# George0828Zhang/simulst

Measured on AMD Instinct MI355X. Metric: decoded tgt tokens/sec (Emformer encoder + wait-k=5 greedy decode, MuST-C en-de shape), higher is better.
Workload: dtype bf16; 1 GPU; configs[1]: Emformer enc (12L) + wait-k=5 dec (6L), 80x1000 fbank, batch 64/GPU, 110 forced greedy steps; batch_per_gpu=64, frames=1000, decode_steps=110, streams=3, warmup_steps_executed=164

## Files before the change

include/simulst_hip.h:

```cpp
#ifndef SIMULST_HIP_H
#define SIMULST_HIP_H

#include <stdint.h>

#ifdef __cplusplus
extern "C" {
#endif

typedef struct simulst_handle simulst_handle;

enum { SIMULST_F32 = 0, SIMULST_BF16 = 1 };

enum {
  SIMULST_OK = 0,
  SIMULST_E_NULL = -1,
  SIMULST_E_SHAPE = -2,
  SIMULST_E_DTYPE = -3,
  SIMULST_E_ARG = -4
};

enum {
  SIMULST_EPI_BIAS = 0,
  SIMULST_EPI_BIAS_GELU = 1,
  SIMULST_EPI_BIAS_RES = 2,
  SIMULST_EPI_GLU = 3,
  SIMULST_EPI_EMF_OUT = 4,
  SIMULST_EPI_BIAS_F32OUT = 5,
  SIMULST_EPI_BIAS_RES_GELU = 6
};

enum { SIMULST_ATTN_HARD = 0, SIMULST_ATTN_INFINITE_LOOKBACK = 1, SIMULST_ATTN_WAITK = 2,
       SIMULST_ATTN_CHUNKWISE = 3, SIMULST_ATTN_FULL = 4 };

enum { SIMULST_K_LINEAR = 0, SIMULST_K_LAYERNORM = 1, SIMULST_K_EMF_ATTN = 2, SIMULST_K_CONV_POS = 3,
       SIMULST_K_DEC_SELF_ATTN = 4, SIMULST_K_DEC_CROSS_ATTN = 5, SIMULST_K_SCAN = 6,
       SIMULST_K_ARGMAX = 7, SIMULST_K_MISC = 8, SIMULST_K_LINEAR_SKINNY = 9, SIMULST_K_LINEAR_TILE64 = 10,
       SIMULST_K_DEC_QKV_CHAIN = 11, SIMULST_K_DEC_PROJ_CHAIN = 12, SIMULST_K_DEC_FFN_CHAIN = 13,
       SIMULST_K_DEC_ATTN_CHAIN = 14, SIMULST_K_DEC_VOCAB_CHAIN = 15,
       SIMULST_K_DEC_TALL_GEMM = 16, SIMULST_K_COUNT = 17 };

int simulst_create(simulst_handle** out, void* hip_stream);
int simulst_destroy(simulst_handle* h);
int simulst_set_stream(simulst_handle* h, void* hip_stream);
const char* simulst_last_error(simulst_handle* h);
int simulst_version(void);
int simulst_stream_create(void** out_stream, int32_t priority, const uint32_t* cu_mask, int32_t mask_words);
int simulst_stream_destroy(void* stream);
int simulst_timer_enable(simulst_handle* h, int kernel_class, int on);
int simulst_timer_read(simulst_handle* h, int kernel_class, double* total_ms, int64_t* launches);
int simulst_timer_reset(simulst_handle* h);
int simulst_graph_enable(simulst_handle* h, int on);
enum { SIMULST_OPT_VALU_ATTENTION = 0, SIMULST_OPT_UNFUSED_DECODE = 1, SIMULST_OPT_FFN_WAVES = 2, SIMULST_OPT_DEC_CHAIN = 3,
       SIMULST_OPT_DEC_ATTN_CHAIN_MAX_ROWS = 4, SIMULST_OPT_DEC_ATTN_CHAIN_ROWS = 5, SIMULST_OPT_FUSED_ARGMAX = 6,
       SIMULST_OPT_DEC_VOCAB_CHAIN_SPLIT = 7, SIMULST_OPT_DEC_EMBED_QKV_CHAIN = 8, SIMULST_OPT_PANEL_WIDE = 9,
       SIMULST_OPT_DEC_FUSE_PROJ_CROSS = 10, SIMULST_OPT_WEIGHT_STATIONARY = 11, SIMULST_OPT_CONV_TILE256 = 12, SIMULST_OPT_DEC_FUSE_FFN_QKV = 13, SIMULST_OPT_DEC_CHAIN_ROWS32 = 14,
       SIMULST_OPT_DEC_TALL_FFN = 15 };
int simulst_set_option(simulst_handle* h, int32_t option, int32_t value);
int simulst_get_option(simulst_handle* h, int32_t option, int32_t* value);
int simulst_has_experiments(void);

#ifdef SIMULST_DEBUG_HOOKS
int simulst_debug_ffn_variant(simulst_handle* h, int variant);

int simulst_debug_chain_lds_bytes(simulst_handle* h, int32_t bytes);
int simulst_debug_chain_xmode(simulst_handle* h, int32_t mode);
int simulst_debug_chain_tail(simulst_handle* h, void* dbg);
int64_t simulst_debug_chain_probe_bytes(int32_t B);
int simulst_debug_chain_probe(simulst_handle* h, const void* ctx, void* x, const void* wo_fm, const float* bo,
                              const float* ln_g, const float* ln_b, const void* wq_fm, const float* bq, void* q,
                              int32_t B, int32_t variant, void* dbg);
#endif

typedef struct {
  int32_t M_batches, rows_per_batch, N, K;
  int64_t a_batch_stride, a_row_stride, a_lead;
  int64_t c_batch_stride, c_row_stride;
  int64_t r_batch_stride, r_row_stride;
  int32_t epilogue, dtype;
  float scale;
  int32_t n_main, aux_rows;
  int64_t aux_batch_stride;
  const float* ln_gamma;
  const float* ln_beta;
  int32_t w_fragment_major;
  int32_t c_head_dim;
  int64_t c_head_stride;
  int32_t c_tensor_heads;
  int64_t c_tensor_stride;
} simulst_linear_desc;

int simulst_linear(simulst_handle* h, const simulst_linear_desc* d, const void* A, const void* W,
                   const float* bias, const void* R, void* C, void* aux);
int simulst_dec_tall_gemm(simulst_handle* h, const void* A, const void* W, const float* bias, const void* R, void* C,
                          int32_t B, int32_t N, int32_t K, int32_t dtype);
int simulst_dec_tall_fc1(simulst_handle* h, const void* A, const void* W, const float* bias, const float* ln_g, const float* ln_b,
                         void* C, int32_t B, int32_t N, int32_t K, int32_t dtype);

int simulst_fbank(simulst_handle* h, const float* wave, int64_t wave_stride, const float* window, const float* tw_cos,
                  const float* tw_sin, const int32_t* mel_lo, const float* mel_w, void* out, int32_t B,
                  int32_t n_frames, int32_t n_mel, float preemphasis, int32_t out_dtype);

int simulst_conv_pos(simulst_handle* h, const void* x, const void* hist, const void* W,
                     const float* bias, const int32_t* lengths, void* y,
                     int32_t B, int32_t T, int32_t D, int32_t groups, int32_t k, int32_t dtype);

int simulst_conv_pos_mfma(simulst_handle* h, const void* x, const void* hist, const void* Wp, const float* bias,
                          const int32_t* lengths, void* y, int32_t B, int32_t T, int32_t D, int32_t groups,
                          int32_t k);

int simulst_emformer_pack_rows(simulst_handle* h, const void* x, void* X, int32_t B, int32_t T, int32_t D, int32_t seg_len,
                               int32_t right_context, int32_t n_seg, int32_t dtype);

int simulst_emformer_ffn(simulst_handle* h, const void* x, const float* ln_gamma, const float* ln_beta,
                         const void* w1_packed, const float* b1, const void* w2_packed, const float* b2, void* out,
                         int64_t rows, int32_t D, int32_t F, int32_t dtype);

int simulst_emformer_ffn_prenorm(simulst_handle* h, const void* x, const float* ln_gamma, const float* ln_beta,
                                 const void* w1_packed, const float* b1, const void* w2_packed, const float* b2, void* out,
                                 const float* next_gamma, const float* next_beta, const int32_t* lengths, void* z_next,
                                 int32_t B, int32_t T, int32_t D, int32_t F, int32_t n_mem, int32_t n_rc, int32_t n_sum,
                                 int32_t seg_len, int32_t dtype);

int simulst_emformer_ffn_prenorm_qkv(simulst_handle* h, const void* x, const float* ln_gamma, const float* ln_beta,
                                     const void* w1_packed, const float* b1, const void* w2_packed, const float* b2, void* out,
                                     const float* next_gamma, const float* next_beta, const int32_t* lengths, void* z_next,
                                     const void* wqkv_fm, const float* bqkv, void* qkv_next,
                                     int32_t B, int32_t T, int32_t D, int32_t F, int32_t n_mem, int32_t n_rc, int32_t n_sum,
                                     int32_t seg_len, int32_t dtype);

int simulst_emformer_qkv_mem_sum(simulst_handle* h, const void* z, const void* wqkv_fm, const float* bqkv, void* qkv,
                                 int32_t B, int32_t T, int32_t D, int32_t n_mem, int32_t n_rc, int32_t n_sum, int32_t dtype);

int simulst_emformer_prenorm(simulst_handle* h, const void* X, const float* gamma, const float* beta,
                             const int32_t* lengths, void* Z, int32_t B, int32_t T, int32_t D,
                             int32_t n_mem, int32_t n_rc, int32_t n_sum, int32_t seg_len, int32_t dtype);

int simulst_layernorm(simulst_handle* h, const void* X, const float* gamma, const float* beta, void* Y,
                      int64_t rows, int32_t D, int64_t x_row_stride, int64_t y_row_stride, int32_t dtype);

int simulst_segment_mean(simulst_handle* h, const void* X, const int32_t* lengths, void* out,
                         int32_t B, int32_t T, int32_t D, int64_t x_batch_stride, int64_t out_batch_stride,
                         int32_t seg_len, int32_t n_out, int32_t dtype);

typedef struct {
  int32_t B, T, D, H, S, R, Lc, M;
  int32_t n_mem, n_seg;
  int32_t use_summary;
  int32_t dtype;
} simulst_emf_attn_desc;

int simulst_emformer_attention(simulst_handle* h, const simulst_emf_attn_desc* d, const void* QKV,
                               const int32_t* lengths, const void* lc_k, const void* lc_v,
                               const int32_t* lc_valid, const int32_t* n_mem_valid, void* CTX);

int simulst_waitk_p_choose(simulst_handle* h, float* p, const int32_t* key_len, int32_t BH,
                           int32_t tgt_len, int32_t tgt_offset, int32_t S, int32_t k, int32_t online);

int simulst_mma_step_search(simulst_handle* h, const float* p, int64_t* head_step, uint8_t* head_read,
                            float* alpha, const int32_t* src_len, int32_t BH, int32_t S,
                            int32_t mass_preservation);

int simulst_expected_alignment(simulst_handle* h, const float* p, float* alpha, const int32_t* key_len,
                               int32_t BH, int32_t U, int32_t S, float eps);

int simulst_mass_preservation(simulst_handle* h, float* alpha, const int32_t* key_len,
                              int32_t BH, int32_t U, int32_t S);

int simulst_expected_delays(simulst_handle* h, const float* alpha, float* out, int64_t rows, int32_t S);

enum { SIMULST_LATENCY_AL = 0, SIMULST_LATENCY_AP = 1, SIMULST_LATENCY_DAL = 2 };
int simulst_latency_metric(simulst_handle* h, const float* delays, const float* src_len, const float* tgt_len,
                           const uint8_t* target_padding_mask, float* out, int32_t B, int32_t T, int32_t metric);

int simulst_expected_alignment_backward(simulst_handle* h, const float* p, const float* alpha, const float* grad_alpha,
                                        float* grad_p, const int32_t* key_len, int32_t BH, int32_t U, int32_t S,
                                        float eps);
int simulst_expected_delays_backward(simulst_handle* h, const float* grad_out, float* grad_alpha, int64_t rows, int32_t S);
int simulst_latency_metric_backward(simulst_handle* h, const float* delays, const float* src_len, const float* tgt_len,
                                    const uint8_t* target_padding_mask, const float* grad_out, float* grad_delays,
                                    int32_t B, int32_t T, int32_t metric);

int simulst_expected_soft_attention(simulst_handle* h, const float* alpha, const float* energy,
                                    float* beta, const int32_t* key_len, int32_t BH, int32_t U,
                                    int32_t S, int32_t chunk_size, float eps);

int simulst_step_p_choose(simulst_handle* h, const void* q, const void* Kmono, float energy_bias,
                          const int32_t* key_len, float* p, int32_t B, int32_t S_cap, int32_t H, int32_t d,
                          int32_t ratio, int32_t incremental, int32_t attn_type, int32_t waitk_k,
                          const int32_t* tgt_idx, int32_t online, int32_t dtype);

int simulst_step_p_choose_padded(simulst_handle* h, const void* q, const void* Kmono, float energy_bias,
                                 const int32_t* key_len, float* p, int32_t B, int32_t S_pad, int32_t S_cap, int32_t H,
                                 int32_t d, int32_t ratio, int32_t incremental, int32_t attn_type, float pad_threshold,
                                 int32_t dtype);

int simulst_cif_integrate(simulst_handle* h, const void* x, const float* alpha, const int32_t* src_len,
                          void* out, int32_t* cif_len, float* delays, float* tail_w, float* alpha_sum,
                          int32_t B, int32_t S, int32_t C, int32_t T_cap, float beta, float tail_thres,
                          int32_t dtype);

int simulst_cif_alpha_head(simulst_handle* h, const void* hidden, const float* gamma, const float* beta_ln,
                           const void* w, float bias, float* alpha, int64_t rows, int32_t D, int32_t dtype);

int simulst_embed_tokens(simulst_handle* h, const int64_t* tokens, const void* E, const float* pos_table,
                         const int32_t* pos_row, void* x, int32_t B, int32_t D, float scale, int32_t dtype);

int simulst_decoder_self_attention(simulst_handle* h, const void* qkv, void* k_cache, void* v_cache,
                                   const int32_t* n_prev, void* ctx, int32_t B, int32_t H, int32_t d,
                                   int32_t cap, int32_t dtype);

int simulst_decoder_cross_attention(simulst_handle* h, const void* q, const void* Kc, const void* Vc,
                                    const int64_t* step, const int32_t* key_len, void* ctx, float* beta,
                                    int32_t B, int32_t H, int32_t d, int32_t S_cap, int32_t attn_type,
                                    int32_t mass_preservation, int32_t dtype);

int simulst_greedy_argmax(simulst_handle* h, const float* logits, const float* eos_bias, int64_t* out,
                          int32_t B, int32_t V, int32_t pad_idx, int32_t eos_idx, int32_t mask_eos);

int simulst_pack_fragment_major(simulst_handle* h, const void* W, void* out, int32_t N, int32_t K, int32_t dtype);

int64_t simulst_ctc_best_alignment_scratch_bytes(int32_t N, int32_t S, int32_t max_target_length);
int simulst_ctc_best_alignment(simulst_handle* h, const float* log_probs, int64_t lp_stride_t, int64_t lp_stride_b,
                               int64_t lp_stride_v, const int64_t* targets, int64_t tg_stride_b,
                               const int64_t* input_lengths, const int64_t* target_lengths, int32_t S, int32_t N,
                               int32_t max_target_length, int32_t blank, int32_t as_labels, void* scratch,
                               int64_t* out, float* neg_log_likelihood);

typedef struct {
  const void* wqkv; const float* bqkv;
  const void* wo; const float* bo;
  const float *ln1_g, *ln1_b, *ln2_g, *ln2_b, *ln3_g, *ln3_b;
  const void* c_wq; const float* c_bq;
  const void* c_wq_soft; const float* c_bq_soft;
  const void* c_wo; const float* c_bo;
  const void* fc1; const float* b1; const void* fc2; const float* b2;
  float energy_bias;
  void *k_cache, *v_cache;
  int64_t* head_step;
  uint8_t* head_read;
  const void *Kmono, *Ksoft, *V;
  const float* Kpool;
} simulst_dec_layer;

typedef struct {
  int32_t B, D, H, F, V, n_layers, cap, S_cap, dtype;
  int32_t attn_type, ratio, waitk_k, mass_preservation, online;
  int32_t pad_idx, eos_idx;
  int32_t n_prev_uniform;
  float embed_scale;
  const void* E;
  const void* out_proj;
  const float* pos_table;
  const float *ln_g, *ln_b;
  const int32_t* enc_len;
  int32_t* n_prev;
  void *x, *qkv, *ctx, *q, *q2, *hidden;
  float* logits;
  void* x_mid;
  float* partial_self;
  int32_t weights_fragment_major;
  float* ffn_partial;
  int32_t P_cap;
  int32_t* ffn_sem;
} simulst_decoder_desc;

int simulst_mma_decode(simulst_handle* h, const simulst_decoder_desc* d, const simulst_dec_layer* layers,
                       int64_t* tokens_io, int64_t* out_tokens, int32_t n_steps, int32_t mask_eos);

int simulst_mma_retire_rows(simulst_handle* h, const simulst_decoder_desc* d, const simulst_dec_layer* layers,
                            const int64_t* chunk_tokens, int32_t n_steps, int32_t rows, int32_t B, int32_t* slot_row,
                            int32_t* row_cap, int64_t* last_tokens, int64_t* hyp, int32_t U, int32_t* enc_len_bh,
                            int32_t* result);

int simulst_beam_topk(simulst_handle* h, const float* logits, int32_t R, int32_t V, int32_t beam, int32_t step,
                      const int32_t* max_len, const int32_t* finished, int32_t pad_idx, int32_t eos_idx, float* cand_lp,
                      int32_t* cand_tok);

int simulst_beam_select(simulst_handle* h, const float* cand_lp, const int32_t* cand_tok, int32_t Bs, int32_t beam, int32_t V,
                        int32_t step, const int32_t* max_len, int32_t L, double lenpen, int32_t eos_idx, float* cum,
                        int64_t* next_tok, int32_t* reorder, int32_t* bp_parent, int32_t* bp_token, float* bp_cum,
                        int32_t* fin_step, int32_t* fin_row, float* fin_score, float* fin_raw, int32_t* fin_count,
                        int32_t* finished, int32_t* result);

int simulst_beam_reorder(simulst_handle* h, const simulst_decoder_desc* d, const simulst_dec_layer* src, const simulst_dec_layer* dst,
                         const int32_t* reorder, const int32_t* finished, int32_t beam, int32_t n_prev, int32_t* result);

int simulst_beam_backtrack(simulst_handle* h, int32_t Bs, int32_t beam, int32_t nbest, int32_t L, const int32_t* bp_parent,
                           const int32_t* bp_token, const float* bp_cum, const int32_t* fin_step, const int32_t* fin_row,
                           const float* fin_score, const float* fin_raw, const int32_t* fin_count, int32_t pad_idx,
                           int32_t eos_idx, int64_t* tokens, int32_t* lengths, float* scores, float* pos_scores);

typedef struct {
  uint8_t* active;
  uint8_t* read_flag;
  uint8_t* online;
  uint8_t* done;
  int32_t* delays_ms;
  int64_t* hyp;
  int32_t cap, cur_ms, max_len_now;
  int32_t n_chunks;
  const int32_t* sched_rows;
  const int32_t* sched_ms;
  const int32_t* sched_max_len;
  int32_t* chunk_idx;
  int32_t* enc_len;
  int32_t* tok_chunk;
  const int32_t* row_chunks;
  int32_t ff_waitk, ff_ratio;
  float* p_probe; int64_t* step_probe; const int64_t* step_force; int32_t probe_P;
  int32_t* row_map; int32_t compact_rows;
} simulst_stream_ctl;

int simulst_mma_stream_steps(simulst_handle* h, const simulst_decoder_desc* d, const simulst_dec_layer* layers,
                             int64_t* tokens_io, const simulst_stream_ctl* ctl, int32_t n_iter);


typedef struct {
  const void* wqkv; const float* bqkv;
  const void* wo; const float* bo;
  const float *ln1_g, *ln1_b, *ln2_g, *ln2_b, *ln3_g, *ln3_b;
  const void* c_wq;
  const void* c_wo; const float* c_bo;
  const void* fc1; const float* b1; const void* fc2; const float* b2;
  void *k_cache, *v_cache;
  const void* Kc;
} simulst_cif_dec_layer;

typedef struct {
  int32_t B, D, H, F, V, n_layers, cap, n_cap, dtype;
  int32_t pad_idx, eos_idx;
  int32_t highway;
  int32_t n_prev_uniform;
  float embed_scale, overshoot_weight;
  const void* E; const void* out_proj; const float* pos_table; const float *ln_g, *ln_b;
  const int32_t* cif_len;
  const void* cif;
  int32_t* n_prev;
  void *x, *qkv, *ctx, *q, *hidden;
  float* logits;
  void* kk;
  void* cif_t;
  float* eos_bias;
  void* x_mid; float* ffn_partial;
  int32_t weights_fragment_major;
} simulst_cif_decoder_desc;

int simulst_cif_decode(simulst_handle* h, const simulst_cif_decoder_desc* d, const simulst_cif_dec_layer* layers,
                       int64_t* tokens_io, int64_t* out_tokens, int32_t n_steps, int32_t mask_eos);

typedef struct {
  uint8_t* online;
  uint8_t* done;
  int32_t* delays_ms;
  int64_t* hyp;
  int32_t cap, cur_ms, max_len_now;
  int32_t n_chunks;
  const int32_t* sched_cif_len;
  const int32_t* sched_ms;
  const int32_t* sched_max_len;
  int32_t* chunk_idx;
  int32_t* cif_len;
  int32_t* tok_chunk;
  const int32_t* row_chunks;
} simulst_cif_stream_ctl;

int simulst_cif_stream_steps(simulst_handle* h, const simulst_cif_decoder_desc* d, const simulst_cif_dec_layer* layers,
                             int64_t* tokens_io, const simulst_cif_stream_ctl* ctl, int32_t n_iter);

int simulst_cif_stream_append(simulst_handle* h, const void* out, const int32_t* n, const float* tail_w, void* acc,
                              int32_t* acc_len, void* prev_feat, float* prev_weight, int32_t B, int32_t T_cap, int32_t n_cap,
                              int32_t D, float beta, int32_t finish, int32_t dtype);

int simulst_decoder_proj_chain(simulst_handle* h, const void* ctx, void* x, const void* wo_fm, const float* bo,
                               const float* ln_g, const float* ln_b, const void* wq_fm, const float* bq, void* q,
                               const void* wq2_fm, const float* bq2, void* q2, int32_t B, int32_t D, int32_t dtype);
int simulst_decoder_ffn_chain(simulst_handle* h, const void* ctx, void* x, const void* wco_fm, const float* bco,
                              const float* ln_g, const float* ln_b, const void* w1_fm, const float* b1, const void* w2_fm,
                              const float* b2, float* partial, int32_t* sem, void* x_mid, int32_t B, int32_t D, int32_t F,
                              int32_t dtype);
int simulst_decoder_slab_sum_qkv(simulst_handle* h, const void* x_mid, void* x, const float* partial, const float* b2,
                                 const float* ln_g, const float* ln_b, const void* wqkv_fm, const float* bqkv, void* qkv,
                                 int32_t B, int32_t D, int32_t F, int32_t dtype);

int simulst_decoder_vocab_chain(simulst_handle* h, const void* x_mid, void* x, const float* partial, const float* b2,
                                const float* ln_g, const float* ln_b, const void* wout_fm, float* pairs, int32_t B, int32_t D,
                                int32_t F, int32_t V, int32_t split, int32_t skip_a, int32_t skip_b, const float* row_bias,
                                int32_t row_bias_col, int32_t dtype);

#ifdef SIMULST_EXPERIMENTS
int simulst_decoder_attn_proj_chain(simulst_handle* h, const void* qkv, void* k_cache, void* v_cache, const int32_t* n_prev,
                                    void* x, const void* wo_fm, const float* bo, const float* ln_g, const float* ln_b,
                                    const void* wq_fm, const float* bq, void* q, const void* wq2_fm, const float* bq2, void* q2,
                                    const void* kk_gelu, int32_t B, int32_t H, int32_t d, int32_t cap, int32_t n_prev_uniform,
                                    int32_t rows_per_workgroup, int32_t dtype);
#endif

int simulst_pool_keys(simulst_handle* h, const void* Kmono, float* Kpool, const int32_t* key_len, int32_t B, int32_t H, int32_t d,
                      int32_t S_cap, int32_t P_cap, int32_t ratio, int32_t j_lo, int32_t j_hi, int32_t dtype);

int simulst_policy_cross_attention(simulst_handle* h, const void* qm, const void* qs, const void* Kmono,
                                   const void* Ksoft, const void* Vc, float energy_bias, const int32_t* key_len,
                                   const int32_t* tgt_idx, int64_t* head_step, uint8_t* head_read, void* ctx,
                                   int32_t B, int32_t H, int32_t d, int32_t S_cap, int32_t ratio, int32_t attn_type,
                                   int32_t waitk_k, int32_t online, int32_t mass_preservation, int32_t dtype);

int simulst_decoder_self_attention_causal(simulst_handle* h, const void* qkv, void* ctx, int32_t B, int32_t U, int32_t H,
                                          int32_t d, int32_t dtype);

enum { SIMULST_ENERGY_SOFT = 0, SIMULST_ENERGY_MONOTONIC = 1, SIMULST_ENERGY_WAITK = 2 };
int simulst_mma_energy(simulst_handle* h, const void* q, const void* K, float* out, const int32_t* key_len, float energy_bias,
                       float pad_threshold, int32_t B, int32_t U, int32_t S, int32_t S_cap, int32_t H, int32_t d, int32_t ratio,
                       int32_t mode, int32_t waitk_k, int32_t dtype);

int simulst_mma_softmax(simulst_handle* h, float* energy, const int32_t* key_len, int32_t B, int32_t U, int32_t S, int32_t H);

int simulst_mma_context(simulst_handle* h, const float* beta, const void* V, void* ctx, int32_t B, int32_t U, int32_t S,
                        int32_t S_cap, int32_t H, int32_t d, int32_t dtype);

int simulst_transducer_pool(simulst_handle* h, const void* x, const int32_t* lengths, void* y, int32_t* new_len, int32_t B,
                            int32_t S_in, int32_t D, int64_t x_batch_stride, int32_t T_max, int32_t k, int32_t dtype);

int simulst_joiner_scan(simulst_handle* h, const float* P, const float* g, const void* W_fm, const int32_t* prev_emit,
                        const int32_t* src_len, float* blank_logit, float* best, int32_t* best_idx, int32_t B, int32_t S,
                        int32_t D, int32_t V, int32_t blank, int32_t n_split, int32_t dtype);

int simulst_joiner_emit(simulst_handle* h, const float* P, const float* g, const float* blank_logit, const float* best,
                        const int32_t* best_idx, int32_t* prev_emit, const int32_t* src_len, void* z, int32_t* at_eos, int32_t B,
                        int32_t S, int32_t D, int32_t V, int32_t blank, int32_t n_split, int32_t dtype);

int simulst_joiner_mask_blank(simulst_handle* h, float* logits, const int32_t* at_eos, int32_t B, int32_t V, int32_t blank);

#ifdef __cplusplus
}
#endif
#endif
```

simulst_amd/_lib.py:

```python
import ctypes as C
import os

_HERE = os.path.dirname(os.path.abspath(__file__))
LIB_PATH = os.environ.get("SIMULST_LIB_PATH") or os.path.join(_HERE, "libsimulst_hip.so")

F32, BF16 = 0, 1
EPI_BIAS, EPI_BIAS_GELU, EPI_BIAS_RES, EPI_GLU, EPI_EMF_OUT, EPI_BIAS_F32OUT, EPI_BIAS_RES_GELU = range(7)
ATTN_HARD, ATTN_INFINITE_LOOKBACK, ATTN_WAITK, ATTN_CHUNKWISE, ATTN_FULL = range(5)
(K_LINEAR, K_LAYERNORM, K_EMF_ATTN, K_CONV_POS, K_DEC_SELF_ATTN, K_DEC_CROSS_ATTN, K_SCAN, K_ARGMAX,
 K_MISC, K_LINEAR_SKINNY, K_LINEAR_TILE64, K_DEC_QKV_CHAIN, K_DEC_PROJ_CHAIN, K_DEC_FFN_CHAIN, K_DEC_ATTN_CHAIN,
 K_DEC_VOCAB_CHAIN, K_DEC_TALL_GEMM, K_COUNT) = range(18)
KERNEL_CLASS_NAMES = ["linear", "layernorm", "emformer_attention", "conv_pos", "decoder_self_attention",
                      "decoder_cross_attention", "scan", "argmax", "misc", "linear_skinny", "linear_tile64",
                      "dec_qkv_chain", "dec_proj_chain", "dec_ffn_chain", "dec_attn_proj_chain", "dec_vocab_chain", "dec_tall_gemm"]

ATTN_ENUM = {"hard_aligned": ATTN_HARD, "infinite_lookback": ATTN_INFINITE_LOOKBACK,
             "waitk": ATTN_WAITK, "chunkwise": ATTN_CHUNKWISE, "full": ATTN_FULL}


class LinearDesc(C.Structure):
    _fields_ = [("M_batches", C.c_int32), ("rows_per_batch", C.c_int32), ("N", C.c_int32), ("K", C.c_int32),
                ("a_batch_stride", C.c_int64), ("a_row_stride", C.c_int64), ("a_lead", C.c_int64),
                ("c_batch_stride", C.c_int64), ("c_row_stride", C.c_int64),
                ("r_batch_stride", C.c_int64), ("r_row_stride", C.c_int64),
                ("epilogue", C.c_int32), ("dtype", C.c_int32), ("scale", C.c_float),
                ("n_main", C.c_int32), ("aux_rows", C.c_int32), ("aux_batch_stride", C.c_int64),
                ("ln_gamma", C.c_void_p), ("ln_beta", C.c_void_p), ("w_fragment_major", C.c_int32),
                ("c_head_dim", C.c_int32), ("c_head_stride", C.c_int64),
                ("c_tensor_heads", C.c_int32), ("c_tensor_stride", C.c_int64)]


class EmfAttnDesc(C.Structure):
    _fields_ = [(n, C.c_int32) for n in ("B", "T", "D", "H", "S", "R", "Lc", "M", "n_mem", "n_seg",
                                         "use_summary", "dtype")]


_vp, _i32, _i64, _f32 = C.c_void_p, C.c_int32, C.c_int64, C.c_float


class DecLayer(C.Structure):
    _fields_ = [(n, C.c_void_p) for n in ("wqkv", "bqkv", "wo", "bo", "ln1_g", "ln1_b", "ln2_g", "ln2_b", "ln3_g",
                                          "ln3_b", "c_wq", "c_bq", "c_wq_soft", "c_bq_soft", "c_wo", "c_bo", "fc1",
                                          "b1", "fc2", "b2")] + [("energy_bias", C.c_float)] + \
               [(n, C.c_void_p) for n in ("k_cache", "v_cache", "head_step", "head_read", "Kmono", "Ksoft", "V", "Kpool")]


class DecoderDesc(C.Structure):
    _fields_ = [(n, C.c_int32) for n in ("B", "D", "H", "F", "V", "n_layers", "cap", "S_cap", "dtype", "attn_type",
                                         "ratio", "waitk_k", "mass_preservation", "online", "pad_idx", "eos_idx",
                                         "n_prev_uniform")] + \
               [("embed_scale", C.c_float)] + \
               [(n, C.c_void_p) for n in ("E", "out_proj", "pos_table", "ln_g", "ln_b", "enc_len", "n_prev", "x", "qkv",
                                          "ctx", "q", "q2", "hidden", "logits", "x_mid", "partial_self")] + \
               [("weights_fragment_major", C.c_int32), ("ffn_partial", C.c_void_p), ("P_cap", C.c_int32), ("ffn_sem", C.c_void_p)]

class CifDecLayer(C.Structure):
    _fields_ = [(n, C.c_void_p) for n in ("wqkv", "bqkv", "wo", "bo", "ln1_g", "ln1_b", "ln2_g", "ln2_b", "ln3_g", "ln3_b",
                                          "c_wq", "c_wo", "c_bo", "fc1", "b1", "fc2", "b2", "k_cache", "v_cache", "Kc")]


class CifDecoderDesc(C.Structure):
    _fields_ = [(n, C.c_int32) for n in ("B", "D", "H", "F", "V", "n_layers", "cap", "n_cap", "dtype", "pad_idx", "eos_idx",
                                         "highway", "n_prev_uniform")] + \
               [("embed_scale", C.c_float), ("overshoot_weight", C.c_float)] + \
               [(n, C.c_void_p) for n in ("E", "out_proj", "pos_table", "ln_g", "ln_b", "cif_len", "cif", "n_prev", "x", "qkv",
                                          "ctx", "q", "hidden", "logits", "kk", "cif_t", "eos_bias", "x_mid", "ffn_partial")] + \
               [("weights_fragment_major", C.c_int32)]


class CifStreamCtl(C.Structure):
    _fields_ = [(n, C.c_void_p) for n in ("online", "done", "delays_ms", "hyp")] + \
               [(n, C.c_int32) for n in ("cap", "cur_ms", "max_len_now", "n_chunks")] + \
               [(n, C.c_void_p) for n in ("sched_cif_len", "sched_ms", "sched_max_len", "chunk_idx", "cif_len", "tok_chunk", "row_chunks")]


class StreamCtl(C.Structure):
    _fields_ = [(n, C.c_void_p) for n in ("active", "read_flag", "online", "done", "delays_ms", "hyp")] + \
               [(n, C.c_int32) for n in ("cap", "cur_ms", "max_len_now", "n_chunks")] + \
               [(n, C.c_void_p) for n in ("sched_rows", "sched_ms", "sched_max_len", "chunk_idx", "enc_len", "tok_chunk", "row_chunks")] + \
               [(n, C.c_int32) for n in ("ff_waitk", "ff_ratio")] + \
               [(n, C.c_void_p) for n in ("p_probe", "step_probe", "step_force")] + [("probe_P", C.c_int32)] + \
               [("row_map", C.c_void_p), ("compact_rows", C.c_int32)]


SIGNATURES = {
    "simulst_create": [C.POINTER(_vp), _vp],
    "simulst_destroy": [_vp],
    "simulst_set_stream": [_vp, _vp],
    "simulst_last_error": [_vp],
    "simulst_version": [],
    "simulst_timer_enable": [_vp, C.c_int, C.c_int],
    "simulst_timer_read": [_vp, C.c_int, C.POINTER(C.c_double), C.POINTER(_i64)],
    "simulst_timer_reset": [_vp],
    "simulst_graph_enable": [_vp, C.c_int],
    "simulst_set_option": [_vp, _i32, _i32],
    "simulst_get_option": [_vp, _i32, C.POINTER(_i32)],
    "simulst_stream_create": [C.POINTER(_vp), _i32, _vp, _i32],
    "simulst_stream_destroy": [_vp],
    "simulst_pack_fragment_major": [_vp, _vp, _vp, _i32, _i32, _i32],
    "simulst_linear": [_vp, C.POINTER(LinearDesc), _vp, _vp, _vp, _vp, _vp, _vp],
    "simulst_dec_tall_gemm": [_vp, _vp, _vp, _vp, _vp, _vp, _i32, _i32, _i32, _i32],
    "simulst_dec_tall_fc1": [_vp, _vp, _vp, _vp, _vp, _vp, _vp, _i32, _i32, _i32, _i32],
    "simulst_conv_pos": [_vp, _vp, _vp, _vp, _vp, _vp, _vp, _i32, _i32, _i32, _i32, _i32, _i32],
    "simulst_ctc_best_alignment_scratch_bytes": [_i32, _i32, _i32],
    "simulst_ctc_best_alignment": [_vp, _vp, _i64, _i64, _i64, _vp, _i64, _vp, _vp, _i32, _i32, _i32, _i32, _i32, _vp,
                                   _vp, _vp],
    "simulst_fbank": [_vp, _vp, _i64, _vp, _vp, _vp, _vp, _vp, _vp, _i32, _i32, _i32, C.c_float, _i32],
    "simulst_conv_pos_mfma": [_vp, _vp, _vp, _vp, _vp, _vp, _vp, _i32, _i32, _i32, _i32, _i32],
    "simulst_emformer_pack_rows": [_vp, _vp, _vp, _i32, _i32, _i32, _i32, _i32, _i32, _i32],
    "simulst_emformer_ffn": [_vp, _vp, _vp, _vp, _vp, _vp, _vp, _vp, _vp, _i64, _i32, _i32, _i32],
    "simulst_emformer_ffn_prenorm": [_vp, _vp, _vp, _vp, _vp, _vp, _vp, _vp, _vp, _vp, _vp, _vp, _vp, _i32, _i32, _i32, _i32, _i32, _i32,
                                     _i32, _i32, _i32],
    "simulst_emformer_ffn_prenorm_qkv": [_vp, _vp, _vp, _vp, _vp, _vp, _vp, _vp, _vp, _vp, _vp, _vp, _vp, _vp, _vp, _vp, _i32, _i32, _i32, _i32,
                                         _i32, _i32, _i32, _i32, _i32],
    "simulst_emformer_qkv_mem_sum": [_vp, _vp, _vp, _vp, _vp, _i32, _i32, _i32, _i32, _i32, _i32, _i32],
    "simulst_emformer_prenorm": [_vp, _vp, _vp, _vp, _vp, _vp, _i32, _i32, _i32, _i32, _i32, _i32, _i32, _i32],
    "simulst_layernorm": [_vp, _vp, _vp, _vp, _vp, _i64, _i32, _i64, _i64, _i32],
    "simulst_segment_mean": [_vp, _vp, _vp, _vp, _i32, _i32, _i32, _i64, _i64, _i32, _i32, _i32],
    "simulst_emformer_attention": [_vp, C.POINTER(EmfAttnDesc), _vp, _vp, _vp, _vp, _vp, _vp, _vp],
    "simulst_waitk_p_choose": [_vp, _vp, _vp, _i32, _i32, _i32, _i32, _i32, _i32],
    "simulst_mma_step_search": [_vp, _vp, _vp, _vp, _vp, _vp, _i32, _i32, _i32],
    "simulst_expected_alignment": [_vp, _vp, _vp, _vp, _i32, _i32, _i32, _f32],
    "simulst_mass_preservation": [_vp, _vp, _vp, _i32, _i32, _i32],
    "simulst_expected_delays": [_vp, _vp, _vp, _i64, _i32],
    "simulst_latency_metric": [_vp, _vp, _vp, _vp, _vp, _vp, _i32, _i32, _i32],
    "simulst_expected_alignment_backward": [_vp, _vp, _vp, _vp, _vp, _vp, _i32, _i32, _i32, _f32],
    "simulst_expected_delays_backward": [_vp, _vp, _vp, _i64, _i32],
    "simulst_latency_metric_backward": [_vp, _vp, _vp, _vp, _vp, _vp, _vp, _i32, _i32, _i32],
    "simulst_expected_soft_attention": [_vp, _vp, _vp, _vp, _vp, _i32, _i32, _i32, _i32, _f32],
    "simulst_step_p_choose": [_vp, _vp, _vp, _f32, _vp, _vp, _i32, _i32, _i32, _i32, _i32, _i32, _i32, _i32,
                              _vp, _i32, _i32],
    "simulst_cif_integrate": [_vp, _vp, _vp, _vp, _vp, _vp, _vp, _vp, _vp, _i32, _i32, _i32, _i32, _f32, _f32, _i32],
    "simulst_cif_alpha_head": [_vp, _vp, _vp, _vp, _vp, _f32, _vp, _i64, _i32, _i32],
    "simulst_embed_tokens": [_vp, _vp, _vp, _vp, _vp, _vp, _i32, _i32, _f32, _i32],
    "simulst_decoder_self_attention": [_vp, _vp, _vp, _vp, _vp, _vp, _i32, _i32, _i32, _i32, _i32],
    "simulst_decoder_cross_attention": [_vp, _vp, _vp, _vp, _vp, _vp, _vp, _vp, _i32, _i32, _i32, _i32, _i32,
                                        _i32, _i32],
    "simulst_greedy_argmax": [_vp, _vp, _vp, _vp, _i32, _i32, _i32, _i32, _i32],
    "simulst_mma_decode": [_vp, C.POINTER(DecoderDesc), C.POINTER(DecLayer), _vp, _vp, _i32, _i32],
    "simulst_mma_stream_steps": [_vp, C.POINTER(DecoderDesc), C.POINTER(DecLayer), _vp, C.POINTER(StreamCtl), _i32],
    "simulst_mma_retire_rows": [_vp, C.POINTER(DecoderDesc), C.POINTER(DecLayer), _vp, _i32, _i32, _i32, _vp, _vp, _vp, _vp, _i32,
                                _vp, _vp],
    "simulst_beam_topk": [_vp, _vp, _i32, _i32, _i32, _i32, _vp, _vp, _i32, _i32, _vp, _vp],
    "simulst_beam_select": [_vp, _vp, _vp, _i32, _i32, _i32, _i32, _vp, _i32, C.c_double, _i32] + [_vp] * 13,
    "simulst_beam_reorder": [_vp, C.POINTER(DecoderDesc), C.POINTER(DecLayer), C.POINTER(DecLayer), _vp, _vp, _i32, _i32, _vp],
    "simulst_beam_backtrack": [_vp, _i32, _i32, _i32, _i32] + [_vp] * 8 + [_i32, _i32] + [_vp] * 4,
    "simulst_step_p_choose_padded": [_vp, _vp, _vp, _f32, _vp, _vp] + [_i32] * 8 + [_f32, _i32],
    "simulst_pool_keys": [_vp, _vp, _vp, _vp] + [_i32] * 9,
    "simulst_policy_cross_attention": [_vp, _vp, _vp, _vp, _vp, _vp, _f32, _vp, _vp, _vp, _vp, _vp, _i32, _i32, _i32,
                                       _i32, _i32, _i32, _i32, _i32, _i32, _i32],
    "simulst_cif_decode": [_vp, C.POINTER(CifDecoderDesc), C.POINTER(CifDecLayer), _vp, _vp, _i32, _i32],
    "simulst_cif_stream_steps": [_vp, C.POINTER(CifDecoderDesc), C.POINTER(CifDecLayer), _vp, C.POINTER(CifStreamCtl), _i32],
    "simulst_cif_stream_append": [_vp] * 8 + [_i32, _i32, _i32, _i32, C.c_float, _i32, _i32],
    "simulst_decoder_proj_chain": [_vp] * 13 + [_i32, _i32, _i32],
    "simulst_decoder_ffn_chain": [_vp] * 14 + [_i32, _i32, _i32, _i32],
    "simulst_decoder_slab_sum_qkv": [_vp] * 10 + [_i32, _i32, _i32, _i32],
    "simulst_decoder_vocab_chain": [_vp] * 9 + [_i32] * 7 + [_vp, _i32, _i32],
    "simulst_has_experiments": [],
    "simulst_decoder_self_attention_causal": [_vp, _vp, _vp, _i32, _i32, _i32, _i32, _i32],
    "simulst_mma_energy": [_vp, _vp, _vp, _vp, _vp, _f32, _f32] + [_i32] * 10,
    "simulst_mma_softmax": [_vp, _vp, _vp, _i32, _i32, _i32, _i32],
    "simulst_mma_context": [_vp, _vp, _vp, _vp] + [_i32] * 7,
    "simulst_transducer_pool": [_vp, _vp, _vp, _vp, _vp, _i32, _i32, _i32, _i64, _i32, _i32, _i32],
    "simulst_joiner_scan": [_vp] * 9 + [_i32] * 7,
    "simulst_joiner_emit": [_vp] * 10 + [_i32] * 7,
    "simulst_joiner_mask_blank": [_vp, _vp, _vp, _i32, _i32, _i32],
}
ENERGY_SOFT, ENERGY_MONOTONIC, ENERGY_WAITK = range(3)

EXPERIMENT_SIGNATURES = {
    "simulst_decoder_attn_proj_chain": [_vp] * 17 + [_i32] * 7,
}

DEBUG_SIGNATURES = {
    "simulst_debug_ffn_variant": [_vp, C.c_int],
    "simulst_debug_chain_lds_bytes": [_vp, _i32],
    "simulst_debug_chain_xmode": [_vp, _i32],
    "simulst_debug_chain_tail": [_vp, _vp],
    "simulst_debug_chain_probe_bytes": [_i32],
    "simulst_debug_chain_probe": [_vp] * 10 + [_i32, _i32, _vp],
}
(OPT_VALU_ATTENTION, OPT_UNFUSED_DECODE, OPT_FFN_WAVES, OPT_DEC_CHAIN, OPT_DEC_ATTN_CHAIN_MAX_ROWS, OPT_DEC_ATTN_CHAIN_ROWS,
 OPT_FUSED_ARGMAX, OPT_DEC_VOCAB_CHAIN_SPLIT, OPT_DEC_EMBED_QKV_CHAIN, OPT_PANEL_WIDE, OPT_DEC_FUSE_PROJ_CROSS,
 OPT_WEIGHT_STATIONARY, OPT_CONV_TILE256, OPT_DEC_FUSE_FFN_QKV, OPT_DEC_CHAIN_ROWS32, OPT_DEC_TALL_FFN) = range(16)

_lib = None
ABI_VERSION = 108


def load():
    global _lib
    if _lib is not None:
        return _lib
    if not os.path.exists(LIB_PATH):
        raise RuntimeError(
            f"simulst_amd: {LIB_PATH} is missing -- build it with `python -c 'import __graft_entry__ as g; "
            f"g.build()'` (or `make -C simulst_amd/csrc`). There is no CPU fallback.")
    lib = C.CDLL(LIB_PATH)
    for name, argtypes in SIGNATURES.items():
        fn = getattr(lib, name)
        fn.argtypes = argtypes
        fn.restype = (C.c_char_p if name == "simulst_last_error"
                      else C.c_int64 if name == "simulst_ctc_best_alignment_scratch_bytes"
                      else C.c_int)
    for name, argtypes in EXPERIMENT_SIGNATURES.items():
        fn = getattr(lib, name, None)
        if fn is not None:
            fn.argtypes = argtypes
            fn.restype = C.c_int
    for name, argtypes in DEBUG_SIGNATURES.items():
        fn = getattr(lib, name, None)
        if fn is not None:
            fn.argtypes = argtypes
            fn.restype = C.c_int64 if name == "simulst_debug_chain_probe_bytes" else C.c_int
    if lib.simulst_version() != ABI_VERSION:
        raise RuntimeError(f"simulst_amd: {LIB_PATH} reports ABI version {lib.simulst_version()}, this binding is written for "
                           f"{ABI_VERSION} -- rebuild the library (make -C simulst_amd/csrc)")
    _lib = lib
    return lib


def has_experiments():
    return bool(load().simulst_has_experiments())


def cu_mask_words(cus_per_xcd, n_xcd=8, cus_total_per_xcd=32, take_high=False):
    lo, hi = (cus_total_per_xcd - cus_per_xcd, cus_total_per_xcd) if take_high else (0, cus_per_xcd)
    words = [0] * (n_xcd * cus_total_per_xcd // 32)
    for cu in range(lo, hi):
        for x in range(n_xcd):
            i = cu * n_xcd + x
            words[i >> 5] |= 1 << (i & 31)
    return words


def create_stream(device=None, cu_mask=None, priority=0):
    import torch
    lib = load()
    arr = (C.c_uint32 * len(cu_mask))(*cu_mask) if cu_mask else None
    out = _vp()
    rc = lib.simulst_stream_create(C.byref(out), int(priority), arr, len(cu_mask) if cu_mask else 0)
    if rc != 0:
        raise RuntimeError(f"simulst_stream_create failed (status {rc})")
    return torch.cuda.ExternalStream(out.value, device=device)


def destroy_stream(stream):
    rc = load().simulst_stream_destroy(_vp(stream.cuda_stream))
    if rc != 0:
        raise RuntimeError(f"simulst_stream_destroy failed (status {rc})")


class Handle:

    def __init__(self, stream_ptr=None):
        self.lib = load()
        if stream_ptr is None:
            import torch
            if not torch.cuda.is_available():
                raise RuntimeError("simulst_amd: no HIP device visible; the hot path is GPU only "
                                   "(no CPU fallback)")
            stream_ptr = torch.cuda.current_stream().cuda_stream
        self._h = _vp()
        self.stream_ptr = stream_ptr
        rc = self.lib.simulst_create(C.byref(self._h), _vp(stream_ptr))
        if rc != 0:
            raise RuntimeError(f"simulst_create failed: {rc}")

    @property
    def ptr(self):
        return self._h

    def set_stream(self, stream_ptr):
        self.check(self.lib.simulst_set_stream(self._h, _vp(stream_ptr)), "simulst_set_stream")
        self.stream_ptr = stream_ptr

    def check(self, rc, what):
        if rc != 0:
            msg = self.lib.simulst_last_error(self._h)
            raise RuntimeError(f"{what} failed (status {rc}): {msg.decode() if msg else ''}")

    def set_option(self, option, value):
        self.check(self.lib.simulst_set_option(self._h, int(option), int(value)), "simulst_set_option")

    def get_option(self, option):
        v = _i32(0)
        self.check(self.lib.simulst_get_option(self._h, int(option), C.byref(v)), "simulst_get_option")
        return v.value

    def timer_enable(self, kernel_class=-1, on=True):
        self.check(self.lib.simulst_timer_enable(self._h, kernel_class, int(on)), "simulst_timer_enable")

    def graph_enable(self, on=True):
        self.check(self.lib.simulst_graph_enable(self._h, int(on)), "simulst_graph_enable")

    def timer_reset(self):
        self.check(self.lib.simulst_timer_reset(self._h), "simulst_timer_reset")

    def timer_read(self, kernel_class):
        ms, n = C.c_double(0), _i64(0)
        self.check(self.lib.simulst_timer_read(self._h, kernel_class, C.byref(ms), C.byref(n)), "simulst_timer_read")
        return ms.value, n.value

    def __del__(self):
        try:
            if getattr(self, "_h", None) is not None and self._h.value:
                self.lib.simulst_destroy(self._h)
                self._h = _vp()
        except Exception:
            pass
```

simulst_amd/csrc/common.h:

```cpp
#pragma once
#include <hip/hip_runtime.h>
#include <hip/hip_bf16.h>
#include <stdint.h>
#include <string>
#include <vector>

#include "../../include/simulst_hip.h"

typedef __hip_bfloat16 bf16;
typedef float f32x16 __attribute__((ext_vector_type(16)));
typedef float f32x4 __attribute__((ext_vector_type(4)));
typedef short s16x8 __attribute__((ext_vector_type(8)));
typedef short s16x4 __attribute__((ext_vector_type(4)));

struct simulst_handle {
  hipStream_t stream;
  std::string err;
  bool timer_on[SIMULST_K_COUNT];
  double timer_ms[SIMULST_K_COUNT];
  int64_t timer_n[SIMULST_K_COUNT];
  struct EvPair { hipEvent_t a, b; int cls; };
  std::vector<EvPair> ev_pool;
  int ev_used;
  void* ws;
  size_t ws_bytes;
  bool graph_on;
  bool capturing;
  bool force_valu_attention;
  int panel_split_min_rows;
  int panel_split_blocks;
  int mid_min_blocks;
  int mid_narrow_min_rows;
  int skinny_min_blocks_tall;
  int fuse_q_max_rows;
  bool force_unfused_decode;
  hipGraphExec_t graph_exec;
  uint64_t graph_key;
  bool ffn_lds_attr_set;
  bool ffn_pipe_lds_attr_set;
  bool qkv_rows_lds_attr_set;
  bool ea_general_only;
  int ffn_variant;
  int ffn_waves;
  bool conv_pos_lds_attr_set;
  bool ctc_lds_attr_set;
  bool dec_chain_on;
  int dec_chain_min_rows;
  int dec_chain_max_rows;
  int dec_chain_ffn_max_rows;
  bool dec_tall_ffn;
  int dec_tall_min_rows;
  bool dec_chain_lds_attr_set;
  int dec_chain_lds_bytes;
  bool dec_chain_probe_attr_set;
  void* dec_chain_tail;
  int dec_chain_xmode;
  int dec_attn_chain_max_rows;
  int dec_attn_chain_rows;
  bool dec_embed_qkv_chain;
  bool panel_wide_plain_stores;
  bool dec_chain_rows32;
  int dec_chain_rows32_min;
  bool dec_fuse_ffn_qkv;
  int* chain_sem;
  int chain_sem_splits;
  int tile256;
  bool tile256_lds_attr_set, tile256_ring_attr_set;
  bool wstat;
  bool wstat_lds_attr_set;
  int n_cus;
  bool panel_wide;
  int policy_lds_bytes;
  int dec_vocab_chain_split;
  bool fused_argmax;
  bool dec_fuse_proj_cross;
  int* fuse_flags;
  int fuse_epoch;
};

#define SL_CHECK_NULL(h, p)                                   \
  do {                                                        \
    if ((p) == nullptr) {                                     \
      if (h) (h)->err = std::string("null pointer: ") + #p;   \
      return SIMULST_E_NULL;                                  \
    }                                                         \
  } while (0)

#define SL_REQUIRE(h, cond, code, msg)                        \
  do {                                                        \
    if (!(cond)) {                                            \
      if (h) (h)->err = std::string(msg) + " [" #cond "]";    \
      return (code);                                          \
    }                                                         \
  } while (0)

struct KTimer {
  simulst_handle* h;
  int cls;
  int slot;
  KTimer(simulst_handle* h_, int cls_) : h(h_), cls(cls_), slot(-1) {
    if (!h->timer_on[cls_] || h->capturing) return;
    if (h->ev_used >= (int)h->ev_pool.size()) {
      if (h->ev_pool.size() >= 40000) return;
      simulst_handle::EvPair p;
      if (hipEventCreate(&p.a) != hipSuccess || hipEventCreate(&p.b) != hipSuccess) return;
      p.cls = cls_;
      h->ev_pool.push_back(p);
    }
    slot = h->ev_used++;
    h->ev_pool[slot].cls = cls_;
    if (slot == 0) (void)hipEventRecord(h->ev_pool[0].a, h->stream);
  }
  ~KTimer() {
    if (slot >= 0) (void)hipEventRecord(h->ev_pool[slot].b, h->stream);
  }
};

static inline int sl_launch_status(simulst_handle* h, const char* what) {
  hipError_t e = hipGetLastError();
  if (e != hipSuccess) {
    h->err = std::string(what) + ": " + hipGetErrorString(e);
    return (int)e;
  }
  return SIMULST_OK;
}

__host__ __device__ __forceinline__ int pooled_count(int len, int ratio, bool incremental, bool last) {
  if (last && len < ratio) return incremental ? (len - 1 > 1 ? len - 1 : 1) : len;
  int P = (len + ratio - 1) / ratio;
  if (incremental) { const int fl = len / ratio > 1 ? len / ratio : 1; P = P < fl ? P : fl; }
  return P;
}
__device__ __forceinline__ void pooled_frames(int j, int len, int ratio, bool last, int& f0, int& f1) {
  if (last) {
    f1 = len < ratio ? j + 1 : min((j + 1) * ratio, len);
    f0 = f1 - 1;
  } else {
    f0 = j * ratio;
    f1 = min(f0 + ratio, len);
  }
}

__device__ __forceinline__ float to_f32(float v) { return v; }
__device__ __forceinline__ float to_f32(bf16 v) { return __bfloat162float(v); }
template <typename T> __device__ __forceinline__ T from_f32(float v);
template <> __device__ __forceinline__ float from_f32<float>(float v) { return v; }
template <> __device__ __forceinline__ bf16 from_f32<bf16>(float v) { return __float2bfloat16(v); }

__device__ __forceinline__ float bf16_bits_to_f32(unsigned short b) {
  return __uint_as_float(((unsigned int)b) << 16);
}

__device__ __forceinline__ float wave_sum(float v) {
#pragma unroll
  for (int o = 32; o > 0; o >>= 1) v += __shfl_xor(v, o, 64);
  return v;
}
__device__ __forceinline__ float wave_max(float v) {
#pragma unroll
  for (int o = 32; o > 0; o >>= 1) v = fmaxf(v, __shfl_xor(v, o, 64));
  return v;
}
__device__ __forceinline__ float wave_scan_incl(float v, int lane) {
#pragma unroll
  for (int o = 1; o < 64; o <<= 1) {
    float t = __shfl_up(v, o, 64);
    if (lane >= o) v += t;
  }
  return v;
}

__device__ __forceinline__ float wave_scan_incl_dpp(float v) {
#define SL_DPP_ADD(ctrl, row_mask, bound)                                                                              \
  v += __builtin_bit_cast(float, __builtin_amdgcn_update_dpp(0, __builtin_bit_cast(int, v), ctrl, row_mask, 0xf, bound))
  SL_DPP_ADD(0x111, 0xf, true);
  SL_DPP_ADD(0x112, 0xf, true);
  SL_DPP_ADD(0x114, 0xf, true);
  SL_DPP_ADD(0x118, 0xf, true);
  SL_DPP_ADD(0x142, 0xa, false);
  SL_DPP_ADD(0x143, 0xc, false);
#undef SL_DPP_ADD
  return v;
}
template <int M>
__device__ __forceinline__ float lane_xor_dpp(float v) {
  static_assert(M == 1 || M == 2 || M == 4 || M == 8, "DPP butterfly steps inside a 16-lane row");
  constexpr int ctrl = M == 1 ? 0xB1 : M == 2 ? 0x4E : M == 4 ? 0x141 : 0x128;
  return __builtin_bit_cast(float, __builtin_amdgcn_update_dpp(0, __builtin_bit_cast(int, v), ctrl, 0xf, 0xf, false));
}
template <int O>
__device__ __forceinline__ float lane_xor(float v) {
  if constexpr (O <= 8) return lane_xor_dpp<O>(v);
  else return __shfl_xor(v, O, 64);
}

__device__ __forceinline__ float wave_last(float v) {
  return __builtin_bit_cast(float, __builtin_amdgcn_readlane(__builtin_bit_cast(int, v), 63));
}

__device__ __forceinline__ float gelu_erf(float x) { return 0.5f * x * (1.0f + erff(x * 0.70710678118654752440f)); }
typedef float f32x2 __attribute__((ext_vector_type(2)));
#define SL_GELU_C1 (-2.3020009994506836f)
#define SL_GELU_C2 (-1.838383436203003f)
#define SL_GELU_C3 (-0.4171730577945709f)
#define SL_GELU_C4 (0.11517949402332306f)
#define SL_GELU_C5 (-0.015619269572198391f)
__device__ __forceinline__ f32x2 gelu_fast2(f32x2 x) {
  const f32x2 h = x * 0.5f;
  const f32x2 a = __builtin_elementwise_abs(h);
  f32x2 q = a * SL_GELU_C5 + SL_GELU_C4;
  q = q * a + SL_GELU_C3;
  q = q * a + SL_GELU_C2;
  q = q * a + SL_GELU_C1;
  q = q * a;
  f32x2 e;
  e.x = __builtin_amdgcn_exp2f(q.x);
  e.y = __builtin_amdgcn_exp2f(q.y);
  return (h + a) - a * e;
}
__device__ __forceinline__ float gelu_fast(float x) { return gelu_fast2(f32x2{x, x}).x; }
typedef unsigned int u32x4_t __attribute__((ext_vector_type(4)));
template <typename T>
__device__ __forceinline__ uint4 ld_stream16(const T* p) {
  const u32x4_t v = __builtin_nontemporal_load(reinterpret_cast<const u32x4_t*>(p));
  return make_uint4(v.x, v.y, v.z, v.w);
}
__device__ __forceinline__ void st_stream16(void* p, uint4 v) {
  __builtin_nontemporal_store(u32x4_t{v.x, v.y, v.z, v.w}, reinterpret_cast<u32x4_t*>(p));
}
__device__ __forceinline__ float sigmoidf_(float x) { return 1.0f / (1.0f + __expf(-x)); }

__device__ __forceinline__ void load4(const float* p, float (&o)[4]) {
  float4 v = *reinterpret_cast<const float4*>(p);
  o[0] = v.x; o[1] = v.y; o[2] = v.z; o[3] = v.w;
}
__device__ __forceinline__ void load4(const bf16* p, float (&o)[4]) {
  ushort4 v = *reinterpret_cast<const ushort4*>(p);
  o[0] = bf16_bits_to_f32(v.x); o[1] = bf16_bits_to_f32(v.y);
  o[2] = bf16_bits_to_f32(v.z); o[3] = bf16_bits_to_f32(v.w);
}
__device__ __forceinline__ void store4(float* p, const float (&o)[4]) {
  *reinterpret_cast<float4*>(p) = make_float4(o[0], o[1], o[2], o[3]);
}
__device__ __forceinline__ void store4(bf16* p, const float (&o)[4]) {
  bf16 t[4] = {__float2bfloat16(o[0]), __float2bfloat16(o[1]), __float2bfloat16(o[2]), __float2bfloat16(o[3])};
  *reinterpret_cast<uint2*>(p) = *reinterpret_cast<uint2*>(t);
}

int sl_self_attention(simulst_handle* h, const void* qkv, void* k_cache, void* v_cache, const int32_t* n_prev,
                      int np_uniform, void* ctx, int32_t B, int32_t H, int32_t d, int32_t cap, int32_t dtype,
                      const int32_t* row_map = nullptr);

static inline bool sl_self_attention_fused_ok(int H, int d, int cap) {
  return (d == 32 || d == 64) && H * d <= 1024 && cap <= 256;
}
bool sl_dec_chain_ok(const simulst_handle* h, int dtype, int B, int D, int F, bool packed);
int sl_dec_proj_chain(simulst_handle* h, const void* ctx, void* x, const void* Wo, const float* bo, const float* ln_g,
                      const float* ln_b, const void* Wq, const float* bq, void* q, const void* Wq2, const float* bq2,
                      void* q2, int B, const void* kk_gelu = nullptr);
bool sl_dec_attn_chain_ok(const simulst_handle* h, int dtype, int B, int H, int d, int cap);
int sl_dec_vocab_chain_split(const simulst_handle* h, int dtype, int B, int V, int D, bool packed, bool has_ln);
int sl_dec_embed_qkv_chain(simulst_handle* h, const float2* pairs, int n_pairs, int64_t* tokens, int64_t* out_row, int32_t* n_prev,
                           int np, const void* E, const float* pos, float scale, int pad_idx, void* x, const float* ln_g,
                           const float* ln_b, const void* Wqkv, const float* bqkv, void* qkv, int B);
int sl_dec_vocab_chain(simulst_handle* h, const void* x_mid, void* x, const float* partial, const float* b2, const float* ln_g,
                       const float* ln_b, const void* Wout, float2* pairs, int B, int F, int V, int n_cb, int skip_a, int skip_b,
                       const float* row_bias = nullptr, int row_bias_col = -1);
int sl_dec_attn_proj_chain(simulst_handle* h, const void* qkv, void* k_cache, void* v_cache, const int32_t* n_prev, int np_uniform,
                           int cap, void* x, const void* Wo, const float* bo, const float* ln_g, const float* ln_b, const void* Wq,
                           const float* bq, void* q, const void* Wq2, const float* bq2, void* q2, int B, const void* kk_gelu = nullptr);
bool sl_dec_proj_cross_fused_ok(const simulst_handle* h, int dtype, int B, int H, int d, int S_cap, int attn_type, bool lockstep_offline,
                                bool separate_soft);
int sl_dec_proj_cross_fused(simulst_handle* h, const void* ctx_in, void* x, const void* Wo, const float* bo, const float* ln_g,
                            const float* ln_b, const void* Wq, const float* bq, void* q, const void* Ks, const void* Vc,
                            const int32_t* key_len, const int32_t* tgt_idx, int64_t* head_step, uint8_t* head_read, void* ctx_out, int B,
                            int H, int S_cap, int ratio, int waitk_k, int online, int mass_pres, int n_hint);
int sl_dec_ffn_chain(simulst_handle* h, const void* ctx, void* x, const void* Wco, const float* bco, const float* ln_g,
                     const float* ln_b, const void* W1, const float* b1, const void* W2, const float* b2, float* partial,
                     int32_t* sem, void* x_mid, int B, int F);
bool sl_dec_ffn_qkv_chain_ok(const simulst_handle* h, int B, int F);
int sl_dec_ffn_qkv_chain(simulst_handle* h, const void* ctx, void* x, const void* Wco, const float* bco, const float* ln_g,
                         const float* ln_b, const void* W1, const float* b1, const void* W2, const float* b2, float* partial, int B,
                         int F, const float* nln_g, const float* nln_b, const void* nWqkv, const float* nbqkv, void* qkv);
int sl_dec_qkv_chain(simulst_handle* h, const void* x_mid, void* x, const float* partial, const float* b2, const float* ln_g,
                     const float* ln_b, const void* Wqkv, const float* bqkv, void* qkv, int B, int F);
int sl_self_attention_fused(simulst_handle* h, const void* x, const float* ln_g, const float* ln_b, const void* Wqkv,
                            const float* bqkv, const void* Wo, void* k_cache, void* v_cache, const int32_t* n_prev,
                            int np_uniform, float* partial, int32_t B, int32_t H, int32_t d, int32_t cap,
                            int32_t dtype);

int sl_emformer_attention_mfma(simulst_handle* h, const simulst_emf_attn_desc* d, const void* QKV,
                               const int32_t* lengths, const void* lc_k, const void* lc_v, const int32_t* lc_valid,
                               const int32_t* n_mem_valid, void* CTX);
```

simulst_amd/csrc/dec_gemm_tall.hip:

```cpp
#include "decode_plan.h"
#include "gemm_plan.h"

namespace {

constexpr int DT_CH = 8;
constexpr int DT_STAGE = 4 * DT_CH * 64;

__global__ __launch_bounds__(256) void dec_tall_fc2_kernel(const bf16* __restrict__ A, const bf16* __restrict__ W,
                                                           const float* __restrict__ bias, const bf16* R, bf16* C, int M, int N, int K) {
  constexpr int KS = 32, G = 8;
  __shared__ __attribute__((aligned(16))) unsigned char smem[2 * DT_STAGE * 16];
  uint4* wl = reinterpret_cast<uint4*>(smem);
  float (*tile)[65] = reinterpret_cast<float (*)[65]>(smem);
  float* lbias = reinterpret_cast<float*>(smem + 64 * 65 * sizeof(float));
  const int tid = threadIdx.x, lane = tid & 63, wave = tid >> 6;
  const int lr = lane & 15, lg = lane >> 4;
  int bx, by;
  {
    const int id = (int)blockIdx.x + (int)gridDim.x * (int)blockIdx.y, total = (int)(gridDim.x * gridDim.y);
    const int full = total & ~7;
    const int bid = id < full ? (id & 7) * (full >> 3) + (id >> 3) : id;
    bx = bid % (int)gridDim.x;
    by = bid / (int)gridDim.x;
  }
  const int n0 = bx * 64, m0 = by * 64;
  const int nks = K / KS, nch = (nks + DT_CH - 1) / DT_CH, ntile = N >> 4;
  const int er = tid >> 2, ec = (tid & 3) * 16;
  const bool eok = m0 + er < M && n0 + ec < N;
  const long eoff = eok ? (long)(m0 + er) * N + n0 + ec : 0;
  const uint4 rpre0 = ld16(R + eoff), rpre1 = ld16(R + eoff + 8);
  const float bpre = (tid < 64 && bias && n0 + tid < N) ? bias[n0 + tid] : 0.f;
  const bf16* arow = A + (long)min(m0 + wave * 16 + lr, M - 1) * K + lg * G;
  const bf16* wlane = W + lane * G;
  uint4 faN[DT_CH], wv[DT_CH];
  auto load_chunk = [&](int c) {
#pragma unroll
    for (int u = 0; u < DT_CH; ++u) {
      const int s = c * DT_CH + u;
      faN[u] = ld16(arow + (s < nks ? s : 0) * KS);
    }
#pragma unroll
    for (int q = 0; q < DT_CH; ++q) {
      const int s = c * DT_CH + (q & 1) * 4 + wave, tj = (n0 >> 4) + (q >> 1);
      const bool ok = s < nks && tj < ntile;
      wv[q] = ld16(wlane + ((long)(ok ? tj : 0) * nks + (ok ? s : 0)) * (64 * G));
    }
  };
  auto store_chunk = [&](int c, uint4* dst) {
#pragma unroll
    for (int q = 0; q < DT_CH; ++q) {
      const int s = c * DT_CH + (q & 1) * 4 + wave, tj = (n0 >> 4) + (q >> 1);
      const bool ok = s < nks && tj < ntile;
      dst[q * 256 + tid] = make_uint4(ok ? wv[q].x : 0u, ok ? wv[q].y : 0u, ok ? wv[q].z : 0u, ok ? wv[q].w : 0u);
    }
  };
  f32x4 acc[4][4];
#pragma unroll
  for (int t = 0; t < 4; ++t)
#pragma unroll
    for (int j = 0; j < 4; ++j) acc[t][j] = f32x4{0.f, 0.f, 0.f, 0.f};
  load_chunk(0);
  store_chunk(0, wl);
  for (int c = 0; c < nch; ++c) {
    uint4 fa[DT_CH];
#pragma unroll
    for (int u = 0; u < DT_CH; ++u) fa[u] = faN[u];
    if ((c + 1) * DT_CH > nks) {
#pragma unroll
      for (int u = 0; u < DT_CH; ++u)
        if (c * DT_CH + u >= nks) fa[u] = make_uint4(0u, 0u, 0u, 0u);
    }
    const bool more = c + 1 < nch;
    if (more) load_chunk(c + 1);
    __syncthreads();
    const uint4* wb = wl + (c & 1) * DT_STAGE;
    uint4 wf[2][4];
#pragma unroll
    for (int j = 0; j < 4; ++j) wf[0][j] = wb[(j * DT_CH) * 64 + lane];
#pragma unroll
    for (int u = 0; u < DT_CH; ++u) {
      if (u + 1 < DT_CH) {
#pragma unroll
        for (int j = 0; j < 4; ++j) wf[(u + 1) & 1][j] = wb[(j * DT_CH + u + 1) * 64 + lane];
      }
      __builtin_amdgcn_sched_barrier(0);
      const bf16x8_t af = *reinterpret_cast<const bf16x8_t*>(&fa[u]);
#pragma unroll
      for (int j = 0; j < 4; ++j)
        acc[u & 3][j] = __builtin_amdgcn_mfma_f32_16x16x32_bf16(af, *reinterpret_cast<const bf16x8_t*>(&wf[u & 1][j]), acc[u & 3][j], 0, 0, 0);
      __builtin_amdgcn_sched_barrier(0);
    }
    if (more) store_chunk(c + 1, wl + ((c + 1) & 1) * DT_STAGE);
  }
  __syncthreads();
#pragma unroll
  for (int j = 0; j < 4; ++j)
#pragma unroll
    for (int e = 0; e < 4; ++e)
      tile[wave * 16 + lg * 4 + e][j * 16 + lr] = ((acc[0][j][e] + acc[1][j][e]) + acc[2][j][e]) + acc[3][j][e];
  if (tid < 64) lbias[tid] = bpre;
  __syncthreads();
  if (!eok) return;
  float y[16];
#pragma unroll
  for (int e = 0; e < 16; ++e) {
    const unsigned int w = reinterpret_cast<const unsigned int*>(e < 8 ? &rpre0 : &rpre1)[(e & 7) >> 1];
    float v = tile[er][ec + e] + lbias[ec + e];
    v += __uint_as_float((e & 1) ? (w & 0xffff0000u) : (w << 16));
    y[e] = v;
  }
  bf16* cp = C + eoff;
#pragma unroll
  for (int e = 0; e < 16; e += 4) store4(cp + e, reinterpret_cast<const float(&)[4]>(y[e]));
}

constexpr int DT_F1_STEPS = 2;
constexpr int DT_F1_PF = 3;

__global__ __launch_bounds__(256, 2) void dec_tall_fc1_kernel(const bf16* __restrict__ A, const bf16* __restrict__ Wp,
                                                              const float* __restrict__ bias, const float* __restrict__ ln_g,
                                                              const float* __restrict__ ln_b, bf16* __restrict__ C, int M, int N, int K) {
  __shared__ __attribute__((aligned(16))) uint4 wl[2][4 * 8 * 64];
  float* lng = reinterpret_cast<float*>(wl[1]);
  float* lnb = lng + 256;
  const int tid = threadIdx.x, lane = tid & 63, wave = tid >> 6;
  const int lr = lane & 15, lg = lane >> 4;
  const int m0 = blockIdx.x * 128;
  const int nks = K / 32;
  uint4 fa[2][8];
#pragma unroll
  for (int m = 0; m < 2; ++m) {
    const int ar = m0 + wave * 32 + m * 16 + lr;
    const bool aok = ar < M;
    const bf16* arow = A + (long)(aok ? ar : 0) * K;
#pragma unroll
    for (int s = 0; s < 8; ++s) {
      const bool ok = aok && s < nks;
      const uint4 v = ld16(arow + (ok ? s * 32 + lg * 8 : 0));
      fa[m][s] = make_uint4(ok ? v.x : 0u, ok ? v.y : 0u, ok ? v.z : 0u, ok ? v.w : 0u);
    }
  }
  const int n_all = (N + 63) / 64;
  const int step0 = blockIdx.y * DT_F1_STEPS, n_steps = min(n_all, step0 + DT_F1_STEPS);
  uint4 wv[8];
  auto wload = [&](int step) {
#pragma unroll
    for (int q = 0; q < 8; ++q) {
      const int slot = q * 256 + tid;
      const int ln = slot & 63, s = (slot >> 6) & 7, j = slot >> 9;
      const int ntile = step * 4 + j;
      const bool ok = s < nks && ntile * 16 < N;
      const uint4 v = ld16(Wp + (((long)(ok ? ntile : 0) * nks + (ok ? s : 0)) * 64 + ln) * 8);
      wv[q] = make_uint4(ok ? v.x : 0u, ok ? v.y : 0u, ok ? v.z : 0u, ok ? v.w : 0u);
    }
  };
  float4 bnext[4];
  auto bload = [&](int step) {
#pragma unroll
    for (int j = 0; j < 4; ++j) {
      const int c = step * 64 + j * 16 + 4 * lg;
      bnext[j] = (bias && c < N) ? *reinterpret_cast<const float4*>(bias + c) : float4{0.f, 0.f, 0.f, 0.f};
    }
  };
  wload(step0);
  bload(step0);
  for (int k = tid; k < K; k += 256) { lng[k] = ln_g[k]; lnb[k] = ln_b[k]; }
  __syncthreads();
#pragma unroll
  for (int m = 0; m < 2; ++m) {
    float s1 = 0.f, s2 = 0.f;
#pragma unroll
    for (int s = 0; s < 8; ++s) moments_mid(fa[m][s], s1, s2, bf16());
    s1 += __shfl_xor(s1, 16, 64); s2 += __shfl_xor(s2, 16, 64);
    s1 += __shfl_xor(s1, 32, 64); s2 += __shfl_xor(s2, 32, 64);
    const float mean = s1 / (float)K;
    const float rstd = 1.0f / sqrtf(fmaxf(s2 / (float)K - mean * mean, 0.f) + 1e-5f);
#pragma unroll
    for (int s = 0; s < 8; ++s)
      if (s < nks) fa[m][s] = ln_frag_mid(fa[m][s], mean, rstd, lng, lnb, s * 32 + lg * 8, bf16());
  }
#pragma unroll
  for (int q = 0; q < 8; ++q) wl[0][q * 256 + tid] = wv[q];
  for (int step = step0; step < n_steps; ++step) {
    const int cur = (step - step0) & 1;
    float4 bcur[4];
#pragma unroll
    for (int j = 0; j < 4; ++j) bcur[j] = bnext[j];
    const bool more = step + 1 < n_steps;
    if (more) { wload(step + 1); bload(step + 1); }
    __syncthreads();
    f32x4 acc[2][4];
#pragma unroll
    for (int m = 0; m < 2; ++m)
#pragma unroll
      for (int j = 0; j < 4; ++j) acc[m][j] = f32x4{0.f, 0.f, 0.f, 0.f};
    const uint4* wb = wl[cur];
    u32x4_t wfr[DT_F1_PF];
#pragma unroll
    for (int f = 0; f < DT_F1_PF - 1; ++f) wfr[f] = *reinterpret_cast<const u32x4_t*>(&wb[((f & 3) * 8 + (f >> 2)) * 64 + lane]);
#pragma unroll
    for (int f = 0; f < 32; ++f) {
      const int s = f >> 2, j = f & 3;
      if (f + DT_F1_PF - 1 < 32) {
        const int g2 = f + DT_F1_PF - 1;
        wfr[g2 % DT_F1_PF] = *reinterpret_cast<const u32x4_t*>(&wb[((g2 & 3) * 8 + (g2 >> 2)) * 64 + lane]);
      }
#pragma unroll
      for (int m = 0; m < 2; ++m)
        acc[m][j] = __builtin_amdgcn_mfma_f32_16x16x32_bf16(__builtin_bit_cast(bf16x8_t, wfr[f % DT_F1_PF]),
                                                           *reinterpret_cast<const bf16x8_t*>(&fa[m][s]), acc[m][j], 0, 0, 0);
      asm volatile("" :: "v"(wfr[f % DT_F1_PF]), "v"(acc[0][j]), "v"(acc[1][j]));
    }
    if (more) {
#pragma unroll
      for (int q = 0; q < 8; ++q) wl[cur ^ 1][q * 256 + tid] = wv[q];
    }
#pragma unroll
    for (int m = 0; m < 2; ++m) {
      const int r = m0 + wave * 32 + m * 16 + lr;
#pragma unroll
      for (int j = 0; j < 4; ++j) {
        const int c = step * 64 + j * 16 + 4 * lg;
        const float4 bv = bcur[j];
        f32x2 v0 = f32x2{acc[m][j][0] + bv.x, acc[m][j][1] + bv.y};
        f32x2 v1 = f32x2{acc[m][j][2] + bv.z, acc[m][j][3] + bv.w};
        v0 = gelu_fast2(v0);
        v1 = gelu_fast2(v1);
        const bf16 o0 = __float2bfloat16(v0.x), o1 = __float2bfloat16(v0.y), o2 = __float2bfloat16(v1.x), o3 = __float2bfloat16(v1.y);
        const unsigned int lo = (unsigned int)(*reinterpret_cast<const unsigned short*>(&o0)) |
                                ((unsigned int)(*reinterpret_cast<const unsigned short*>(&o1)) << 16);
        const unsigned int hi = (unsigned int)(*reinterpret_cast<const unsigned short*>(&o2)) |
                                ((unsigned int)(*reinterpret_cast<const unsigned short*>(&o3)) << 16);
        if (r < M && c < N) *reinterpret_cast<uint2*>(C + (long)r * N + c) = make_uint2(lo, hi);
      }
    }
  }
}

}

int sl_dec_tall_fc2(simulst_handle* h, const void* A, const void* W, const float* bias, const void* R, void* C, int B, int N, int K) {
  KTimer t(h, SIMULST_K_DEC_TALL_GEMM);
  hipLaunchKernelGGL(dec_tall_fc2_kernel, dim3((N + 63) / 64, (B + 63) / 64), dim3(256), 0, h->stream, (const bf16*)A, (const bf16*)W,
                     bias, (const bf16*)R, (bf16*)C, B, N, K);
  return sl_launch_status(h, "decode step: tall fc2 tile");
}

int sl_dec_tall_fc1(simulst_handle* h, const void* A, const void* W, const float* bias, const float* ln_g, const float* ln_b, void* C,
                    int B, int N, int K) {
  KTimer t(h, SIMULST_K_DEC_TALL_GEMM);
  const int n_all = (N + 63) / 64;
  hipLaunchKernelGGL(dec_tall_fc1_kernel, dim3((B + 127) / 128, (n_all + DT_F1_STEPS - 1) / DT_F1_STEPS), dim3(256), 0, h->stream,
                     (const bf16*)A, (const bf16*)W, bias, ln_g, ln_b, (bf16*)C, B, N, K);
  return sl_launch_status(h, "decode step: tall fc1 panel");
}

extern "C" int simulst_dec_tall_fc1(simulst_handle* h, const void* A, const void* W, const float* bias, const float* ln_g,
                                    const float* ln_b, void* C, int32_t B, int32_t N, int32_t K, int32_t dtype) {
  if (!h) return SIMULST_E_NULL;
  SL_CHECK_NULL(h, A);
  SL_CHECK_NULL(h, W);
  SL_CHECK_NULL(h, ln_g);
  SL_CHECK_NULL(h, ln_b);
  SL_CHECK_NULL(h, C);
  SL_REQUIRE(h, B > 0 && N > 0 && K > 0, SIMULST_E_SHAPE, "simulst_dec_tall_fc1: non-positive shape");
  SL_REQUIRE(h, sl_dec_tall_fc1_shape_ok(h, dtype, B, N, K, true), SIMULST_E_SHAPE,
             "simulst_dec_tall_fc1: bf16 rows whose simulst_linear launch is the split row panel");
  SL_REQUIRE(h, sl_dec_tall_operands_ok(A, W, C, bias), SIMULST_E_ARG, "simulst_dec_tall_fc1: operands must be 16-byte aligned");
  return sl_dec_tall_fc1(h, A, W, bias, ln_g, ln_b, C, B, N, K);
}

extern "C" int simulst_dec_tall_gemm(simulst_handle* h, const void* A, const void* W, const float* bias, const void* R, void* C,
                                     int32_t B, int32_t N, int32_t K, int32_t dtype) {
  if (!h) return SIMULST_E_NULL;
  SL_CHECK_NULL(h, A);
  SL_CHECK_NULL(h, W);
  SL_CHECK_NULL(h, R);
  SL_CHECK_NULL(h, C);
  SL_REQUIRE(h, B > 0 && N > 0 && K > 0, SIMULST_E_SHAPE, "simulst_dec_tall_gemm: non-positive shape");
  SL_REQUIRE(h, sl_dec_tall_fc2_shape_ok(h, dtype, B, N, K, true), SIMULST_E_SHAPE,
             "simulst_dec_tall_gemm: bf16 rows whose simulst_linear launch is the k-interleaved 16 MT x 16 NT tile without split-K");
  SL_REQUIRE(h, sl_dec_tall_operands_ok(A, W, R, C), SIMULST_E_ARG, "simulst_dec_tall_gemm: operands must be 16-byte aligned");
  return sl_dec_tall_fc2(h, A, W, bias, R, C, B, N, K);
}
```

simulst_amd/csrc/decode_driver.hip:

```cpp
#include "attn_core.h"
#include "policy_core.h"
#include "gemv_mfma.h"
#include "decode_plan.h"
#include "gemm_plan.h"

namespace {

using attn::VL;

struct StreamCtl {
  unsigned char* active;
  unsigned char* read_flag;
  unsigned char* online;
  unsigned char* done;
  int* delays;
  long* hyp;
  int cap, cur_ms, max_len_now;
  int layer;
  const int* sched_rows; const int* sched_ms; const int* sched_max_len;
  const int* row_chunks;
  int* chunk_idx; int* enc_len; int* tok_chunk;
  int n_chunks;
  int ff_waitk, ff_ratio;
  float* p_probe;
  long* step_probe;
  const long* step_force;
  int probe_P;
  const int* row_map;
  int compact_rows;
};

__device__ __forceinline__ bool row_skipped(const StreamCtl ctl, int b) {
  if (!ctl.active) return false;
  const unsigned char rf = ctl.read_flag[b];
  if (!ctl.active[b] || (rf && rf != ctl.layer)) return true;
  return false;
}

struct HeadSplit {
  const float* po;
  const float* bo;
  void* x_mid;
  int w_packed;
};

#ifndef SL_POLICY_WGS
#define SL_POLICY_WGS 4
#endif
template <typename T, int NP, bool FQ>
__global__ __launch_bounds__(256, NP >= 16 ? 2 : (FQ ? 3 : SL_POLICY_WGS)) void policy_cross_attn_kernel(
    const T* __restrict__ qm, const T* __restrict__ qs, const T* __restrict__ Km, const T* __restrict__ Ks,
    const T* __restrict__ Vc, float energy_bias, const int* __restrict__ key_len, const int* __restrict__ tgt_idx,
    long* __restrict__ head_step, unsigned char* __restrict__ head_read, T* __restrict__ ctx, int H, int d,
    int S_cap, int ratio, int attn_type, int waitk_k, int online, int mass_pres, int n_hint,
    const T* __restrict__ xres, const float* __restrict__ ln_g, const float* __restrict__ ln_b,
    const T* __restrict__ Wqm, const float* __restrict__ bqm, const T* __restrict__ Wqs,
    const float* __restrict__ bqs, StreamCtl ctl,
    const float* __restrict__ po, const float* __restrict__ bo, T* __restrict__ x_mid, int w_packed,
    const float* __restrict__ Kpool, int P_cap) {
  constexpr int W = VL<T>::W;
  const int slot = blockIdx.y;
  int brow = slot;
  if (ctl.row_map) { brow = ctl.row_map[slot]; if (brow < 0) return; }
  if (row_skipped(ctl, brow)) return;
  if (ctl.online) online = ctl.online[brow];
  extern __shared__ float sm[];
  float* q_s = sm;
  float* red = sm + 64;
  float* sc = red + attn::RED_FLOATS;
  float* pl = sc + (S_cap > 256 ? S_cap : 256);
  float* pp = pl + S_cap + 1;
  float* xn = pp + S_cap;
  float* qsoft_s = xn + H * d;
  __shared__ int s_found;
  __shared__ __attribute__((aligned(16))) T xn_t[1024];
  const int h = blockIdx.x, b = brow, tid = threadIdx.x, lane = tid & 63;
  const int D = H * d;
  const int len = key_len ? key_len[b] : S_cap;
  const int r = b * H + h;
  const bool pool_last = ratio < 0;
  ratio = ratio < 0 ? -ratio : ratio;
  const int P = pooled_count(len, ratio, true, pool_last);
  const long hb = ((long)b * H + h) * S_cap * d;
  const T* Vh = Vc + hb;
  const T* Kh = Ks ? Ks + hb : nullptr;
  const bool soft = attn_type != SIMULST_ATTN_HARD;
  const bool fast = NP > 0 && soft && S_cap <= 256;
  attn::Regs2<T, NP> rg2;
  const bool full = attn_type == SIMULST_ATTN_FULL;
  const int tg = tgt_idx ? tgt_idx[b] : 0;
  const long hs = full ? 0 : head_step[r];
  if (n_hint < 0) n_hint = attn_type == SIMULST_ATTN_WAITK ? (tg + waitk_k) * ratio : S_cap;
  if (full) n_hint = len;
#ifdef SL_ABLATE_CROSS
  n_hint = 8;
#endif
  const bool fusedq = FQ && xres != nullptr;
  const int n_pref = min(S_cap, n_hint);
  if constexpr (NP > 0) {
    if (fast) attn::prefetch2<T, NP>(rg2, fusedq ? nullptr : qs + (long)slot * D + h * d, Kh, d, Vh, d, n_pref, -1, nullptr, nullptr);
  }
  if constexpr (FQ) if (fusedq) {
    float ps = 0.f;
    for (int k = tid; k < D; k += 256) {
      float v = to_f32(xres[(long)b * D + k]);
      if (po) {
        float a = 0.f;
        for (int hh = 0; hh < H; ++hh) a += po[((long)b * H + hh) * D + k];
        const T r = from_f32<T>(a + (bo ? bo[k] : 0.f) + v);
        if (h == 0) x_mid[(long)b * D + k] = r;
        v = to_f32(r);
      }
      xn[k] = v;
      ps += v;
    }
    const float mean = attn::blk_sum(ps, red + 1024) / (float)D;
    float pq = 0.f;
    for (int k = tid; k < D; k += 256) { const float dd = xn[k] - mean; pq += dd * dd; }
    const float rstd = 1.0f / sqrtf(attn::blk_sum(pq, red + 1024) / (float)D + 1e-5f);
    const float scl = rsqrtf((float)d);
    if (w_packed) {
      constexpr int KS = gemv::MF<T>::KS;
      const int nks = D / KS, wave = tid >> 6, tpp = d >> 4;
      const int tile = (h * d >> 4) + min(wave, tpp - 1);
      gemv::Frag<T, 8> fm;
      gemv::load<T, 8>(fm, Wqm, tile, nks, 0, min(nks, 8));
      for (int k = tid; k < D; k += 256) xn_t[k] = from_f32<T>((xn[k] - mean) * rstd * ln_g[k] + ln_b[k]);
      __syncthreads();
      for (int pass = 0; pass < 2; ++pass) {
        const T* Wp = pass == 0 ? Wqm : Wqs;
        const float* bp = pass == 0 ? bqm : bqs;
        if (!Wp) continue;
        f32x4 acc = {0.f, 0.f, 0.f, 0.f};
        if (pass == 1) gemv::load<T, 8>(fm, Wqs, tile, nks, 0, min(nks, 8));
        gemv::mac<T, 8>(acc, fm, xn_t, min(nks, 8));
        for (int s0 = 8; s0 < nks; s0 += 8) {
          gemv::Frag<T, 8> f;
          gemv::load<T, 8>(f, Wp, tile, nks, s0, min(nks - s0, 8));
          gemv::mac<T, 8>(acc, f, xn_t + s0 * KS, min(nks - s0, 8));
        }
        if (wave < tpp && lane < 16) {
          const int o = wave * 16 + lane;
          const float qv = to_f32(from_f32<T>(acc[0] + (bp ? bp[h * d + o] : 0.f))) * scl;
          if (pass == 0) q_s[o] = qv; else qsoft_s[o] = qv;
        }
      }
    } else {
    for (int k = tid; k < D; k += 256)
      xn[k] = to_f32(from_f32<T>((xn[k] - mean) * rstd * ln_g[k] + ln_b[k]));
    __syncthreads();
    const int o = tid >> 2, part = tid & 3, kq = D >> 2;
    for (int pass = 0; pass < 2; ++pass) {
      const T* Wp = pass == 0 ? Wqm : Wqs;
      const float* bp = pass == 0 ? bqm : bqs;
      if (!Wp) continue;
      float acc = 0.f;
      if (o < d) {
        const T* wr = Wp + (long)(h * d + o) * D + part * kq;
        for (int k = 0; k < kq; k += W) {
          float wv[W];
          VL<T>::cvt(*reinterpret_cast<const uint4*>(wr + k), wv);
#pragma unroll
          for (int i = 0; i < W; ++i) acc = fmaf(wv[i], xn[part * kq + k + i], acc);
        }
      }
      acc += __shfl_xor(acc, 1, 64);
      acc += __shfl_xor(acc, 2, 64);
      if (o < d && part == 0) {
        const float qv = to_f32(from_f32<T>(acc + (bp ? bp[h * d + o] : 0.f))) * scl;
        if (pass == 0) q_s[o] = qv; else qsoft_s[o] = qv;
      }
    }
    }
    __syncthreads();
  }
  long st;
  if (full) {
    st = len - 1;
  } else if (attn_type == SIMULST_ATTN_WAITK) {
    const policy::Step w = policy::waitk_step(tg, waitk_k, online, P, ratio, len, mass_pres, hs);
    st = w.found;
    if (tid == 0) {
      head_step[r] = w.found;
      head_read[r] = w.read ? 1 : 0;
      if (ctl.read_flag && w.read && online) ctl.read_flag[b] = (unsigned char)ctl.layer;
    }
  } else {
  {
    if (!fusedq) {
      if (tid < d) q_s[tid] = to_f32(qm[(long)slot * D + h * d + tid]) * rsqrtf((float)d);
      __syncthreads();
    }
    for (int j = tid; j < P; j += 256) {
      int f0, f1;
      pooled_frames(j, len, ratio, pool_last, f0, f1);
      float en = 0.f;
      if (Kpool && !pool_last && f1 - f0 == ratio && j < P_cap) {
        const float* kp = Kpool + ((long)r * P_cap + j) * d;
        for (int c = 0; c < d; c += 4) {
          const float4 v = *reinterpret_cast<const float4*>(kp + c);
          en = fmaf(v.x, q_s[c], en); en = fmaf(v.y, q_s[c + 1], en); en = fmaf(v.z, q_s[c + 2], en); en = fmaf(v.w, q_s[c + 3], en);
        }
      } else
      for (int c = 0; c < d; c += W) {
        float accv[W];
#pragma unroll
        for (int i = 0; i < W; ++i) accv[i] = 0.f;
        for (int f = f0; f < f1; ++f) {
          float kv[W];
          VL<T>::cvt(*reinterpret_cast<const uint4*>(Km + hb + (long)f * d + c), kv);
#pragma unroll
          for (int i = 0; i < W; ++i) accv[i] += kv[i];
        }
#pragma unroll
        for (int i = 0; i < W; ++i) en = fmaf(accv[i] / (float)(f1 - f0), q_s[c + i], en);
      }
      pp[j] = 1.0f / (1.0f + expf(-(en + energy_bias)));
      if (ctl.p_probe && j < ctl.probe_P) ctl.p_probe[((long)(ctl.layer - 1) * gridDim.y * H + r) * ctl.probe_P + j] = pp[j];
    }
  }
  __syncthreads();
  for (int s = tid; s < S_cap; s += 256) {
    const int j = policy::pooled_index_at(s, len, ratio, P);
    pl[s] = j >= 0 ? pp[j] : 0.f;
  }
  __syncthreads();
  if (tid < 64) {
    int found = policy::first_step(pl, S_cap, len, mass_pres, hs, lane);
    if (ctl.step_probe && lane == 0) ctl.step_probe[(long)(ctl.layer - 1) * gridDim.y * H + r] = found;
    if (ctl.step_force) { const long f = ctl.step_force[(long)(ctl.layer - 1) * gridDim.y * H + r]; if (f >= 0) found = (int)f; }
    if (lane == 0) {
      const bool hr = policy::head_read_of(found, len, mass_pres, policy::p_at_clamp(pl, found, len));
      head_step[r] = found;
      head_read[r] = hr ? 1 : 0;
      if (ctl.read_flag && hr && online) ctl.read_flag[b] = (unsigned char)ctl.layer;
      s_found = found;
    }
  }
  __syncthreads();
    st = s_found;
  }
  float o = 0.f;
  if (!soft) {
    const long row = policy::hard_row(st, len, mass_pres);
    if (row >= 0 && tid < d) o = to_f32(Vh[row * d + tid]);
  } else {
    const int n = policy::attended_keys(st, len, full);
    if (n > 0) {
      const float* qfused = fusedq ? (Wqs ? qsoft_s : q_s) : nullptr;
      if (fast) {
        if constexpr (NP > 0) o = attn::finish3<T, NP>(rg2, n, n_pref, rsqrtf((float)d), red, nullptr, qfused);
      } else {
        __syncthreads();
        if (!fusedq) {
          if (tid < d) q_s[tid] = to_f32(qs[(long)slot * D + h * d + tid]) * rsqrtf((float)d);
          __syncthreads();
        }
        o = attn::looped<T>(fusedq ? qfused : q_s, Kh, d, Vh, d, n, d, -1, nullptr, nullptr, sc, red, nullptr);
      }
    }
  }
  if (tid < d) ctx[(long)slot * D + h * d + tid] = from_f32<T>(o);
}

constexpr int KB_KEYS = SL_CROSS_KEY_BLOCK;
template <typename T, int NP>
__global__ __launch_bounds__(256, NP >= 16 ? 2 : 4) void waitk_cross_attn_block_kernel(
    const T* __restrict__ qs, const T* __restrict__ Ks, const T* __restrict__ Vc, const int* __restrict__ key_len,
    const int* __restrict__ tgt_idx, long* __restrict__ head_step, unsigned char* __restrict__ head_read,
    float* __restrict__ part, int H, int d, int S_cap, int ratio, int waitk_k, int online, int mass_pres, int n_hint,
    StreamCtl ctl, int full) {
  if (row_skipped(ctl, blockIdx.y)) return;
  if (ctl.online) online = ctl.online[blockIdx.y];
  __shared__ float red[attn::RED_FLOATS];
  const int h = blockIdx.x, b = blockIdx.y, kb = blockIdx.z, nblk = gridDim.z, tid = threadIdx.x;
  const int D = H * d;
  const int len = key_len ? key_len[b] : S_cap;
  const int r = b * H + h;
  const bool pool_last = ratio < 0;
  ratio = ratio < 0 ? -ratio : ratio;
  const int P = pooled_count(len, ratio, true, pool_last);
  const long hb = ((long)b * H + h) * S_cap * d;
  const int tg = full ? 0 : tgt_idx[b];
  const long hs = full ? 0 : head_step[r];
  if (n_hint < 0) n_hint = (tg + waitk_k) * ratio;
  if (full) n_hint = len;
  const int j0 = kb * KB_KEYS;
  const int n_pref = max(0, min(min(S_cap, n_hint) - j0, KB_KEYS));
  attn::Regs2<T, NP> rg2;
  if (n_pref > 0)
    attn::prefetch2<T, NP>(rg2, qs + (long)b * D + h * d, Ks + hb + (long)j0 * d, d, Vc + hb + (long)j0 * d, d, n_pref, -1, nullptr, nullptr);
  long st = len - 1;
  if (!full) {
    const policy::Step w = policy::waitk_step(tg, waitk_k, online, P, ratio, len, mass_pres, hs);
    if (kb == 0 && tid == 0) {
      head_step[r] = w.found;
      head_read[r] = w.read ? 1 : 0;
      if (ctl.read_flag && w.read && online) ctl.read_flag[b] = (unsigned char)ctl.layer;
    }
    st = w.found;
  }
  const int n = policy::attended_keys(st, len, full != 0);
  const int nb = n > 0 ? max(0, min(n - j0, KB_KEYS)) : 0;
  float* pw = part + ((long)r * nblk + kb) * (d + 2);
  if (nb <= 0 || n_pref <= 0) {
    if (tid == 0) { pw[0] = -INFINITY; pw[1] = 0.f; }
    return;
  }
  float ml[2];
  const float o = attn::finish3<T, NP>(rg2, nb, n_pref, rsqrtf((float)d), red, nullptr, nullptr, ml);
  if (tid == 0) { pw[0] = ml[0]; pw[1] = ml[1]; }
  if (tid < d) pw[2 + tid] = o;
}

template <typename T>
__global__ __launch_bounds__(64) void cross_attn_merge_kernel(const float* __restrict__ part, T* __restrict__ ctx, int H, int d,
                                                              int nblk, StreamCtl ctl) {
  const int r = blockIdx.x, b = r / H, h = r - b * H, tid = threadIdx.x;
  if (row_skipped(ctl, b)) return;
  const float* p = part + (long)r * nblk * (d + 2);
  float m = -INFINITY;
  for (int k = 0; k < nblk; ++k) m = fmaxf(m, p[k * (d + 2)]);
  float l = 0.f, o = 0.f;
  if (m != -INFINITY)
    for (int k = 0; k < nblk; ++k) {
      const float mk = p[k * (d + 2)];
      if (mk == -INFINITY) continue;
      const float w = expf(mk - m);
      l += p[k * (d + 2) + 1] * w;
      if (tid < d) o += p[k * (d + 2) + 2 + tid] * w;
    }
  if (tid < d) ctx[(long)b * H * d + h * d + tid] = from_f32<T>(l > 0.f ? o / l : 0.f);
}

template <typename T>
__global__ __launch_bounds__(256) void argmax_embed_kernel(const float* __restrict__ logits, long* __restrict__ tokens,
                                                           long* __restrict__ out_tokens, int* __restrict__ n_prev,
                                                           const T* __restrict__ E, const float* __restrict__ pos,
                                                           T* __restrict__ x, int V, int D, int pad_idx, int eos_idx,
                                                           int mask_eos, float scale, int B_, int np_base,
                                                           StreamCtl ctl, const float2* __restrict__ partial, int n_tiles) {
  __shared__ float sv[4];
  __shared__ int si[4];
  __shared__ int s_tok;
  const int slot = blockIdx.x, tid = threadIdx.x;
  int b = slot;
  if (ctl.row_map) { b = ctl.row_map[slot]; if (b < 0) return; }
  const float* row = logits + (long)slot * V;
  const int np = n_prev[b];
  const bool streaming = ctl.active != nullptr;
  const bool no_eos = !streaming && (mask_eos || np == 0);
  float best = -INFINITY;
  int bi = 0x7fffffff;
  if (partial) {
    for (int t = tid; t < n_tiles; t += 256) {
      const float2 pr = partial[(long)slot * n_tiles + t];
      const int c = __float_as_int(pr.y);
      if (pr.x > best || (pr.x == best && c < bi)) { best = pr.x; bi = c; }
    }
  } else
  if ((V & 3) == 0) {
    for (int c4 = tid; c4 < (V >> 2); c4 += 256) {
      const float4 q = *reinterpret_cast<const float4*>(row + 4 * c4);
      const float vv[4] = {q.x, q.y, q.z, q.w};
#pragma unroll
      for (int e = 0; e < 4; ++e) {
        const int c = 4 * c4 + e;
        float v = vv[e];
        if ((!streaming && c == pad_idx) || (no_eos && c == eos_idx)) v = -INFINITY;
        if (v > best || (v == best && c < bi)) { best = v; bi = c; }
      }
    }
  } else
  for (int c = tid; c < V; c += 256) {
    float v = row[c];
    if ((!streaming && c == pad_idx) || (no_eos && c == eos_idx)) v = -INFINITY;
    if (v > best || (v == best && c < bi)) { best = v; bi = c; }
  }
#pragma unroll
  for (int o = 32; o > 0; o >>= 1) {
    float ov = __shfl_xor(best, o, 64);
    int oi = __shfl_xor(bi, o, 64);
    if (ov > best || (ov == best && oi < bi)) { best = ov; bi = oi; }
  }
  if ((tid & 63) == 0) { sv[tid >> 6] = best; si[tid >> 6] = bi; }
  __syncthreads();
  if (tid == 0) {
    for (int w = 1; w < 4; ++w)
      if (sv[w] > best || (sv[w] == best && si[w] < bi)) { best = sv[w]; bi = si[w]; }
    if (bi == 0x7fffffff) bi = 0;
    if (streaming) {
      const bool act = ctl.active[b] != 0, rd = ctl.read_flag[b] != 0;
      int tok_next = (int)tokens[b], np_next = np;
      const int ci = ctl.sched_rows ? ctl.chunk_idx[b] : 0;
      const long sb = (long)b * ctl.n_chunks;
      const int nc = ctl.row_chunks ? ctl.row_chunks[b] : ctl.n_chunks;
      const int cur_ms = ctl.sched_rows ? ctl.sched_ms[sb + ci] : ctl.cur_ms;
      const int max_len_now = ctl.sched_rows ? ctl.sched_max_len[sb + ci] : ctl.max_len_now;
      int c_now = ci;
      bool live = act;
      if (act && !rd) {
        if (np < ctl.cap) {
          ctl.hyp[(long)b * ctl.cap + np] = bi;
          if (ctl.delays) ctl.delays[(long)b * ctl.cap + np] = cur_ms;
          if (ctl.tok_chunk) ctl.tok_chunk[(long)b * ctl.cap + np] = ci;
        }
        tok_next = bi; np_next = np + 1;
        tokens[b] = bi;
        n_prev[b] = np_next;
        if (bi == eos_idx || np_next > max_len_now) { ctl.done[b] = 1; ctl.active[b] = 0; live = false; }
      } else if (act && rd) {
        if (ctl.sched_rows && ci + 1 < nc) {
          c_now = ci + 1;
        } else {
          ctl.active[b] = 0;
          live = false;
        }
      }
      if (ctl.sched_rows && live) {
        if (ctl.ff_waitk > 0) {
          const int ra = ctl.ff_ratio < 0 ? -ctl.ff_ratio : ctl.ff_ratio;
          while (c_now + 1 < nc &&
                 np_next + ctl.ff_waitk - 1 >= pooled_count(ctl.sched_rows[sb + c_now], ra, true, ctl.ff_ratio < 0)) ++c_now;
        }
        if (c_now != ci) {
          ctl.chunk_idx[b] = c_now;
          ctl.enc_len[b] = ctl.sched_rows[sb + c_now];
          ctl.online[b] = c_now + 1 < nc;
        }
      }
      ctl.read_flag[b] = 0;
      s_tok = tok_next;
      sv[0] = __int_as_float(np_next);
    } else {
    tokens[b] = bi;
    if (np_base >= 0) out_tokens[(long)(np - np_base) * B_ + b] = bi; else out_tokens[b] = bi;
    n_prev[b] = np + 1;
    s_tok = bi;
    sv[0] = __int_as_float(np + 1);
    }
  }
  if (ctl.row_map) return;
  __syncthreads();
  const long tok = s_tok;
  const long pr = pad_idx + 1 + __float_as_int(sv[0]);
  for (int c = tid; c < D; c += 256)
    x[(long)b * D + c] = from_f32<T>(scale * to_f32(E[tok * D + c]) + pos[pr * D + c]);
}

__global__ __launch_bounds__(1024) void stream_compact_kernel(const unsigned char* __restrict__ active, int B, int* __restrict__ row_map,
                                                              int cap_rows) {
  __shared__ int wsum[16];
  __shared__ int base;
  const int tid = threadIdx.x, lane = tid & 63, wave = tid >> 6;
  if (tid == 0) base = 0;
  __syncthreads();
  for (int b0 = 0; b0 < B; b0 += 1024) {
    const int b = b0 + tid;
    const bool a = b < B && active[b] != 0;
    const unsigned long long m = __ballot(a);
    const int in_wave = __popcll(m & ((1ull << lane) - 1ull));
    if (lane == 0) wsum[wave] = __popcll(m);
    __syncthreads();
    int off = base;
    for (int w = 0; w < wave; ++w) off += wsum[w];
    if (a && off + in_wave < cap_rows) row_map[off + in_wave] = b;
    __syncthreads();
    if (tid == 0) { int t = 0; for (int w = 0; w < 16; ++w) t += wsum[w]; base += t; }
    __syncthreads();
  }
  for (int i = base + tid; i < cap_rows; i += 1024) row_map[i] = -1;
}

template <typename T>
__global__ void embed_first_kernel(const long* __restrict__ tokens, const T* __restrict__ E,
                                   const float* __restrict__ pos, const int* __restrict__ n_prev, T* __restrict__ x,
                                   int D, int pad_idx, float scale, const int* __restrict__ row_map = nullptr) {
  const int slot = blockIdx.x;
  int b = slot;
  if (row_map) {
    b = row_map[slot];
    if (b < 0) {
      for (int c = threadIdx.x; c < D; c += blockDim.x) x[(long)slot * D + c] = from_f32<T>(0.f);
      return;
    }
  }
  const long tok = tokens[b];
  const long pr = pad_idx + 1 + n_prev[b];
  for (int c = threadIdx.x; c < D; c += blockDim.x)
    x[(long)slot * D + c] = from_f32<T>(scale * to_f32(E[tok * D + c]) + pos[pr * D + c]);
}

template <typename T>
int launch_policy_cross(simulst_handle* h, const void* qm, const void* qs, const void* Km, const void* Ks,
                        const void* Vc, float energy_bias, const int32_t* key_len, const int32_t* tgt_idx,
                        int64_t* head_step, uint8_t* head_read, void* ctx, int B, int H, int d, int S_cap, int ratio,
                        int attn_type, int waitk_k, int online, int mass_pres, int n_hint, const void* xres,
                        const float* ln_g, const float* ln_b, const void* Wqm, const float* bqm, const void* Wqs,
                        const float* bqs, const StreamCtl& ctl, const HeadSplit& hs, const float* kpool, int P_cap) {
  size_t lds = (size_t)(64 + attn::RED_FLOATS + (S_cap > 256 ? S_cap : 256) + 2 * S_cap + 1 + H * d + 64) * sizeof(float);
  if ((size_t)h->policy_lds_bytes > lds && B >= h->dec_chain_min_rows) lds = (size_t)h->policy_lds_bytes;
  KTimer t(h, SIMULST_K_DEC_CROSS_ATTN);
  const int np = attn::lanes_per_row<T>(d);
  if ((attn_type == SIMULST_ATTN_WAITK || attn_type == SIMULST_ATTN_FULL) && S_cap > KB_KEYS && !xres && qs && Ks && np > 0 &&
      !h->force_unfused_decode) {
    const int nblk = (S_cap + KB_KEYS - 1) / KB_KEYS;
    const size_t need = (size_t)B * H * nblk * (d + 2) * sizeof(float);
    if (h->ws_bytes < need) {
      if (h->capturing) { h->err = "simulst_policy_cross_attention: scratch too small while capturing a graph"; return SIMULST_E_ARG; }
      if (h->ws) (void)hipFree(h->ws);
      h->ws = nullptr; h->ws_bytes = 0;
      const size_t want = need < ((size_t)4 << 20) ? ((size_t)4 << 20) : need;
      hipError_t e = hipMalloc(&h->ws, want);
      if (e != hipSuccess) { h->err = "simulst_policy_cross_attention: scratch allocation failed"; return (int)e; }
      h->ws_bytes = want;
    }
    float* part = (float*)h->ws;
#define KB_LAUNCH(NP)                                                                                                  \
    hipLaunchKernelGGL((waitk_cross_attn_block_kernel<T, NP>), dim3(H, B, nblk), dim3(256), 0, h->stream, (const T*)qs,     \
                       (const T*)Ks, (const T*)Vc, key_len, tgt_idx, (long*)head_step, head_read, part, H, d, S_cap, ratio,  \
                       waitk_k, online, mass_pres, n_hint, ctl, attn_type == SIMULST_ATTN_FULL ? 1 : 0)
    switch (np) { case 2: KB_LAUNCH(2); break; case 4: KB_LAUNCH(4); break; case 8: KB_LAUNCH(8); break; default: KB_LAUNCH(16); break; }
#undef KB_LAUNCH
    int rc = sl_launch_status(h, "simulst_policy_cross_attention(blocks)");
    if (rc) return rc;
    hipLaunchKernelGGL(cross_attn_merge_kernel<T>, dim3(B * H), dim3(64), 0, h->stream, (const float*)part, (T*)ctx, H, d, nblk, ctl);
    return sl_launch_status(h, "simulst_policy_cross_attention(merge)");
  }
#define PC_LAUNCH_Q(NP, FQ)                                                                                            \
  hipLaunchKernelGGL((policy_cross_attn_kernel<T, NP, FQ>), dim3(H, B), dim3(256), lds, h->stream, (const T*)qm,       \
                     (const T*)qs, (const T*)Km, (const T*)Ks, (const T*)Vc, energy_bias, key_len, tgt_idx,            \
                     (long*)head_step, head_read, (T*)ctx, H, d, S_cap, ratio, attn_type, waitk_k, online, mass_pres,   \
                     n_hint, (const T*)xres, ln_g, ln_b, (const T*)Wqm, bqm, (const T*)Wqs, bqs, ctl, hs.po, hs.bo,     \
                     (T*)hs.x_mid, hs.w_packed, kpool, P_cap)
#define PC_LAUNCH(NP) do { if (xres) PC_LAUNCH_Q(NP, true); else PC_LAUNCH_Q(NP, false); } while (0)
  SL_DISPATCH_NP(attn::lanes_per_row<T>(d), PC_LAUNCH)
#undef PC_LAUNCH
#undef PC_LAUNCH_Q
  return sl_launch_status(h, "simulst_policy_cross_attention");
}

}

static int policy_cross(simulst_handle* h, const void* qm, const void* qs, const void* Kmono, const void* Ksoft,
                        const void* Vc, float energy_bias, const int32_t* key_len, const int32_t* tgt_idx,
                        int64_t* head_step, uint8_t* head_read, void* ctx, int32_t B, int32_t H, int32_t d,
                        int32_t S_cap, int32_t ratio, int32_t attn_type, int32_t waitk_k, int32_t online,
                        int32_t mass_preservation, int32_t dtype, int32_t n_hint, const void* xres = nullptr,
                        const float* ln_g = nullptr, const float* ln_b = nullptr, const void* Wqm = nullptr,
                        const float* bqm = nullptr, const void* Wqs = nullptr, const float* bqs = nullptr,
                        const StreamCtl* ctl = nullptr, const HeadSplit* hs = nullptr, const float* kpool = nullptr,
                        int P_cap = 0);

extern "C" int simulst_policy_cross_attention(simulst_handle* h, const void* qm, const void* qs, const void* Kmono,
                                              const void* Ksoft, const void* Vc, float energy_bias,
                                              const int32_t* key_len, const int32_t* tgt_idx, int64_t* head_step,
                                              uint8_t* head_read, void* ctx, int32_t B, int32_t H, int32_t d,
                                              int32_t S_cap, int32_t ratio, int32_t attn_type, int32_t waitk_k,
                                              int32_t online, int32_t mass_preservation, int32_t dtype) {
  return policy_cross(h, qm, qs, Kmono, Ksoft, Vc, energy_bias, key_len, tgt_idx, head_step, head_read, ctx, B, H, d,
                      S_cap, ratio, attn_type, waitk_k, online, mass_preservation, dtype, S_cap);
}

static int policy_cross(simulst_handle* h, const void* qm, const void* qs, const void* Kmono, const void* Ksoft,
                        const void* Vc, float energy_bias, const int32_t* key_len, const int32_t* tgt_idx,
                        int64_t* head_step, uint8_t* head_read, void* ctx, int32_t B, int32_t H, int32_t d,
                        int32_t S_cap, int32_t ratio, int32_t attn_type, int32_t waitk_k, int32_t online,
                        int32_t mass_preservation, int32_t dtype, int32_t n_hint, const void* xres,
                        const float* ln_g, const float* ln_b, const void* Wqm, const float* bqm, const void* Wqs,
                        const float* bqs, const StreamCtl* ctlp, const HeadSplit* hsp, const float* kpool, int P_cap) {
  if (!h) return SIMULST_E_NULL;
  StreamCtl ctl = {};
  if (ctlp) ctl = *ctlp;
  HeadSplit hs = {};
  if (hsp) {
    hs = *hsp;
    SL_REQUIRE(h, (xres || (!hs.po && !hs.w_packed)) && (!hs.po || hs.x_mid) && (!hs.w_packed || d % 16 == 0), SIMULST_E_ARG,
               "simulst_policy_cross_attention: head-split projections need the fused query path");
  }
  SL_CHECK_NULL(h, Vc); SL_CHECK_NULL(h, ctx);
  SL_REQUIRE(h, dtype == SIMULST_F32 || dtype == SIMULST_BF16, SIMULST_E_DTYPE, "simulst_policy_cross_attention: dtype");
  SL_REQUIRE(h, attn_type >= SIMULST_ATTN_HARD && attn_type <= SIMULST_ATTN_FULL, SIMULST_E_ARG,
             "simulst_policy_cross_attention: attn_type");
  if (attn_type != SIMULST_ATTN_FULL) { SL_CHECK_NULL(h, head_step); SL_CHECK_NULL(h, head_read); }
  if (attn_type == SIMULST_ATTN_WAITK) { SL_CHECK_NULL(h, tgt_idx); SL_REQUIRE(h, waitk_k > 0, SIMULST_E_ARG, "simulst_policy_cross_attention: lagging"); }
  else if (attn_type != SIMULST_ATTN_FULL) { if (!xres) SL_CHECK_NULL(h, qm); SL_CHECK_NULL(h, Kmono); }
  if (attn_type != SIMULST_ATTN_HARD) { if (!xres) SL_CHECK_NULL(h, qs); SL_CHECK_NULL(h, Ksoft); }
  if (xres) { SL_CHECK_NULL(h, ln_g); SL_CHECK_NULL(h, ln_b); SL_CHECK_NULL(h, Wqm);
              SL_REQUIRE(h, (H * d) % 32 == 0, SIMULST_E_SHAPE, "simulst_policy_cross_attention: D % 32 for the fused projection"); }
  SL_REQUIRE(h, H > 0 && d >= 8 && d <= 64 && d % 8 == 0 && S_cap > 0 && ratio != 0, SIMULST_E_SHAPE,
             "simulst_policy_cross_attention: head_dim must be a multiple of 8, <= 64");
  SL_REQUIRE(h, (size_t)(64 + attn::RED_FLOATS + (S_cap > 256 ? S_cap : 256) + 2 * S_cap + 1 + H * d + 64) * sizeof(float) <= 64 * 1024, SIMULST_E_SHAPE,
             "simulst_policy_cross_attention: source too long for the LDS rows");
  if (B <= 0) return SIMULST_OK;
  if (dtype == SIMULST_F32)
    return launch_policy_cross<float>(h, qm, qs, Kmono, Ksoft, Vc, energy_bias, key_len, tgt_idx, head_step, head_read,
                                      ctx, B, H, d, S_cap, ratio, attn_type, waitk_k, online, mass_preservation, n_hint,
                                      xres, ln_g, ln_b, Wqm, bqm, Wqs, bqs, ctl, hs, kpool, P_cap);
  return launch_policy_cross<bf16>(h, qm, qs, Kmono, Ksoft, Vc, energy_bias, key_len, tgt_idx, head_step, head_read,
                                   ctx, B, H, d, S_cap, ratio, attn_type, waitk_k, online, mass_preservation, n_hint,
                                   xres, ln_g, ln_b, Wqm, bqm, Wqs, bqs, ctl, hs, kpool, P_cap);
}


template <typename T>
__global__ void pool_keys_kernel(const T* __restrict__ Km, float* __restrict__ Kpool, const int* __restrict__ key_len, int H, int d,
                                 int S_cap, int P_cap, int ratio, int j_lo) {
  const int j = j_lo + blockIdx.x, r = blockIdx.y, b = r / H, c = threadIdx.x;
  const int len = key_len ? key_len[b] : S_cap;
  if (c >= d || j >= P_cap || (j + 1) * ratio > len) return;
  const T* k = Km + ((long)r * S_cap + (long)j * ratio) * d + c;
  float acc = 0.f;
  for (int f = 0; f < ratio; ++f) acc += to_f32(k[(long)f * d]);
  Kpool[((long)r * P_cap + j) * d + c] = acc / (float)ratio;
}

extern "C" int simulst_pool_keys(simulst_handle* h, const void* Kmono, float* Kpool, const int32_t* key_len, int32_t B, int32_t H,
                                 int32_t d, int32_t S_cap, int32_t P_cap, int32_t ratio, int32_t j_lo, int32_t j_hi, int32_t dtype) {
  if (!h) return SIMULST_E_NULL;
  SL_CHECK_NULL(h, Kmono); SL_CHECK_NULL(h, Kpool);
  SL_REQUIRE(h, dtype == SIMULST_F32 || dtype == SIMULST_BF16, SIMULST_E_DTYPE, "simulst_pool_keys: dtype");
  SL_REQUIRE(h, B >= 0 && H > 0 && d > 0 && d <= 256 && S_cap > 0 && P_cap > 0 && ratio > 0 && j_lo >= 0, SIMULST_E_SHAPE,
             "simulst_pool_keys: shape (average pooling only: ratio > 0)");
  if (j_hi > P_cap) j_hi = P_cap;
  if (B == 0 || j_hi <= j_lo) return SIMULST_OK;
  KTimer t(h, SIMULST_K_MISC);
  const dim3 grid(j_hi - j_lo, B * H), block(d <= 64 ? 64 : 256);
  if (dtype == SIMULST_F32)
    hipLaunchKernelGGL(pool_keys_kernel<float>, grid, block, 0, h->stream, (const float*)Kmono, Kpool, key_len, H, d, S_cap, P_cap, ratio, j_lo);
  else
    hipLaunchKernelGGL(pool_keys_kernel<bf16>, grid, block, 0, h->stream, (const bf16*)Kmono, Kpool, key_len, H, d, S_cap, P_cap, ratio, j_lo);
  return sl_launch_status(h, "simulst_pool_keys");
}

static int run_decode(simulst_handle* h, const simulst_decoder_desc* dd, const simulst_dec_layer* layers,
                      int64_t* tokens_io, int64_t* out_tokens, int32_t n_steps, int32_t mask_eos, bool do_embed,
                      bool device_indexed, const StreamCtl* ctlp = nullptr);

static uint64_t fnv(uint64_t hsh, const void* p, size_t n) {
  const unsigned char* c = (const unsigned char*)p;
  for (size_t i = 0; i < n; ++i) { hsh ^= c[i]; hsh *= 1099511628211ull; }
  return hsh;
}

extern "C" int simulst_mma_decode(simulst_handle* h, const simulst_decoder_desc* dd, const simulst_dec_layer* layers,
                                  int64_t* tokens_io, int64_t* out_tokens, int32_t n_steps, int32_t mask_eos) {
  if (!h) return SIMULST_E_NULL;
  SL_CHECK_NULL(h, dd); SL_CHECK_NULL(h, layers);
  bool timers = false;
  for (int i = 0; i < SIMULST_K_COUNT; ++i) timers |= h->timer_on[i];
  if (!h->graph_on || timers || h->stream == nullptr || n_steps <= 0 || dd->n_prev_uniform < 0)
    return run_decode(h, dd, layers, tokens_io, out_tokens, n_steps, mask_eos, true, false);
  uint64_t key = 1469598103934665603ull;
  key = fnv(key, dd, sizeof(*dd));
  key = fnv(key, layers, sizeof(simulst_dec_layer) * dd->n_layers);
  key = fnv(key, &tokens_io, sizeof(tokens_io));
  key = fnv(key, &out_tokens, sizeof(out_tokens));
  key = fnv(key, &mask_eos, sizeof(mask_eos));
  int rc0 = run_decode(h, dd, layers, tokens_io, out_tokens, 0, mask_eos, true, true);
  if (rc0 != SIMULST_OK) return rc0;
  if (!h->graph_exec || h->graph_key != key) {
    if (h->graph_exec) { (void)hipGraphExecDestroy(h->graph_exec); h->graph_exec = nullptr; }
    hipError_t e = hipStreamBeginCapture(h->stream, hipStreamCaptureModeThreadLocal);
    if (e != hipSuccess) { h->err = std::string("simulst_mma_decode: begin capture: ") + hipGetErrorString(e); return (int)e; }
    h->capturing = true;
    int rc = run_decode(h, dd, layers, tokens_io, out_tokens, 1, mask_eos, false, true);
    h->capturing = false;
    hipGraph_t g = nullptr;
    e = hipStreamEndCapture(h->stream, &g);
    if (rc != SIMULST_OK) { if (g) (void)hipGraphDestroy(g); return rc; }
    if (e != hipSuccess) { h->err = std::string("simulst_mma_decode: end capture: ") + hipGetErrorString(e); return (int)e; }
    e = hipGraphInstantiate(&h->graph_exec, g, nullptr, nullptr, 0);
    (void)hipGraphDestroy(g);
    if (e != hipSuccess) { h->graph_exec = nullptr; h->err = std::string("simulst_mma_decode: instantiate: ") + hipGetErrorString(e); return (int)e; }
    h->graph_key = key;
  }
  for (int s = 0; s < n_steps; ++s) {
    hipError_t e = hipGraphLaunch(h->graph_exec, h->stream);
    if (e != hipSuccess) { h->err = std::string("simulst_mma_decode: graph launch: ") + hipGetErrorString(e); return (int)e; }
  }
  return SIMULST_OK;
}

struct DecodeCall {
  simulst_handle* h;
  const simulst_decoder_desc* dd;
  const simulst_dec_layer* layers;
  int64_t* tokens_io;
  int64_t* out_tokens;
  sl_decode_call in;
  sl_decode_plan plan;
  sl_step_bufs bufs;
  StreamCtl ctl;
  int np_base, mask_eos;
};

static int launch_embed(const DecodeCall& c, const int* row_map) {
  const simulst_decoder_desc* dd = c.dd;
  if (dd->dtype == SIMULST_F32)
    hipLaunchKernelGGL(embed_first_kernel<float>, dim3(c.in.B), dim3(256), 0, c.h->stream, (const long*)c.tokens_io, (const float*)dd->E,
                       dd->pos_table, dd->n_prev, (float*)dd->x, dd->D, dd->pad_idx, dd->embed_scale, row_map);
  else
    hipLaunchKernelGGL(embed_first_kernel<bf16>, dim3(c.in.B), dim3(256), 0, c.h->stream, (const long*)c.tokens_io, (const bf16*)dd->E,
                       dd->pos_table, dd->n_prev, (bf16*)dd->x, dd->D, dd->pad_idx, dd->embed_scale, row_map);
  return sl_launch_status(c.h, row_map ? "simulst_mma_stream_steps(compaction + embedding)" : "simulst_mma_decode(embed)");
}

static int self_attention_block(const DecodeCall& c, int s, int l, HeadSplit& hs, const void*& xin) {
  simulst_handle* h = c.h;
  const simulst_decoder_desc* dd = c.dd;
  const simulst_dec_layer& L = c.layers[l];
  const int B = c.in.B, D = dd->D, H = dd->H, d = D / H, dt = dd->dtype, np = c.in.np_uniform < 0 ? -1 : c.in.np_uniform + s;
  int rc;
  if (c.plan.split) {
    rc = sl_self_attention_fused(h, dd->x, L.ln1_g, L.ln1_b, L.wqkv, L.bqkv, L.wo, L.k_cache, L.v_cache, dd->n_prev, np,
                                 dd->partial_self, B, H, d, dd->cap, dt);
    hs.po = dd->partial_self; hs.bo = L.bo; hs.x_mid = dd->x_mid;
    xin = dd->x_mid;
    return rc;
  }
  if (l == 0 && s > 0 && c.plan.fuse_commit)
    rc = sl_dec_embed_qkv_chain(h, (const float2*)dd->logits, c.plan.n_pairs, c.tokens_io, c.out_tokens + (long)(s - 1) * B, dd->n_prev,
                                c.in.np_uniform + s - 1, dd->E, dd->pos_table, dd->embed_scale, dd->pad_idx, dd->x, L.ln1_g, L.ln1_b,
                                L.wqkv, L.bqkv, dd->qkv, B);
  else
    rc = sl_step_qkv(h, c.plan, c.bufs, l, l > 0 ? c.layers[l - 1].b2 : nullptr, sl_qkv_of(L));
  if (rc) return rc;
  if (!c.plan.attn_chain)
    if ((rc = sl_self_attention(h, dd->qkv, L.k_cache, L.v_cache, dd->n_prev, np, dd->ctx, B, H, d, dd->cap, dt,
                                c.in.compact ? c.ctl.row_map : nullptr))) return rc;
  if (!c.plan.chain)
    return sl_lin(h, dt, B, D, D, dd->ctx, L.wo, L.bo, dd->x, dd->x, SIMULST_EPI_BIAS_RES, nullptr, nullptr, c.bufs.packed);
  return SIMULST_OK;
}

static int cross_attention_block(DecodeCall& c, int s, int l, const HeadSplit& hs) {
  simulst_handle* h = c.h;
  const simulst_decoder_desc* dd = c.dd;
  const simulst_dec_layer& L = c.layers[l];
  const int B = c.in.B, D = dd->D, H = dd->H, d = D / H, dt = dd->dtype, pk = c.bufs.packed;
  const int n_hint = c.in.mode != SL_CALL_OFFLINE ? -1
                     : (dd->attn_type == SIMULST_ATTN_WAITK && c.in.np_uniform >= 0)
                           ? (c.in.np_uniform + s + dd->waitk_k) * (dd->ratio < 0 ? -dd->ratio : dd->ratio) : dd->S_cap;
  const StreamCtl* ctlp = c.in.mode == SL_CALL_STREAM ? &c.ctl : nullptr;
  const void* Ks = L.Ksoft ? L.Ksoft : L.Kmono;
  int rc;
  c.ctl.layer = l + 1;
  if (c.plan.fuse_q)
    return policy_cross(h, nullptr, nullptr, L.Kmono, Ks, L.V, L.energy_bias, dd->enc_len, dd->n_prev, L.head_step, L.head_read, dd->ctx,
                        B, H, d, dd->S_cap, dd->ratio, dd->attn_type, dd->waitk_k, dd->online, dd->mass_preservation, dt, n_hint, dd->x,
                        L.ln2_g, L.ln2_b, L.c_wq, L.c_bq, L.c_wq_soft, L.c_bq_soft, ctlp, &hs, L.Kpool, dd->P_cap);
  if (c.plan.attn_chain) {
    rc = sl_dec_attn_proj_chain(h, dd->qkv, L.k_cache, L.v_cache, dd->n_prev, c.in.np_uniform < 0 ? -1 : c.in.np_uniform + s, dd->cap, dd->x,
                                L.wo, L.bo, L.ln2_g, L.ln2_b, L.c_wq, L.c_bq, dd->q, L.c_wq_soft, L.c_bq_soft, dd->q2, B);
  } else if (c.plan.proj_cross && !L.c_wq_soft) {
    return sl_dec_proj_cross_fused(h, dd->ctx, dd->x, L.wo, L.bo, L.ln2_g, L.ln2_b, L.c_wq, L.c_bq, dd->q, Ks, L.V, dd->enc_len,
                                   dd->n_prev, L.head_step, L.head_read, dd->ctx, B, H, dd->S_cap, dd->ratio, dd->waitk_k, dd->online,
                                   dd->mass_preservation, n_hint);
  } else if (c.plan.chain) {
    rc = sl_dec_proj_chain(h, dd->ctx, dd->x, L.wo, L.bo, L.ln2_g, L.ln2_b, L.c_wq, L.c_bq, dd->q, L.c_wq_soft, L.c_bq_soft, dd->q2, B);
  } else {
    rc = sl_lin(h, dt, B, D, D, dd->x, L.c_wq, L.c_bq, nullptr, dd->q, SIMULST_EPI_BIAS, L.ln2_g, L.ln2_b, pk);
    if (!rc && L.c_wq_soft)
      rc = sl_lin(h, dt, B, D, D, dd->x, L.c_wq_soft, L.c_bq_soft, nullptr, dd->q2, SIMULST_EPI_BIAS, L.ln2_g, L.ln2_b, pk);
  }
  if (rc) return rc;
  return policy_cross(h, dd->q, L.c_wq_soft ? dd->q2 : dd->q, L.Kmono, Ks, L.V, L.energy_bias, dd->enc_len, dd->n_prev, L.head_step,
                      L.head_read, dd->ctx, B, H, d, dd->S_cap, dd->ratio, dd->attn_type, dd->waitk_k, dd->online, dd->mass_preservation,
                      dt, n_hint, nullptr, nullptr, nullptr, nullptr, nullptr, nullptr, nullptr, ctlp, nullptr, L.Kpool, dd->P_cap);
}

static int close_step(const DecodeCall& c, int s, int n_steps) {
  simulst_handle* h = c.h;
  const simulst_decoder_desc* dd = c.dd;
  const int B = c.in.B, D = dd->D, V = dd->V, dt = dd->dtype;
  const float* last_b2 = c.layers[dd->n_layers - 1].b2;
  const bool stream = c.in.mode == SL_CALL_STREAM;
  const int skip_pad = stream ? -1 : dd->pad_idx;
  const bool no_eos = !stream && (c.mask_eos || (c.in.np_uniform >= 0 && c.in.np_uniform + s == 0));
  int rc;
  if ((rc = sl_step_last_slabs(h, c.plan, c.bufs, last_b2))) return rc;
  if (c.plan.vsplit)
    rc = sl_dec_vocab_chain(h, dd->x_mid, dd->x, dd->ffn_partial, last_b2, dd->ln_g, dd->ln_b, dd->out_proj, (float2*)dd->logits, B,
                            dd->F, V, c.plan.vsplit, skip_pad, no_eos ? dd->eos_idx : -1);
  else if (c.plan.tile_argmax)
    rc = sl_launch_vocab_argmax(h, dd->x, dd->out_proj, dd->ln_g, dd->ln_b, (float2*)dd->logits, B, V, D, skip_pad,
                                no_eos ? dd->eos_idx : -1);
  else
    rc = sl_lin(h, dt, B, V, D, dd->x, dd->out_proj, nullptr, nullptr, dd->logits, SIMULST_EPI_BIAS_F32OUT, dd->ln_g, dd->ln_b,
                c.bufs.packed);
  if (rc) return rc;
  if (c.plan.fuse_commit && s + 1 < n_steps) return SIMULST_OK;
  const float2* part = c.plan.n_pairs ? (const float2*)dd->logits : nullptr;
  const int n_part = c.plan.vsplit ? c.plan.vsplit : V / 64;
  long* out_row = (long*)c.out_tokens + (c.in.mode != SL_CALL_OFFLINE ? 0 : (long)s * B);
  KTimer t(h, SIMULST_K_ARGMAX);
  if (dt == SIMULST_F32)
    hipLaunchKernelGGL(argmax_embed_kernel<float>, dim3(B), dim3(256), 0, h->stream, dd->logits, (long*)c.tokens_io, out_row, dd->n_prev,
                       (const float*)dd->E, dd->pos_table, (float*)dd->x, V, D, dd->pad_idx, dd->eos_idx, c.mask_eos, dd->embed_scale, B,
                       c.np_base, c.ctl, part, n_part);
  else
    hipLaunchKernelGGL(argmax_embed_kernel<bf16>, dim3(B), dim3(256), 0, h->stream, dd->logits, (long*)c.tokens_io, out_row, dd->n_prev,
                       (const bf16*)dd->E, dd->pos_table, (bf16*)dd->x, V, D, dd->pad_idx, dd->eos_idx, c.mask_eos, dd->embed_scale, B,
                       c.np_base, c.ctl, part, n_part);
  return sl_launch_status(h, "simulst_mma_decode(argmax)");
}

static int run_decode(simulst_handle* h, const simulst_decoder_desc* dd, const simulst_dec_layer* layers,
                      int64_t* tokens_io, int64_t* out_tokens, int32_t n_steps, int32_t mask_eos, bool do_embed,
                      bool device_indexed, const StreamCtl* ctlp) {
  StreamCtl ctl = {};
  if (ctlp) ctl = *ctlp;
  const int np_uniform = (dd && !device_indexed) ? dd->n_prev_uniform : -1;
  const int np_base = device_indexed ? dd->n_prev_uniform : -1;
  if (!h) return SIMULST_E_NULL;
  SL_CHECK_NULL(h, dd); SL_CHECK_NULL(h, layers); SL_CHECK_NULL(h, tokens_io);
  if (!ctlp) SL_CHECK_NULL(h, out_tokens);
  SL_CHECK_NULL(h, dd->E); SL_CHECK_NULL(h, dd->out_proj); SL_CHECK_NULL(h, dd->pos_table);
  SL_CHECK_NULL(h, dd->n_prev); SL_CHECK_NULL(h, dd->enc_len);
  SL_CHECK_NULL(h, dd->x); SL_CHECK_NULL(h, dd->qkv); SL_CHECK_NULL(h, dd->ctx); SL_CHECK_NULL(h, dd->q);
  SL_CHECK_NULL(h, dd->q2); SL_CHECK_NULL(h, dd->hidden); SL_CHECK_NULL(h, dd->logits);
  SL_REQUIRE(h, dd->dtype == SIMULST_F32 || dd->dtype == SIMULST_BF16, SIMULST_E_DTYPE, "simulst_mma_decode: dtype");
  SL_REQUIRE(h, dd->B > 0 && dd->D > 0 && dd->H > 0 && dd->D % dd->H == 0 && dd->n_layers > 0 && n_steps >= 0,
             SIMULST_E_SHAPE, "simulst_mma_decode: shape");
  const bool compact = ctlp && ctl.row_map != nullptr;
  const int B_streams = dd->B;
  const int B = compact ? ctl.compact_rows : dd->B, D = dd->D, H = dd->H, F = dd->F, V = dd->V, d = D / H, dt = dd->dtype;
  int rc;
  if (compact) {
    SL_REQUIRE(h, ctl.compact_rows > h->fuse_q_max_rows && ctl.compact_rows <= B_streams, SIMULST_E_ARG,
               "simulst_mma_stream_steps: compact_rows must exceed the fused-query row limit (128) and not the number of streams");
    SL_REQUIRE(h, !(dd->attn_type == SIMULST_ATTN_WAITK && dd->S_cap > KB_KEYS), SIMULST_E_ARG,
               "simulst_mma_stream_steps: active-row compaction covers sources of up to 256 encoder rows");
    SL_REQUIRE(h, !ctl.p_probe && !ctl.step_probe && !ctl.step_force, SIMULST_E_ARG, "simulst_mma_stream_steps: the audit hooks index by stream");
    do_embed = false;
  }
  const int pk = dd->weights_fragment_major;
  SL_REQUIRE(h, !pk || (D % 64 == 0 && F % 64 == 0 && V % 16 == 0 && d % 16 == 0), SIMULST_E_SHAPE,
             "simulst_mma_decode: fragment-major weights need D, F multiples of 64, V and head_dim of 16");
  sl_decode_call call = {};
  call.dtype = dt; call.B = B; call.D = D; call.H = H; call.F = F; call.V = V; call.cap = dd->cap; call.S_cap = dd->S_cap;
  call.attn_type = dd->attn_type; call.packed = pk != 0;
  call.x_mid = dd->x_mid != nullptr; call.partial_self = dd->partial_self != nullptr; call.ffn_partial = dd->ffn_partial != nullptr;
  call.final_ln = dd->ln_g != nullptr && dd->ln_b != nullptr;
  call.mode = ctlp ? SL_CALL_STREAM : device_indexed ? SL_CALL_GRAPH_STEP : SL_CALL_OFFLINE;
  call.np_uniform = np_uniform; call.compact = compact; call.mask_eos = mask_eos != 0; call.force_unfused = h->force_unfused_decode;
  DecodeCall c = {h, dd, layers, tokens_io, out_tokens, call, sl_plan_decode(h, call),
                  {dt, B, D, F, pk, dd->x, dd->x_mid, dd->qkv, dd->hidden, dd->ffn_partial, dd->ffn_sem}, ctl, np_base, mask_eos};
  if (do_embed) {
    KTimer t(h, SIMULST_K_MISC);
    if ((rc = launch_embed(c, nullptr))) return rc;
  }
  for (int s = 0; s < n_steps; ++s) {
    if (compact) {
      KTimer t(h, SIMULST_K_MISC);
      hipLaunchKernelGGL(stream_compact_kernel, dim3(1), dim3(1024), 0, h->stream, ctl.active, B_streams, (int*)ctl.row_map, B);
      if ((rc = launch_embed(c, ctl.row_map))) return rc;
    }
    for (int l = 0; l < dd->n_layers; ++l) {
      const void* xin = dd->x;
      HeadSplit hs = {nullptr, nullptr, nullptr, pk};
      if ((rc = self_attention_block(c, s, l, hs, xin))) return rc;
      if ((rc = cross_attention_block(c, s, l, hs))) return rc;
      if ((rc = sl_step_ffn(h, c.plan, c.bufs, dd->ctx, xin, sl_ffn_of(layers[l]),
                            l + 1 < dd->n_layers ? sl_qkv_of(layers[l + 1]) : sl_qkv_weights{}))) return rc;
    }
    if ((rc = close_step(c, s, n_steps))) return rc;
  }
  return SIMULST_OK;
}

extern "C" int simulst_mma_stream_steps(simulst_handle* h, const simulst_decoder_desc* dd, const simulst_dec_layer* layers,
                                        int64_t* tokens_io, const simulst_stream_ctl* c, int32_t n_iter) {
  if (!h) return SIMULST_E_NULL;
  SL_REQUIRE(h, !dd || dd->attn_type != SIMULST_ATTN_FULL, SIMULST_E_ARG,
             "simulst_mma_stream_steps: full attention is not a simultaneous policy (offline decoding only)");
  SL_CHECK_NULL(h, c); SL_CHECK_NULL(h, c->active); SL_CHECK_NULL(h, c->read_flag); SL_CHECK_NULL(h, c->online);
  SL_CHECK_NULL(h, c->done); SL_CHECK_NULL(h, c->hyp);
  SL_REQUIRE(h, c->cap > 0 && n_iter >= 0, SIMULST_E_SHAPE, "simulst_mma_stream_steps: cap / n_iter");
  StreamCtl ctl;
  ctl.active = c->active; ctl.read_flag = c->read_flag; ctl.online = c->online; ctl.done = c->done;
  ctl.delays = c->delays_ms; ctl.hyp = (long*)c->hyp; ctl.cap = c->cap; ctl.cur_ms = c->cur_ms;
  ctl.max_len_now = c->max_len_now;
  ctl.sched_rows = c->sched_rows; ctl.sched_ms = c->sched_ms; ctl.sched_max_len = c->sched_max_len;
  ctl.chunk_idx = c->chunk_idx; ctl.enc_len = c->enc_len; ctl.tok_chunk = c->tok_chunk; ctl.n_chunks = c->n_chunks;
  ctl.row_chunks = c->row_chunks;
  ctl.ff_waitk = c->sched_rows ? c->ff_waitk : 0; ctl.ff_ratio = c->ff_ratio;
  ctl.p_probe = c->p_probe; ctl.step_probe = (long*)c->step_probe; ctl.step_force = (const long*)c->step_force; ctl.probe_P = c->probe_P;
  ctl.row_map = c->compact_rows > 0 ? c->row_map : nullptr; ctl.compact_rows = c->compact_rows;
  SL_REQUIRE(h, c->compact_rows <= 0 || c->row_map, SIMULST_E_NULL, "simulst_mma_stream_steps: compact_rows needs the row_map scratch");
  SL_REQUIRE(h, !c->p_probe || c->probe_P > 0, SIMULST_E_SHAPE, "simulst_mma_stream_steps: p_probe needs probe_P");
  if (c->sched_rows) {
    SL_REQUIRE(h, c->ff_waitk == 0 || (dd && dd->attn_type == SIMULST_ATTN_WAITK && c->ff_waitk == dd->waitk_k && c->ff_ratio == dd->ratio),
               SIMULST_E_ARG, "simulst_mma_stream_steps: ff_waitk / ff_ratio must be the descriptor's wait-k lagging and ratio");
    SL_CHECK_NULL(h, c->sched_ms); SL_CHECK_NULL(h, c->sched_max_len); SL_CHECK_NULL(h, c->chunk_idx); SL_CHECK_NULL(h, c->enc_len);
    SL_REQUIRE(h, c->n_chunks > 0, SIMULST_E_SHAPE, "simulst_mma_stream_steps: n_chunks");
    SL_REQUIRE(h, dd && c->enc_len == dd->enc_len, SIMULST_E_SHAPE, "simulst_mma_stream_steps: ctl.enc_len must be the descriptor's enc_len");
  }
  return run_decode(h, dd, layers, tokens_io, nullptr, n_iter, 0, true, true, &ctl);
}
```

simulst_amd/csrc/decode_plan.cpp:

```cpp
#include "decode_plan.h"
#include "gemm_plan.h"

#ifdef SL_EXPERIMENTS
static constexpr bool HEAD_SPLIT_BUILT = true;
#else
static constexpr bool HEAD_SPLIT_BUILT = false;
#endif

static bool rows_fuse_q(const simulst_handle* h, int B) { return B <= h->fuse_q_max_rows; }
static bool rows_chain_ffn(const simulst_handle* h, int B) { return B <= h->dec_chain_ffn_max_rows; }

bool sl_dec_tall_fc2_shape_ok(const simulst_handle* h, int dtype, int B, int N, int K, bool packed) {
  if (dtype != SIMULST_BF16 || !packed || B <= 0 || N <= 0 || K <= 0) return false;
  LinArgs p = {};
  p.M = B; p.rpb = B; p.N = N; p.K = K;
  p.a_rs = K; p.c_rs = N; p.r_rs = N;
  p.scale = 1.f; p.w_packed = 1; p.amax_skip_a = p.amax_skip_b = -1;
  const sl_linear_ops o = {};
  const sl_linear_plan pl = sl_plan_linear(h, dtype, SIMULST_EPI_BIAS_RES, p, o);
  return pl.family == SL_LIN_SKINNY && pl.splits == 1;
}
bool sl_dec_tall_fc1_shape_ok(const simulst_handle* h, int dtype, int B, int N, int K, bool packed) {
  if (dtype != SIMULST_BF16 || !packed || B <= 0 || N <= 0 || K <= 0 || K > 256) return false;
  LinArgs p = {};
  p.M = B; p.rpb = B; p.N = N; p.K = K;
  p.a_rs = K; p.c_rs = N; p.r_rs = N;
  p.scale = 1.f; p.w_packed = 1; p.amax_skip_a = p.amax_skip_b = -1;
  p.ln_g = p.ln_b = (const float*)h;
  const sl_linear_ops o = {};
  const sl_linear_plan pl = sl_plan_linear(h, dtype, SIMULST_EPI_BIAS_GELU, p, o);
  return pl.family == SL_LIN_PANEL_SPLIT;
}
bool sl_dec_tall_fc1_ok(const simulst_handle* h, int dtype, int B, int D, int F, bool packed) {
  return h->dec_tall_ffn && B >= h->dec_tall_min_rows && sl_dec_tall_fc1_shape_ok(h, dtype, B, F, D, packed);
}
bool sl_dec_tall_fc2_ok(const simulst_handle* h, int dtype, int B, int D, int F, bool packed) {
  return h->dec_tall_ffn && B >= h->dec_tall_min_rows && sl_dec_tall_fc2_shape_ok(h, dtype, B, D, F, packed);
}

sl_decode_plan sl_plan_decode(const simulst_handle* h, const sl_decode_call& c) {
  sl_decode_plan p = {};
  const int d = c.D / c.H;
  const bool lockstep = c.mode == SL_CALL_OFFLINE && c.np_uniform >= 0;
  const bool own_rows = !c.compact;
  p.full_blocked = c.attn_type == SIMULST_ATTN_FULL && c.S_cap > SL_CROSS_KEY_BLOCK && !c.force_unfused;
  p.split = HEAD_SPLIT_BUILT && own_rows && !c.cif && !p.full_blocked && c.packed && c.x_mid && c.partial_self && !c.force_unfused &&
            sl_self_attention_fused_ok(c.H, d, c.cap) && c.B <= 128 && (c.dtype == SIMULST_BF16 ? c.D <= 512 : c.D <= 256);
  p.fuse_q = !c.cif && (p.split || rows_fuse_q(h, c.B)) && !p.full_blocked;
  p.chain = !p.split && !p.fuse_q && !c.force_unfused && c.ffn_partial && !(c.cif && !c.x_mid) &&
            sl_dec_chain_ok(h, c.dtype, c.B, c.D, c.F, c.packed);
  p.chain_ffn = p.chain && rows_chain_ffn(h, c.B) && c.x_mid;
  p.attn_chain = own_rows && p.chain && sl_dec_attn_chain_ok(h, c.dtype, c.B, c.H, d, c.cap);
  p.proj_cross = own_rows && !c.cif && p.chain && !p.attn_chain &&
                 sl_dec_proj_cross_fused_ok(h, c.dtype, c.B, c.H, d, c.S_cap, c.attn_type, lockstep, false);
  p.fuse_ffn_qkv = p.chain_ffn && !p.attn_chain && sl_dec_ffn_qkv_chain_ok(h, c.B, c.F);
  p.tall_ffn = !p.chain_ffn && !c.force_unfused && sl_dec_tall_fc2_ok(h, c.dtype, c.B, c.D, c.F, c.packed);
  p.tall_fc1 = !p.chain_ffn && !c.force_unfused && sl_dec_tall_fc1_ok(h, c.dtype, c.B, c.D, c.F, c.packed);
  const bool masks_known = c.mode == SL_CALL_STREAM || c.mask_eos || lockstep;
  p.vsplit = (p.chain_ffn && masks_known && h->fused_argmax && !c.highway)
                 ? sl_dec_vocab_chain_split(h, c.dtype, c.B, c.V, c.D, c.packed, c.final_ln) : 0;
  p.tile_argmax = !p.vsplit && !c.cif && masks_known && sl_vocab_argmax_ok(h, c.dtype, c.B, c.V, c.D, c.packed);
  p.n_pairs = p.vsplit ? p.vsplit : p.tile_argmax ? c.V / 64 : 0;
  p.fuse_commit = !c.cif && p.chain_ffn && lockstep && h->dec_embed_qkv_chain && p.n_pairs > 0 && p.n_pairs <= 64;
  return p;
}

int sl_retire_floor_rows(const simulst_handle* h, int B) {
  int f = 1;
  if (!rows_chain_ffn(h, B)) f = h->dec_chain_ffn_max_rows + 1;
  else if (B >= h->dec_chain_min_rows) f = h->dec_chain_min_rows;
  else if (!rows_fuse_q(h, B)) f = h->fuse_q_max_rows + 1;
  for (int t : {TILE_MIN_ROWS, h->mid_narrow_min_rows, h->panel_split_min_rows})
    if (B >= t && f < t) f = t;
  if (B > SKINNY_MAX_ROWS_PACKED) f = B;
  return min((f + 15) / 16 * 16, B);
}

int sl_lin(simulst_handle* h, int dtype, int B, int N, int K, const void* A, const void* W, const float* bias, const void* R,
           void* C, int epi, const float* ln_g, const float* ln_b, int w_packed) {
  simulst_linear_desc d;
  d.M_batches = 1; d.rows_per_batch = B; d.N = N; d.K = K;
  d.a_batch_stride = 0; d.a_row_stride = K; d.a_lead = 0;
  d.c_batch_stride = 0; d.c_row_stride = N;
  d.r_batch_stride = 0; d.r_row_stride = N;
  d.epilogue = epi; d.dtype = dtype; d.scale = 1.f; d.n_main = 0; d.aux_rows = 0; d.aux_batch_stride = 0;
  d.ln_gamma = ln_g; d.ln_beta = ln_b; d.w_fragment_major = w_packed; d.c_head_dim = 0; d.c_head_stride = 0; d.c_tensor_heads = 0; d.c_tensor_stride = 0;
  return simulst_linear(h, &d, A, W, bias, R, C, nullptr);
}

int sl_step_qkv(simulst_handle* h, const sl_decode_plan& p, const sl_step_bufs& w, int l, const float* prev_b2, const sl_qkv_weights& q) {
  if (l > 0 && p.fuse_ffn_qkv) return SIMULST_OK;
  if (l > 0 && p.chain_ffn)
    return sl_dec_qkv_chain(h, w.x_mid, w.x, w.ffn_partial, prev_b2, q.ln_g, q.ln_b, q.w, q.b, w.qkv, w.B, w.F);
  return sl_lin(h, w.dtype, w.B, 3 * w.D, w.D, w.x, q.w, q.b, nullptr, w.qkv, SIMULST_EPI_BIAS, q.ln_g, q.ln_b, w.packed);
}

int sl_step_ffn(simulst_handle* h, const sl_decode_plan& p, const sl_step_bufs& w, const void* ctx, const void* res,
                const sl_ffn_weights& f, const sl_qkv_weights& next) {
  if (p.chain_ffn && p.fuse_ffn_qkv && next.w)
    return sl_dec_ffn_qkv_chain(h, ctx, w.x, f.c_wo, f.c_bo, f.ln_g, f.ln_b, f.fc1, f.b1, f.fc2, f.b2, w.ffn_partial, w.B, w.F,
                                next.ln_g, next.ln_b, next.w, next.b, w.qkv);
  if (p.chain_ffn)
    return sl_dec_ffn_chain(h, ctx, w.x, f.c_wo, f.c_bo, f.ln_g, f.ln_b, f.fc1, f.b1, f.fc2, f.b2, w.ffn_partial, w.ffn_sem, w.x_mid,
                            w.B, w.F);
  int rc;
  if ((rc = sl_lin(h, w.dtype, w.B, w.D, w.D, ctx, f.c_wo, f.c_bo, res, w.x, SIMULST_EPI_BIAS_RES, nullptr, nullptr, w.packed))) return rc;
  if (p.tall_fc1 && f.ln_g && f.ln_b && sl_dec_tall_operands_ok(w.x, f.fc1, w.hidden, f.b1))
    rc = sl_dec_tall_fc1(h, w.x, f.fc1, f.b1, f.ln_g, f.ln_b, w.hidden, w.B, w.F, w.D);
  else
    rc = sl_lin(h, w.dtype, w.B, w.F, w.D, w.x, f.fc1, f.b1, nullptr, w.hidden, SIMULST_EPI_BIAS_GELU, f.ln_g, f.ln_b, w.packed);
  if (rc) return rc;
  if (p.tall_ffn && sl_dec_tall_operands_ok(w.hidden, f.fc2, w.x, w.x))
    return sl_dec_tall_fc2(h, w.hidden, f.fc2, f.b2, w.x, w.x, w.B, w.D, w.F);
  return sl_lin(h, w.dtype, w.B, w.D, w.F, w.hidden, f.fc2, f.b2, w.x, w.x, SIMULST_EPI_BIAS_RES, nullptr, nullptr, w.packed);
}

int sl_step_last_slabs(simulst_handle* h, const sl_decode_plan& p, const sl_step_bufs& w, const float* last_b2) {
  if (!p.chain_ffn || p.vsplit) return SIMULST_OK;
  return sl_dec_qkv_chain(h, w.x_mid, w.x, w.ffn_partial, last_b2, nullptr, nullptr, nullptr, nullptr, nullptr, w.B, w.F);
}
```

simulst_amd/csrc/decode_plan.h:

```cpp
#pragma once
#include "common.h"

constexpr int SL_CROSS_KEY_BLOCK = 256;

enum { SL_CALL_OFFLINE = 0,
       SL_CALL_GRAPH_STEP = 1,
       SL_CALL_STREAM = 2 };

struct sl_decode_call {
  int dtype, B, D, H, F, V, cap, S_cap, attn_type;
  bool packed;
  bool x_mid, partial_self, ffn_partial, final_ln;
  int mode;
  int np_uniform;
  bool compact, mask_eos;
  bool force_unfused;
  bool cif;
  bool highway;
};

struct sl_decode_plan {
  bool full_blocked;
  bool split;
  bool fuse_q;
  bool chain;
  bool chain_ffn;
  bool attn_chain;
  bool proj_cross;
  bool fuse_commit;
  bool fuse_ffn_qkv;
  bool tall_ffn;
  bool tall_fc1;
  int vsplit;
  bool tile_argmax;
  int n_pairs;
};

sl_decode_plan sl_plan_decode(const simulst_handle* h, const sl_decode_call& c);

int sl_retire_floor_rows(const simulst_handle* h, int B);

struct sl_step_bufs {
  int dtype, B, D, F, packed;
  void *x, *x_mid, *qkv, *hidden;
  float* ffn_partial;
  int32_t* ffn_sem;
};
struct sl_qkv_weights { const float *ln_g, *ln_b; const void* w; const float* b; };
struct sl_ffn_weights { const void* c_wo; const float* c_bo; const float *ln_g, *ln_b; const void* fc1; const float* b1; const void* fc2; const float* b2; };
template <typename Layer> sl_qkv_weights sl_qkv_of(const Layer& L) { return {L.ln1_g, L.ln1_b, L.wqkv, L.bqkv}; }
template <typename Layer> sl_ffn_weights sl_ffn_of(const Layer& L) { return {L.c_wo, L.c_bo, L.ln3_g, L.ln3_b, L.fc1, L.b1, L.fc2, L.b2}; }

int sl_lin(simulst_handle* h, int dtype, int B, int N, int K, const void* A, const void* W, const float* bias, const void* R,
           void* C, int epi, const float* ln_g, const float* ln_b, int w_packed);
bool sl_dec_tall_fc2_shape_ok(const simulst_handle* h, int dtype, int B, int N, int K, bool packed);
bool sl_dec_tall_fc2_ok(const simulst_handle* h, int dtype, int B, int D, int F, bool packed);
static inline bool sl_dec_tall_operands_ok(const void* A, const void* W, const void* R, const void* C) {
  return (((uintptr_t)A | (uintptr_t)W | (uintptr_t)R | (uintptr_t)C) & 15) == 0;
}
int sl_dec_tall_fc2(simulst_handle* h, const void* A, const void* W, const float* bias, const void* R, void* C, int B, int N, int K);
bool sl_dec_tall_fc1_shape_ok(const simulst_handle* h, int dtype, int B, int N, int K, bool packed);
bool sl_dec_tall_fc1_ok(const simulst_handle* h, int dtype, int B, int D, int F, bool packed);
int sl_dec_tall_fc1(simulst_handle* h, const void* A, const void* W, const float* bias, const float* ln_g, const float* ln_b, void* C,
                    int B, int N, int K);
int sl_step_qkv(simulst_handle* h, const sl_decode_plan& p, const sl_step_bufs& w, int l, const float* prev_b2, const sl_qkv_weights& q);
int sl_step_ffn(simulst_handle* h, const sl_decode_plan& p, const sl_step_bufs& w, const void* ctx, const void* res,
                const sl_ffn_weights& f, const sl_qkv_weights& next);
int sl_step_last_slabs(simulst_handle* h, const sl_decode_plan& p, const sl_step_bufs& w, const float* last_b2);
```

simulst_amd/csrc/handle.cpp:

```cpp
#include "common.h"
#include <cstdlib>

extern "C" int simulst_version(void) { return 108; }

extern "C" int simulst_create(simulst_handle** out, void* hip_stream) {
  if (!out) return SIMULST_E_NULL;
  simulst_handle* h = new (std::nothrow) simulst_handle();
  if (!h) return SIMULST_E_ARG;
  h->stream = (hipStream_t)hip_stream;
  h->ev_used = 0;
  h->ws = nullptr;
  h->ws_bytes = 0;
  h->graph_on = false;
  h->capturing = false;
  h->force_valu_attention = false;
  h->force_unfused_decode = false;
  h->panel_split_min_rows = 2560;
  if (const char* e = getenv("SIMULST_PANEL_SPLIT_MIN_ROWS")) h->panel_split_min_rows = atoi(e);
  h->panel_split_blocks = 256;
  if (const char* e = getenv("SIMULST_PANEL_SPLIT_BLOCKS")) h->panel_split_blocks = atoi(e);
  h->mid_min_blocks = 48;
  if (const char* e = getenv("SIMULST_MID_MIN_BLOCKS")) h->mid_min_blocks = atoi(e);
  h->mid_narrow_min_rows = 3072;
  if (const char* e = getenv("SIMULST_MID_NARROW_MIN_ROWS")) h->mid_narrow_min_rows = atoi(e);
  h->skinny_min_blocks_tall = 192;
  if (const char* e = getenv("SIMULST_SKINNY_MIN_BLOCKS_TALL")) h->skinny_min_blocks_tall = atoi(e);
  h->fuse_q_max_rows = 128;
  if (const char* e = getenv("SIMULST_FUSE_Q_MAX_ROWS")) h->fuse_q_max_rows = atoi(e);
  h->dec_chain_on = true;
  if (const char* e = getenv("SIMULST_DEC_CHAIN")) h->dec_chain_on = atoi(e) != 0;
  h->dec_chain_min_rows = 129;
  if (const char* e = getenv("SIMULST_DEC_CHAIN_MIN_ROWS")) h->dec_chain_min_rows = atoi(e);
  h->dec_chain_max_rows = 1 << 30;
  if (const char* e = getenv("SIMULST_DEC_CHAIN_MAX_ROWS")) h->dec_chain_max_rows = atoi(e);
  h->dec_chain_ffn_max_rows = 1024;
  if (const char* e = getenv("SIMULST_DEC_CHAIN_FFN_MAX_ROWS")) h->dec_chain_ffn_max_rows = atoi(e);
  h->dec_tall_ffn = true;
  if (const char* e = getenv("SIMULST_DEC_TALL_FFN")) h->dec_tall_ffn = atoi(e) != 0;
  h->dec_tall_min_rows = h->dec_chain_ffn_max_rows + 1;
  if (const char* e = getenv("SIMULST_DEC_TALL_MIN_ROWS")) h->dec_tall_min_rows = atoi(e);
  h->dec_chain_lds_attr_set = false;
  h->dec_chain_probe_attr_set = false;
  h->dec_chain_lds_bytes = 0;
  h->dec_chain_xmode = 3;
  h->dec_chain_tail = nullptr;
#ifdef SL_DEBUG_HOOKS
  if (const char* e = getenv("SIMULST_DEC_CHAIN_XMODE")) { const int v = atoi(e); if (v >= 0 && v <= 3) h->dec_chain_xmode = v; }
  if (const char* e = getenv("SIMULST_DEC_CHAIN_LDS_BYTES")) { const int v = atoi(e); if (v >= 0 && v <= 160 * 1024) h->dec_chain_lds_bytes = v; }
#endif
  h->dec_attn_chain_max_rows = 0;
#ifdef SL_EXPERIMENTS
  if (const char* e = getenv("SIMULST_DEC_ATTN_CHAIN_MAX_ROWS")) h->dec_attn_chain_max_rows = atoi(e);
#endif
  h->dec_attn_chain_rows = 0;
  h->dec_vocab_chain_split = 4;
  if (const char* e = getenv("SIMULST_DEC_VOCAB_CHAIN_SPLIT")) { const int v = atoi(e); if (v == 0 || v == 1 || v == 2 || v == 4 || v == 8 || v == 16) h->dec_vocab_chain_split = v; }
  h->dec_embed_qkv_chain = true;
  if (const char* e = getenv("SIMULST_DEC_EMBED_QKV_CHAIN")) h->dec_embed_qkv_chain = atoi(e) != 0;
  h->dec_chain_rows32 = false;
  h->dec_chain_rows32_min = 256;
#ifdef SL_EXPERIMENTS
  if (const char* e = getenv("SIMULST_DEC_CHAIN_ROWS32")) h->dec_chain_rows32 = atoi(e) != 0;
  if (const char* e = getenv("SIMULST_DEC_CHAIN_ROWS32_MIN")) h->dec_chain_rows32_min = atoi(e);
#endif
  h->dec_fuse_ffn_qkv = false;
#ifdef SL_EXPERIMENTS
  if (const char* e = getenv("SIMULST_DEC_FUSE_FFN_QKV")) h->dec_fuse_ffn_qkv = atoi(e) != 0;
#endif
  h->chain_sem = nullptr;
  h->chain_sem_splits = 0;
  h->tile256 = 2;
  if (const char* e = getenv("SIMULST_CONV_TILE256")) { const int v = atoi(e); if (v >= 0 && v <= 2) h->tile256 = v; }
  h->tile256_lds_attr_set = false;
  h->tile256_ring_attr_set = false;
  h->wstat = true;
  if (const char* e = getenv("SIMULST_WEIGHT_STATIONARY")) h->wstat = atoi(e) != 0;
  h->wstat_lds_attr_set = false;
  {
    int dev = 0, n = 0;
    if (hipGetDevice(&dev) != hipSuccess || hipDeviceGetAttribute(&n, hipDeviceAttributeMultiprocessorCount, dev) != hipSuccess || n < 8) n = 0;
    h->n_cus = n;
  }
  h->panel_wide = true;
  h->panel_wide_plain_stores = false;
  if (const char* e = getenv("SIMULST_PANEL_WIDE")) {
    h->panel_wide = atoi(e) != 0;
#ifdef SL_EXPERIMENTS
    h->panel_wide_plain_stores = atoi(e) == 2;
#endif
  }
  h->policy_lds_bytes = 0;
  if (const char* e = getenv("SIMULST_POLICY_LDS_BYTES")) { const int v = atoi(e); if (v >= 0 && v <= 64 * 1024) h->policy_lds_bytes = v; }
  h->fused_argmax = true;
  if (const char* e = getenv("SIMULST_FUSED_ARGMAX")) h->fused_argmax = atoi(e) != 0;
#ifdef SL_EXPERIMENTS
  if (const char* e = getenv("SIMULST_DEC_ATTN_CHAIN_ROWS")) { const int v = atoi(e); if (v == 4 || v == 8 || v == 16) h->dec_attn_chain_rows = v; }
#endif
  h->dec_fuse_proj_cross = false;
#ifdef SL_EXPERIMENTS
  if (const char* e = getenv("SIMULST_DEC_FUSE_PROJ_CROSS")) h->dec_fuse_proj_cross = atoi(e) != 0;
#endif
  h->fuse_flags = nullptr;
  h->fuse_epoch = 0;
  h->graph_exec = nullptr;
  h->ctc_lds_attr_set = false;
  h->conv_pos_lds_attr_set = false;
  h->ffn_lds_attr_set = false;
  h->ffn_pipe_lds_attr_set = false;
  h->qkv_rows_lds_attr_set = false;
  h->ffn_variant = 0;
  h->ffn_waves = 0;
  h->ea_general_only = false;
  if (const char* e = getenv("SIMULST_EA_GENERAL")) h->ea_general_only = atoi(e) != 0;
  h->graph_key = 0;
  for (int i = 0; i < SIMULST_K_COUNT; ++i) { h->timer_on[i] = false; h->timer_ms[i] = 0.0; h->timer_n[i] = 0; }
  *out = h;
  return SIMULST_OK;
}

extern "C" int simulst_destroy(simulst_handle* h) {
  if (!h) return SIMULST_E_NULL;
  for (auto& p : h->ev_pool) { (void)hipEventDestroy(p.a); (void)hipEventDestroy(p.b); }
  if (h->ws) (void)hipFree(h->ws);
  if (h->fuse_flags) (void)hipFree(h->fuse_flags);
  if (h->chain_sem) (void)hipFree(h->chain_sem);
  if (h->graph_exec) (void)hipGraphExecDestroy(h->graph_exec);
  delete h;
  return SIMULST_OK;
}

extern "C" int simulst_set_stream(simulst_handle* h, void* hip_stream) {
  if (!h) return SIMULST_E_NULL;
  h->stream = (hipStream_t)hip_stream;
  return SIMULST_OK;
}

extern "C" const char* simulst_last_error(simulst_handle* h) { return h ? h->err.c_str() : "null handle"; }

extern "C" int simulst_timer_enable(simulst_handle* h, int cls, int on) {
  if (!h) return SIMULST_E_NULL;
  if (cls < 0) { for (int i = 0; i < SIMULST_K_COUNT; ++i) h->timer_on[i] = on != 0; return SIMULST_OK; }
  SL_REQUIRE(h, cls < SIMULST_K_COUNT, SIMULST_E_ARG, "simulst_timer_enable: kernel class");
  h->timer_on[cls] = on != 0;
  return SIMULST_OK;
}

#include <algorithm>
static void resolve_events(simulst_handle* h) {
  if (h->ev_used == 0) return;
  (void)hipStreamSynchronize(h->stream);
  for (int i = 0; i < h->ev_used; ++i) {
    float ms = 0.f;
    hipEvent_t from = i == 0 ? h->ev_pool[0].a : h->ev_pool[i - 1].b;
    if (hipEventElapsedTime(&ms, from, h->ev_pool[i].b) == hipSuccess) {
      h->timer_ms[h->ev_pool[i].cls] += ms;
      h->timer_n[h->ev_pool[i].cls] += 1;
    }
  }
  h->ev_used = 0;
}

extern "C" int simulst_timer_read(simulst_handle* h, int cls, double* total_ms, int64_t* launches) {
  if (!h) return SIMULST_E_NULL;
  SL_REQUIRE(h, cls >= 0 && cls < SIMULST_K_COUNT, SIMULST_E_ARG, "simulst_timer_read: kernel class");
  resolve_events(h);
  if (total_ms) *total_ms = h->timer_ms[cls];
  if (launches) *launches = h->timer_n[cls];
  return SIMULST_OK;
}

extern "C" int simulst_timer_reset(simulst_handle* h) {
  if (!h) return SIMULST_E_NULL;
  resolve_events(h);
  for (int i = 0; i < SIMULST_K_COUNT; ++i) { h->timer_ms[i] = 0.0; h->timer_n[i] = 0; }
  return SIMULST_OK;
}

extern "C" int simulst_graph_enable(simulst_handle* h, int on) {
  if (!h) return SIMULST_E_NULL;
  h->graph_on = on != 0;
  if (!h->graph_on && h->graph_exec) { (void)hipGraphExecDestroy(h->graph_exec); h->graph_exec = nullptr; h->graph_key = 0; }
  if (h->graph_on && h->ws_bytes < (size_t)(16u << 20)) {
    if (h->ws) (void)hipFree(h->ws);
    h->ws = nullptr; h->ws_bytes = 0;
    hipError_t e = hipMalloc(&h->ws, (size_t)(16u << 20));
    if (e != hipSuccess) { h->err = "simulst_graph_enable: scratch allocation failed"; return (int)e; }
    h->ws_bytes = (size_t)(16u << 20);
  }
  return SIMULST_OK;
}

extern "C" int simulst_set_option(simulst_handle* h, int32_t option, int32_t value) {
  if (!h) return SIMULST_E_NULL;
  switch (option) {
    case SIMULST_OPT_VALU_ATTENTION: h->force_valu_attention = value != 0; return SIMULST_OK;
    case SIMULST_OPT_UNFUSED_DECODE: h->force_unfused_decode = value != 0; return SIMULST_OK;
    case SIMULST_OPT_FFN_WAVES:
#ifdef SL_EXPERIMENTS
      SL_REQUIRE(h, value == 0 || value == 4 || value == 8 || value == 41 || value == 43 || value == 45 || value == 47 || value == 81 || value == 83 || value == 87
#ifdef SL_DEBUG_HOOKS
                        || value == 42 || value == 82
#endif
                 , SIMULST_E_ARG,
                 "simulst_set_option(FFN_WAVES): 0 (the library's choice), 4 / 8 (GELU as a block between the products), 41 / 81 (GELU inside the "
                 "MFMA stream, 4 / 8 waves; 42 / 82: packed GELU, DEBUG_HOOKS builds only), 43 / 83 (GELU spread over all 32 MFMAs), 45 (64 rows per wave)");
#else
      SL_REQUIRE(h, value == 0 || value == 4 || value == 8 || value == 43, SIMULST_E_ARG,
                 "simulst_set_option(FFN_WAVES): 0 (the library's choice: 43 while F <= 2048), 43 (GELU inside the MFMA stream), 4 / 8 (the block form "
                 "with that many waves: GELU between the two products); the measured-slower forms exist in EXPERIMENTS builds");
#endif
      h->ffn_waves = value; return SIMULST_OK;
    case SIMULST_OPT_DEC_CHAIN: h->dec_chain_on = value != 0; return SIMULST_OK;
#ifdef SL_EXPERIMENTS
    case SIMULST_OPT_DEC_ATTN_CHAIN_MAX_ROWS:
      SL_REQUIRE(h, value >= 0, SIMULST_E_ARG, "simulst_set_option(DEC_ATTN_CHAIN_MAX_ROWS): >= 0");
      h->dec_attn_chain_max_rows = value; return SIMULST_OK;
    case SIMULST_OPT_DEC_ATTN_CHAIN_ROWS:
      SL_REQUIRE(h, value == 0 || value == 4 || value == 8 || value == 16, SIMULST_E_ARG, "simulst_set_option(DEC_ATTN_CHAIN_ROWS): 0, 4, 8 or 16");
      h->dec_attn_chain_rows = value; return SIMULST_OK;
#else
    case SIMULST_OPT_DEC_ATTN_CHAIN_MAX_ROWS:
    case SIMULST_OPT_DEC_ATTN_CHAIN_ROWS:
      h->err = "simulst_set_option: self-attention inside the projection chain exists in EXPERIMENTS builds only (measured slower)";
      return SIMULST_E_ARG;
#endif
    case SIMULST_OPT_FUSED_ARGMAX: h->fused_argmax = value != 0; return SIMULST_OK;
    case SIMULST_OPT_DEC_EMBED_QKV_CHAIN: h->dec_embed_qkv_chain = value != 0; return SIMULST_OK;
    case SIMULST_OPT_WEIGHT_STATIONARY: h->wstat = value != 0; return SIMULST_OK;
    case SIMULST_OPT_DEC_TALL_FFN: h->dec_tall_ffn = value != 0; return SIMULST_OK;
    case SIMULST_OPT_CONV_TILE256:
      SL_REQUIRE(h, value >= 0 && value <= 2, SIMULST_E_ARG, "simulst_set_option(CONV_TILE256): 0 (128 x 128 tiles), 1 (256 x 256, register stage), 2 (256 x 256, LDS-DMA ring)");
      h->tile256 = value; return SIMULST_OK;
    case SIMULST_OPT_DEC_CHAIN_ROWS32:
#ifdef SL_EXPERIMENTS
      h->dec_chain_rows32 = value != 0; return SIMULST_OK;
#else
      h->err = "simulst_set_option: the layer chains on 32-row tiles exist in EXPERIMENTS builds only (measured slower)";
      return SIMULST_E_ARG;
#endif
    case SIMULST_OPT_DEC_FUSE_FFN_QKV:
#ifdef SL_EXPERIMENTS
      h->dec_fuse_ffn_qkv = value != 0; return SIMULST_OK;
#else
      h->err = "simulst_set_option: the feed-forward chain + next layer's QKV in one launch exists in EXPERIMENTS builds only (measured slower)";
      return SIMULST_E_ARG;
#endif
    case SIMULST_OPT_PANEL_WIDE:
#ifdef SL_EXPERIMENTS
      SL_REQUIRE(h, value >= 0 && value <= 2, SIMULST_E_ARG, "simulst_set_option(PANEL_WIDE): 0, 1, 2 (plain stores)");
#else
      SL_REQUIRE(h, value == 0 || value == 1, SIMULST_E_ARG, "simulst_set_option(PANEL_WIDE): 0 or 1 (2, plain stores: EXPERIMENTS builds)");
#endif
      h->panel_wide = value != 0; h->panel_wide_plain_stores = value == 2; return SIMULST_OK;
    case SIMULST_OPT_DEC_FUSE_PROJ_CROSS:
#ifdef SL_EXPERIMENTS
      h->dec_fuse_proj_cross = value != 0; return SIMULST_OK;
#else
      h->err = "simulst_set_option: the one-launch projection chain + cross-attention exists in EXPERIMENTS builds only (measured slower)";
      return SIMULST_E_ARG;
#endif
    case SIMULST_OPT_DEC_VOCAB_CHAIN_SPLIT:
      SL_REQUIRE(h, value == 0 || value == 1 || value == 2 || value == 4 || value == 8 || value == 16, SIMULST_E_ARG,
                 "simulst_set_option(DEC_VOCAB_CHAIN_SPLIT): 0 (off), 1, 2, 4, 8 or 16");
      h->dec_vocab_chain_split = value; return SIMULST_OK;
    default: break;
  }
  h->err = "simulst_set_option: unknown option";
  return SIMULST_E_ARG;
}

extern "C" int simulst_get_option(simulst_handle* h, int32_t option, int32_t* value) {
  if (!h) return SIMULST_E_NULL;
  SL_CHECK_NULL(h, value);
  switch (option) {
    case SIMULST_OPT_VALU_ATTENTION: *value = h->force_valu_attention; return SIMULST_OK;
    case SIMULST_OPT_UNFUSED_DECODE: *value = h->force_unfused_decode; return SIMULST_OK;
    case SIMULST_OPT_FFN_WAVES: *value = h->ffn_waves; return SIMULST_OK;
    case SIMULST_OPT_DEC_CHAIN: *value = h->dec_chain_on; return SIMULST_OK;
    case SIMULST_OPT_DEC_ATTN_CHAIN_MAX_ROWS: *value = h->dec_attn_chain_max_rows; return SIMULST_OK;
    case SIMULST_OPT_DEC_ATTN_CHAIN_ROWS: *value = h->dec_attn_chain_rows; return SIMULST_OK;
    case SIMULST_OPT_FUSED_ARGMAX: *value = h->fused_argmax; return SIMULST_OK;
    case SIMULST_OPT_DEC_EMBED_QKV_CHAIN: *value = h->dec_embed_qkv_chain; return SIMULST_OK;
    case SIMULST_OPT_PANEL_WIDE: *value = h->panel_wide ? (h->panel_wide_plain_stores ? 2 : 1) : 0; return SIMULST_OK;
    case SIMULST_OPT_DEC_VOCAB_CHAIN_SPLIT: *value = h->dec_vocab_chain_split; return SIMULST_OK;
    case SIMULST_OPT_WEIGHT_STATIONARY: *value = h->wstat; return SIMULST_OK;
    case SIMULST_OPT_DEC_TALL_FFN: *value = h->dec_tall_ffn; return SIMULST_OK;
    case SIMULST_OPT_CONV_TILE256: *value = h->tile256; return SIMULST_OK;
    case SIMULST_OPT_DEC_FUSE_FFN_QKV: *value = h->dec_fuse_ffn_qkv; return SIMULST_OK;
    case SIMULST_OPT_DEC_CHAIN_ROWS32: *value = h->dec_chain_rows32; return SIMULST_OK;
    case SIMULST_OPT_DEC_FUSE_PROJ_CROSS: {
      int err = 0;
      if (h->fuse_flags) {
        (void)hipStreamSynchronize(h->stream);
        (void)hipMemcpy(&err, h->fuse_flags + 1023, sizeof(int), hipMemcpyDeviceToHost);
      }
      *value = (h->dec_fuse_proj_cross ? 1 : 0) | (err ? 2 : 0);
      return SIMULST_OK;
    }
    default: break;
  }
  h->err = "simulst_get_option: unknown option";
  return SIMULST_E_ARG;
}

extern "C" int simulst_stream_create(void** out_stream, int32_t priority, const uint32_t* cu_mask, int32_t mask_words) {
  if (!out_stream) return SIMULST_E_NULL;
  hipStream_t s = nullptr;
  hipError_t e;
  if (cu_mask && mask_words > 0) {
    e = hipExtStreamCreateWithCUMask(&s, (uint32_t)mask_words, cu_mask);
  } else if (priority != 0) {
    int least = 0, greatest = 0;
    e = hipDeviceGetStreamPriorityRange(&least, &greatest);
    if (e == hipSuccess) e = hipStreamCreateWithPriority(&s, hipStreamNonBlocking, priority > 0 ? greatest : least);
  } else {
    e = hipStreamCreateWithFlags(&s, hipStreamNonBlocking);
  }
  if (e != hipSuccess) return (int)e;
  *out_stream = (void*)s;
  return SIMULST_OK;
}

extern "C" int simulst_stream_destroy(void* stream) {
  if (!stream) return SIMULST_E_NULL;
  hipError_t e = hipStreamDestroy((hipStream_t)stream);
  return e == hipSuccess ? SIMULST_OK : (int)e;
}

extern "C" int simulst_has_experiments(void) {
#ifdef SL_EXPERIMENTS
  return 1;
#else
  return 0;
#endif
}
```

Measured before the change: 1.900 million tokens/s.

## Generalize tall LN-fused K256 panel kernel to QKV and vocab argmax in decode

Turns the tall fc1 panel kernel into a template with three epilogues: bias+GELU, plain bias for the LayerNorm+QKV projection, and per-tile max/argmax pairs for the vocabulary projection with greedy pick. The number of column steps per workgroup becomes tunable and defaults to 4 for fc1 (previously 2), with bias staged in shared memory. The weight load/store pattern is reorganised per wave, and the last step is peeled so it skips the prefetch. The decode plan routes QKV and vocab through the new kernel when the row count is large enough, replacing the generic linear path. The aim is to cut launch and tile overhead on these skinny-K decode GEMMs, at the cost of extra code paths and some risk in the argmax tie handling.

```diff
diff --git a/include/simulst_hip.h b/include/simulst_hip.h
--- a/include/simulst_hip.h
+++ b/include/simulst_hip.h
@@ -54,7 +54,7 @@
        SIMULST_OPT_DEC_ATTN_CHAIN_MAX_ROWS = 4, SIMULST_OPT_DEC_ATTN_CHAIN_ROWS = 5, SIMULST_OPT_FUSED_ARGMAX = 6,
        SIMULST_OPT_DEC_VOCAB_CHAIN_SPLIT = 7, SIMULST_OPT_DEC_EMBED_QKV_CHAIN = 8, SIMULST_OPT_PANEL_WIDE = 9,
        SIMULST_OPT_DEC_FUSE_PROJ_CROSS = 10, SIMULST_OPT_WEIGHT_STATIONARY = 11, SIMULST_OPT_CONV_TILE256 = 12, SIMULST_OPT_DEC_FUSE_FFN_QKV = 13, SIMULST_OPT_DEC_CHAIN_ROWS32 = 14,
-       SIMULST_OPT_DEC_TALL_FFN = 15 };
+       SIMULST_OPT_DEC_TALL_FFN = 15, SIMULST_OPT_DEC_TALL_K256 = 16 };
 int simulst_set_option(simulst_handle* h, int32_t option, int32_t value);
 int simulst_get_option(simulst_handle* h, int32_t option, int32_t* value);
 int simulst_has_experiments(void);
@@ -95,6 +95,10 @@
                           int32_t B, int32_t N, int32_t K, int32_t dtype);
 int simulst_dec_tall_fc1(simulst_handle* h, const void* A, const void* W, const float* bias, const float* ln_g, const float* ln_b,
                          void* C, int32_t B, int32_t N, int32_t K, int32_t dtype);
+int simulst_dec_tall_qkv(simulst_handle* h, const void* A, const void* W, const float* bias, const float* ln_g, const float* ln_b,
+                         void* C, int32_t B, int32_t N, int32_t K, int32_t dtype, int32_t steps);
+int simulst_dec_tall_vocab(simulst_handle* h, const void* x, const void* W, const float* ln_g, const float* ln_b, void* pairs,
+                           int32_t B, int32_t V, int32_t D, int32_t skip_a, int32_t skip_b, int32_t steps);
 
 int simulst_fbank(simulst_handle* h, const float* wave, int64_t wave_stride, const float* window, const float* tw_cos,
                   const float* tw_sin, const int32_t* mel_lo, const float* mel_w, void* out, int32_t B,
diff --git a/simulst_amd/_lib.py b/simulst_amd/_lib.py
--- a/simulst_amd/_lib.py
+++ b/simulst_amd/_lib.py
@@ -101,6 +101,8 @@
     "simulst_linear": [_vp, C.POINTER(LinearDesc), _vp, _vp, _vp, _vp, _vp, _vp],
     "simulst_dec_tall_gemm": [_vp, _vp, _vp, _vp, _vp, _vp, _i32, _i32, _i32, _i32],
     "simulst_dec_tall_fc1": [_vp, _vp, _vp, _vp, _vp, _vp, _vp, _i32, _i32, _i32, _i32],
+    "simulst_dec_tall_qkv": [_vp, _vp, _vp, _vp, _vp, _vp, _vp, _i32, _i32, _i32, _i32, _i32],
+    "simulst_dec_tall_vocab": [_vp, _vp, _vp, _vp, _vp, _vp, _i32, _i32, _i32, _i32, _i32, _i32],
     "simulst_conv_pos": [_vp, _vp, _vp, _vp, _vp, _vp, _vp, _i32, _i32, _i32, _i32, _i32, _i32],
     "simulst_ctc_best_alignment_scratch_bytes": [_i32, _i32, _i32],
     "simulst_ctc_best_alignment": [_vp, _vp, _i64, _i64, _i64, _vp, _i64, _vp, _vp, _i32, _i32, _i32, _i32, _i32, _vp,
@@ -182,7 +184,8 @@
 }
 (OPT_VALU_ATTENTION, OPT_UNFUSED_DECODE, OPT_FFN_WAVES, OPT_DEC_CHAIN, OPT_DEC_ATTN_CHAIN_MAX_ROWS, OPT_DEC_ATTN_CHAIN_ROWS,
  OPT_FUSED_ARGMAX, OPT_DEC_VOCAB_CHAIN_SPLIT, OPT_DEC_EMBED_QKV_CHAIN, OPT_PANEL_WIDE, OPT_DEC_FUSE_PROJ_CROSS,
- OPT_WEIGHT_STATIONARY, OPT_CONV_TILE256, OPT_DEC_FUSE_FFN_QKV, OPT_DEC_CHAIN_ROWS32, OPT_DEC_TALL_FFN) = range(16)
+ OPT_WEIGHT_STATIONARY, OPT_CONV_TILE256, OPT_DEC_FUSE_FFN_QKV, OPT_DEC_CHAIN_ROWS32, OPT_DEC_TALL_FFN,
+ OPT_DEC_TALL_K256) = range(17)
 
 _lib = None
 ABI_VERSION = 108
diff --git a/simulst_amd/csrc/common.h b/simulst_amd/csrc/common.h
--- a/simulst_amd/csrc/common.h
+++ b/simulst_amd/csrc/common.h
@@ -50,6 +50,10 @@
   int dec_chain_ffn_max_rows;
   bool dec_tall_ffn;
   int dec_tall_min_rows;
+  bool dec_tall_k256;
+  int dec_tall_fc1_steps;
+  int dec_tall_qkv_steps;
+  int dec_tall_vocab_steps;
   bool dec_chain_lds_attr_set;
   int dec_chain_lds_bytes;
   bool dec_chain_probe_attr_set;
diff --git a/simulst_amd/csrc/dec_gemm_tall.hip b/simulst_amd/csrc/dec_gemm_tall.hip
--- a/simulst_amd/csrc/dec_gemm_tall.hip
+++ b/simulst_amd/csrc/dec_gemm_tall.hip
@@ -114,13 +114,18 @@
   for (int e = 0; e < 16; e += 4) store4(cp + e, reinterpret_cast<const float(&)[4]>(y[e]));
 }
 
-constexpr int DT_F1_STEPS = 2;
+enum { DT_BIAS_GELU = 0, DT_BIAS = 1, DT_PAIRS = 2 };
+constexpr int DT_MAX_SPW = 8;
 constexpr int DT_F1_PF = 3;
 
-__global__ __launch_bounds__(256, 2) void dec_tall_fc1_kernel(const bf16* __restrict__ A, const bf16* __restrict__ Wp,
-                                                              const float* __restrict__ bias, const float* __restrict__ ln_g,
-                                                              const float* __restrict__ ln_b, bf16* __restrict__ C, int M, int N, int K) {
+template <int EPI>
+__global__ __launch_bounds__(256, 2) void dec_tall_k256_kernel(const bf16* __restrict__ A, const bf16* __restrict__ Wp,
+                                                               const float* __restrict__ bias, const float* __restrict__ ln_g,
+                                                               const float* __restrict__ ln_b, bf16* __restrict__ C,
+                                                               float2* __restrict__ amax, int M, int N, int K, int spw, int amax_tiles,
+                                                               int skip_a, int skip_b) {
   __shared__ __attribute__((aligned(16))) uint4 wl[2][4 * 8 * 64];
+  __shared__ __attribute__((aligned(16))) float lbias[DT_MAX_SPW * 64];
   float* lng = reinterpret_cast<float*>(wl[1]);
   float* lnb = lng + 256;
   const int tid = threadIdx.x, lane = tid & 63, wave = tid >> 6;
@@ -140,31 +145,28 @@
       fa[m][s] = make_uint4(ok ? v.x : 0u, ok ? v.y : 0u, ok ? v.z : 0u, ok ? v.w : 0u);
     }
   }
-  const int n_all = (N + 63) / 64;
-  const int step0 = blockIdx.y * DT_F1_STEPS, n_steps = min(n_all, step0 + DT_F1_STEPS);
+  const int n_all = (N + 63) / 64, ntiles = N >> 4;
+  const int step0 = blockIdx.y * spw, n_steps = min(n_all, step0 + spw);
   uint4 wv[8];
   auto wload = [&](int step) {
 #pragma unroll
     for (int q = 0; q < 8; ++q) {
-      const int slot = q * 256 + tid;
-      const int ln = slot & 63, s = (slot >> 6) & 7, j = slot >> 9;
-      const int ntile = step * 4 + j;
-      const bool ok = s < nks && ntile * 16 < N;
-      const uint4 v = ld16(Wp + (((long)(ok ? ntile : 0) * nks + (ok ? s : 0)) * 64 + ln) * 8);
-      wv[q] = make_uint4(ok ? v.x : 0u, ok ? v.y : 0u, ok ? v.z : 0u, ok ? v.w : 0u);
-    }
-  };
-  float4 bnext[4];
-  auto bload = [&](int step) {
-#pragma unroll
-    for (int j = 0; j < 4; ++j) {
-      const int c = step * 64 + j * 16 + 4 * lg;
-      bnext[j] = (bias && c < N) ? *reinterpret_cast<const float4*>(bias + c) : float4{0.f, 0.f, 0.f, 0.f};
+      const int s = (q * 4 + wave) & 7, ntile = step * 4 + (q >> 1);
+      const bool ok = s < nks && ntile < ntiles;
+      wv[q] = ld16(Wp + (((long)(ok ? ntile : 0) * nks + (ok ? s : 0)) * 64 + lane) * 8);
+    }
+  };
+  auto wstore = [&](int step, uint4* dst) {
+#pragma unroll
+    for (int q = 0; q < 8; ++q) {
+      const int s = (q * 4 + wave) & 7, ntile = step * 4 + (q >> 1);
+      const bool ok = s < nks && ntile < ntiles;
+      dst[q * 256 + tid] = make_uint4(ok ? wv[q].x : 0u, ok ? wv[q].y : 0u, ok ? wv[q].z : 0u, ok ? wv[q].w : 0u);
     }
   };
   wload(step0);
-  bload(step0);
   for (int k = tid; k < K; k += 256) { lng[k] = ln_g[k]; lnb[k] = ln_b[k]; }
+  for (int c = tid; c < spw * 64; c += 256) lbias[c] = (bias && step0 * 64 + c < N) ? bias[step0 * 64 + c] : 0.f;
   __syncthreads();
 #pragma unroll
   for (int m = 0; m < 2; ++m) {
@@ -179,15 +181,12 @@
     for (int s = 0; s < 8; ++s)
       if (s < nks) fa[m][s] = ln_frag_mid(fa[m][s], mean, rstd, lng, lnb, s * 32 + lg * 8, bf16());
   }
-#pragma unroll
-  for (int q = 0; q < 8; ++q) wl[0][q * 256 + tid] = wv[q];
-  for (int step = step0; step < n_steps; ++step) {
+  wstore(step0, wl[0]);
+  auto do_step = [&](int step, auto more_t) {
+    constexpr bool more = decltype(more_t)::value;
     const int cur = (step - step0) & 1;
-    float4 bcur[4];
-#pragma unroll
-    for (int j = 0; j < 4; ++j) bcur[j] = bnext[j];
-    const bool more = step + 1 < n_steps;
-    if (more) { wload(step + 1); bload(step + 1); }
+    if constexpr (more) wload(step + 1);
+    __builtin_amdgcn_sched_barrier(0);
     __syncthreads();
     f32x4 acc[2][4];
 #pragma unroll
@@ -211,30 +210,72 @@
                                                            *reinterpret_cast<const bf16x8_t*>(&fa[m][s]), acc[m][j], 0, 0, 0);
       asm volatile("" :: "v"(wfr[f % DT_F1_PF]), "v"(acc[0][j]), "v"(acc[1][j]));
     }
-    if (more) {
-#pragma unroll
-      for (int q = 0; q < 8; ++q) wl[cur ^ 1][q * 256 + tid] = wv[q];
-    }
+    __builtin_amdgcn_sched_barrier(0);
+    if constexpr (more) wstore(step + 1, wl[cur ^ 1]);
+    const float* lb = lbias + (step - step0) * 64;
+    const bool plain = EPI == DT_PAIRS && (unsigned)(skip_a - step * 64) >= 64u && (unsigned)(skip_b - step * 64) >= 64u && step * 64 + 64 <= N;
 #pragma unroll
     for (int m = 0; m < 2; ++m) {
       const int r = m0 + wave * 32 + m * 16 + lr;
+      float y[4][4];
 #pragma unroll
       for (int j = 0; j < 4; ++j) {
         const int c = step * 64 + j * 16 + 4 * lg;
-        const float4 bv = bcur[j];
+        const float4 bv = *reinterpret_cast<const float4*>(lb + j * 16 + 4 * lg);
         f32x2 v0 = f32x2{acc[m][j][0] + bv.x, acc[m][j][1] + bv.y};
         f32x2 v1 = f32x2{acc[m][j][2] + bv.z, acc[m][j][3] + bv.w};
-        v0 = gelu_fast2(v0);
-        v1 = gelu_fast2(v1);
-        const bf16 o0 = __float2bfloat16(v0.x), o1 = __float2bfloat16(v0.y), o2 = __float2bfloat16(v1.x), o3 = __float2bfloat16(v1.y);
-        const unsigned int lo = (unsigned int)(*reinterpret_cast<const unsigned short*>(&o0)) |
-                                ((unsigned int)(*reinterpret_cast<const unsigned short*>(&o1)) << 16);
-        const unsigned int hi = (unsigned int)(*reinterpret_cast<const unsigned short*>(&o2)) |
-                                ((unsigned int)(*reinterpret_cast<const unsigned short*>(&o3)) << 16);
-        if (r < M && c < N) *reinterpret_cast<uint2*>(C + (long)r * N + c) = make_uint2(lo, hi);
+        if constexpr (EPI == DT_PAIRS) {
+          y[j][0] = v0.x; y[j][1] = v0.y; y[j][2] = v1.x; y[j][3] = v1.y;
+        } else {
+          if constexpr (EPI == DT_BIAS_GELU) { v0 = gelu_fast2(v0); v1 = gelu_fast2(v1); }
+          const bf16 o0 = __float2bfloat16(v0.x), o1 = __float2bfloat16(v0.y), o2 = __float2bfloat16(v1.x), o3 = __float2bfloat16(v1.y);
+          const unsigned int lo = (unsigned int)(*reinterpret_cast<const unsigned short*>(&o0)) |
+                                  ((unsigned int)(*reinterpret_cast<const unsigned short*>(&o1)) << 16);
+          const unsigned int hi = (unsigned int)(*reinterpret_cast<const unsigned short*>(&o2)) |
+                                  ((unsigned int)(*reinterpret_cast<const unsigned short*>(&o3)) << 16);
+          if (r < M && c < N) *reinterpret_cast<uint2*>(C + (long)r * N + c) = make_uint2(lo, hi);
+        }
       }
-    }
-  }
+      if constexpr (EPI == DT_PAIRS) {
+        const int c0 = step * 64 + 4 * lg;
+        float best = -INFINITY;
+        int bi = 0x7fffffff;
+        if (plain) {
+#pragma unroll
+          for (int j = 0; j < 4; ++j)
+#pragma unroll
+            for (int e = 0; e < 4; ++e) best = fmaxf(best, y[j][e]);
+          best = fmaxf(best, __shfl_xor(best, 16, 64));
+          best = fmaxf(best, __shfl_xor(best, 32, 64));
+#pragma unroll
+          for (int j = 3; j >= 0; --j)
+#pragma unroll
+            for (int e = 3; e >= 0; --e) bi = y[j][e] == best ? c0 + j * 16 + e : bi;
+          bi = min(bi, __shfl_xor(bi, 16, 64));
+          bi = min(bi, __shfl_xor(bi, 32, 64));
+        } else {
+#pragma unroll
+          for (int j = 0; j < 4; ++j)
+#pragma unroll
+            for (int e = 0; e < 4; ++e) {
+              const int cc = c0 + j * 16 + e;
+              float v = y[j][e];
+              if (cc == skip_a || cc == skip_b || cc >= N) v = -INFINITY;
+              if (v > best || (v == best && cc < bi)) { best = v; bi = cc; }
+            }
+#pragma unroll
+          for (int o = 16; o <= 32; o <<= 1) {
+            const float ov = __shfl_xor(best, o, 64);
+            const int oi = __shfl_xor(bi, o, 64);
+            if (ov > best || (ov == best && oi < bi)) { best = ov; bi = oi; }
+          }
+        }
+        if (lg == 0 && r < M) amax[(long)r * amax_tiles + step] = make_float2(best, __int_as_float(bi));
+      }
+    }
+  };
+  for (int step = step0; step + 1 < n_steps; ++step) do_step(step, std::true_type());
+  if (step0 < n_steps) do_step(n_steps - 1, std::false_type());
 }
 
 }
@@ -246,13 +287,33 @@
   return sl_launch_status(h, "decode step: tall fc2 tile");
 }
 
+template <int EPI>
+static void launch_k256(simulst_handle* h, const void* A, const void* W, const float* bias, const float* ln_g, const float* ln_b, void* C,
+                        float2* amax, int B, int N, int K, int steps, int skip_a, int skip_b) {
+  const int n_all = (N + 63) / 64, spw = max(1, min(min(steps, DT_MAX_SPW), n_all));
+  hipLaunchKernelGGL(dec_tall_k256_kernel<EPI>, dim3((B + 127) / 128, (n_all + spw - 1) / spw), dim3(256), 0, h->stream, (const bf16*)A,
+                     (const bf16*)W, bias, ln_g, ln_b, (bf16*)C, amax, B, N, K, spw, n_all, skip_a, skip_b);
+}
+
 int sl_dec_tall_fc1(simulst_handle* h, const void* A, const void* W, const float* bias, const float* ln_g, const float* ln_b, void* C,
                     int B, int N, int K) {
   KTimer t(h, SIMULST_K_DEC_TALL_GEMM);
-  const int n_all = (N + 63) / 64;
-  hipLaunchKernelGGL(dec_tall_fc1_kernel, dim3((B + 127) / 128, (n_all + DT_F1_STEPS - 1) / DT_F1_STEPS), dim3(256), 0, h->stream,
-                     (const bf16*)A, (const bf16*)W, bias, ln_g, ln_b, (bf16*)C, B, N, K);
+  launch_k256<DT_BIAS_GELU>(h, A, W, bias, ln_g, ln_b, C, nullptr, B, N, K, h->dec_tall_fc1_steps, -1, -1);
   return sl_launch_status(h, "decode step: tall fc1 panel");
+}
+
+int sl_dec_tall_qkv(simulst_handle* h, const void* A, const void* W, const float* bias, const float* ln_g, const float* ln_b, void* C,
+                    int B, int N, int K, int steps) {
+  KTimer t(h, SIMULST_K_DEC_TALL_GEMM);
+  launch_k256<DT_BIAS>(h, A, W, bias, ln_g, ln_b, C, nullptr, B, N, K, steps > 0 ? steps : h->dec_tall_qkv_steps, -1, -1);
+  return sl_launch_status(h, "decode step: tall LN + QKV panel");
+}
+
+int sl_dec_tall_vocab(simulst_handle* h, const void* x, const void* W, const float* ln_g, const float* ln_b, float2* pairs, int B, int V,
+                      int D, int skip_a, int skip_b, int steps) {
+  KTimer t(h, SIMULST_K_DEC_TALL_GEMM);
+  launch_k256<DT_PAIRS>(h, x, W, nullptr, ln_g, ln_b, nullptr, pairs, B, V, D, steps > 0 ? steps : h->dec_tall_vocab_steps, skip_a, skip_b);
+  return sl_launch_status(h, "decode step: tall vocabulary panel");
 }
 
 extern "C" int simulst_dec_tall_fc1(simulst_handle* h, const void* A, const void* W, const float* bias, const float* ln_g,
@@ -270,6 +331,38 @@
   return sl_dec_tall_fc1(h, A, W, bias, ln_g, ln_b, C, B, N, K);
 }
 
+extern "C" int simulst_dec_tall_qkv(simulst_handle* h, const void* A, const void* W, const float* bias, const float* ln_g,
+                                    const float* ln_b, void* C, int32_t B, int32_t N, int32_t K, int32_t dtype, int32_t steps) {
+  if (!h) return SIMULST_E_NULL;
+  SL_CHECK_NULL(h, A);
+  SL_CHECK_NULL(h, W);
+  SL_CHECK_NULL(h, ln_g);
+  SL_CHECK_NULL(h, ln_b);
+  SL_CHECK_NULL(h, C);
+  SL_REQUIRE(h, B > 0 && N > 0 && K > 0, SIMULST_E_SHAPE, "simulst_dec_tall_qkv: non-positive shape");
+  SL_REQUIRE(h, steps >= 0 && steps <= DT_MAX_SPW, SIMULST_E_ARG, "simulst_dec_tall_qkv: 0 (the default) to 8 column steps per workgroup");
+  SL_REQUIRE(h, sl_dec_tall_qkv_shape_ok(h, dtype, B, N, K, true), SIMULST_E_SHAPE,
+             "simulst_dec_tall_qkv: bf16 rows whose simulst_linear launch is the split row panel");
+  SL_REQUIRE(h, sl_dec_tall_operands_ok(A, W, C, bias), SIMULST_E_ARG, "simulst_dec_tall_qkv: operands must be 16-byte aligned");
+  return sl_dec_tall_qkv(h, A, W, bias, ln_g, ln_b, C, B, N, K, steps);
+}
+
+extern "C" int simulst_dec_tall_vocab(simulst_handle* h, const void* x, const void* W, const float* ln_g, const float* ln_b, void* pairs,
+                                      int32_t B, int32_t V, int32_t D, int32_t skip_a, int32_t skip_b, int32_t steps) {
+  if (!h) return SIMULST_E_NULL;
+  SL_CHECK_NULL(h, x);
+  SL_CHECK_NULL(h, W);
+  SL_CHECK_NULL(h, ln_g);
+  SL_CHECK_NULL(h, ln_b);
+  SL_CHECK_NULL(h, pairs);
+  SL_REQUIRE(h, B > 0 && V > 0 && D > 0, SIMULST_E_SHAPE, "simulst_dec_tall_vocab: non-positive shape");
+  SL_REQUIRE(h, steps >= 0 && steps <= DT_MAX_SPW, SIMULST_E_ARG, "simulst_dec_tall_vocab: 0 (the default) to 8 column steps per workgroup");
+  SL_REQUIRE(h, sl_dec_tall_vocab_shape_ok(h, SIMULST_BF16, B, V, D, true, true), SIMULST_E_SHAPE,
+             "simulst_dec_tall_vocab: bf16 rows whose vocabulary projection with the greedy pick is the split row panel");
+  SL_REQUIRE(h, sl_dec_tall_operands_ok(x, W, pairs, nullptr), SIMULST_E_ARG, "simulst_dec_tall_vocab: operands must be 16-byte aligned");
+  return sl_dec_tall_vocab(h, x, W, ln_g, ln_b, (float2*)pairs, B, V, D, skip_a, skip_b, steps);
+}
+
 extern "C" int simulst_dec_tall_gemm(simulst_handle* h, const void* A, const void* W, const float* bias, const void* R, void* C,
                                      int32_t B, int32_t N, int32_t K, int32_t dtype) {
   if (!h) return SIMULST_E_NULL;
diff --git a/simulst_amd/csrc/decode_driver.hip b/simulst_amd/csrc/decode_driver.hip
--- a/simulst_amd/csrc/decode_driver.hip
+++ b/simulst_amd/csrc/decode_driver.hip
@@ -783,6 +783,8 @@
   if (c.plan.vsplit)
     rc = sl_dec_vocab_chain(h, dd->x_mid, dd->x, dd->ffn_partial, last_b2, dd->ln_g, dd->ln_b, dd->out_proj, (float2*)dd->logits, B,
                             dd->F, V, c.plan.vsplit, skip_pad, no_eos ? dd->eos_idx : -1);
+  else if (c.plan.tall_vocab && dd->ln_g && dd->ln_b && sl_dec_tall_operands_ok(dd->x, dd->out_proj, dd->logits, nullptr))
+    rc = sl_dec_tall_vocab(h, dd->x, dd->out_proj, dd->ln_g, dd->ln_b, (float2*)dd->logits, B, V, D, skip_pad, no_eos ? dd->eos_idx : -1, 0);
   else if (c.plan.tile_argmax)
     rc = sl_launch_vocab_argmax(h, dd->x, dd->out_proj, dd->ln_g, dd->ln_b, (float2*)dd->logits, B, V, D, skip_pad,
                                 no_eos ? dd->eos_idx : -1);
diff --git a/simulst_amd/csrc/decode_plan.cpp b/simulst_amd/csrc/decode_plan.cpp
--- a/simulst_amd/csrc/decode_plan.cpp
+++ b/simulst_amd/csrc/decode_plan.cpp
@@ -20,7 +20,7 @@
   const sl_linear_plan pl = sl_plan_linear(h, dtype, SIMULST_EPI_BIAS_RES, p, o);
   return pl.family == SL_LIN_SKINNY && pl.splits == 1;
 }
-bool sl_dec_tall_fc1_shape_ok(const simulst_handle* h, int dtype, int B, int N, int K, bool packed) {
+static bool ln_panel_split(const simulst_handle* h, int dtype, int epi, int B, int N, int K, bool packed) {
   if (dtype != SIMULST_BF16 || !packed || B <= 0 || N <= 0 || K <= 0 || K > 256) return false;
   LinArgs p = {};
   p.M = B; p.rpb = B; p.N = N; p.K = K;
@@ -28,8 +28,18 @@
   p.scale = 1.f; p.w_packed = 1; p.amax_skip_a = p.amax_skip_b = -1;
   p.ln_g = p.ln_b = (const float*)h;
   const sl_linear_ops o = {};
-  const sl_linear_plan pl = sl_plan_linear(h, dtype, SIMULST_EPI_BIAS_GELU, p, o);
+  const sl_linear_plan pl = sl_plan_linear(h, dtype, epi, p, o);
   return pl.family == SL_LIN_PANEL_SPLIT;
+}
+bool sl_dec_tall_fc1_shape_ok(const simulst_handle* h, int dtype, int B, int N, int K, bool packed) {
+  return ln_panel_split(h, dtype, SIMULST_EPI_BIAS_GELU, B, N, K, packed);
+}
+bool sl_dec_tall_qkv_shape_ok(const simulst_handle* h, int dtype, int B, int N, int K, bool packed) {
+  return ln_panel_split(h, dtype, SIMULST_EPI_BIAS, B, N, K, packed);
+}
+bool sl_dec_tall_vocab_shape_ok(const simulst_handle* h, int dtype, int B, int V, int D, bool packed, bool has_ln) {
+  return B > 0 && B <= SKINNY_MAX_ROWS_PACKED && V > 0 && D > 0 && has_ln &&
+         sl_plan_vocab_argmax(h, dtype, B, V, D, packed, true).family == SL_LIN_PANEL_SPLIT;
 }
 bool sl_dec_tall_fc1_ok(const simulst_handle* h, int dtype, int B, int D, int F, bool packed) {
   return h->dec_tall_ffn && B >= h->dec_tall_min_rows && sl_dec_tall_fc1_shape_ok(h, dtype, B, F, D, packed);
@@ -56,10 +66,13 @@
   p.fuse_ffn_qkv = p.chain_ffn && !p.attn_chain && sl_dec_ffn_qkv_chain_ok(h, c.B, c.F);
   p.tall_ffn = !p.chain_ffn && !c.force_unfused && sl_dec_tall_fc2_ok(h, c.dtype, c.B, c.D, c.F, c.packed);
   p.tall_fc1 = !p.chain_ffn && !c.force_unfused && sl_dec_tall_fc1_ok(h, c.dtype, c.B, c.D, c.F, c.packed);
+  const bool tall_k256 = !p.chain_ffn && !c.force_unfused && h->dec_tall_k256 && c.B >= h->dec_tall_min_rows;
+  p.tall_qkv = tall_k256 && sl_dec_tall_qkv_shape_ok(h, c.dtype, c.B, 3 * c.D, c.D, c.packed);
   const bool masks_known = c.mode == SL_CALL_STREAM || c.mask_eos || lockstep;
   p.vsplit = (p.chain_ffn && masks_known && h->fused_argmax && !c.highway)
                  ? sl_dec_vocab_chain_split(h, c.dtype, c.B, c.V, c.D, c.packed, c.final_ln) : 0;
   p.tile_argmax = !p.vsplit && !c.cif && masks_known && sl_vocab_argmax_ok(h, c.dtype, c.B, c.V, c.D, c.packed);
+  p.tall_vocab = tall_k256 && p.tile_argmax && sl_dec_tall_vocab_shape_ok(h, c.dtype, c.B, c.V, c.D, c.packed, c.final_ln);
   p.n_pairs = p.vsplit ? p.vsplit : p.tile_argmax ? c.V / 64 : 0;
   p.fuse_commit = !c.cif && p.chain_ffn && lockstep && h->dec_embed_qkv_chain && p.n_pairs > 0 && p.n_pairs <= 64;
   return p;
@@ -92,6 +105,8 @@
   if (l > 0 && p.fuse_ffn_qkv) return SIMULST_OK;
   if (l > 0 && p.chain_ffn)
     return sl_dec_qkv_chain(h, w.x_mid, w.x, w.ffn_partial, prev_b2, q.ln_g, q.ln_b, q.w, q.b, w.qkv, w.B, w.F);
+  if (p.tall_qkv && q.ln_g && q.ln_b && sl_dec_tall_operands_ok(w.x, q.w, w.qkv, q.b))
+    return sl_dec_tall_qkv(h, w.x, q.w, q.b, q.ln_g, q.ln_b, w.qkv, w.B, 3 * w.D, w.D, 0);
   return sl_lin(h, w.dtype, w.B, 3 * w.D, w.D, w.x, q.w, q.b, nullptr, w.qkv, SIMULST_EPI_BIAS, q.ln_g, q.ln_b, w.packed);
 }
 
diff --git a/simulst_amd/csrc/decode_plan.h b/simulst_amd/csrc/decode_plan.h
--- a/simulst_amd/csrc/decode_plan.h
+++ b/simulst_amd/csrc/decode_plan.h
@@ -31,6 +31,8 @@
   bool fuse_ffn_qkv;
   bool tall_ffn;
   bool tall_fc1;
+  bool tall_qkv;
+  bool tall_vocab;
   int vsplit;
   bool tile_argmax;
   int n_pairs;
@@ -63,6 +65,12 @@
 bool sl_dec_tall_fc1_ok(const simulst_handle* h, int dtype, int B, int D, int F, bool packed);
 int sl_dec_tall_fc1(simulst_handle* h, const void* A, const void* W, const float* bias, const float* ln_g, const float* ln_b, void* C,
                     int B, int N, int K);
+bool sl_dec_tall_qkv_shape_ok(const simulst_handle* h, int dtype, int B, int N, int K, bool packed);
+bool sl_dec_tall_vocab_shape_ok(const simulst_handle* h, int dtype, int B, int V, int D, bool packed, bool has_ln);
+int sl_dec_tall_qkv(simulst_handle* h, const void* A, const void* W, const float* bias, const float* ln_g, const float* ln_b, void* C,
+                    int B, int N, int K, int steps);
+int sl_dec_tall_vocab(simulst_handle* h, const void* x, const void* W, const float* ln_g, const float* ln_b, float2* pairs, int B, int V,
+                      int D, int skip_a, int skip_b, int steps);
 int sl_step_qkv(simulst_handle* h, const sl_decode_plan& p, const sl_step_bufs& w, int l, const float* prev_b2, const sl_qkv_weights& q);
 int sl_step_ffn(simulst_handle* h, const sl_decode_plan& p, const sl_step_bufs& w, const void* ctx, const void* res,
                 const sl_ffn_weights& f, const sl_qkv_weights& next);
diff --git a/simulst_amd/csrc/handle.cpp b/simulst_amd/csrc/handle.cpp
--- a/simulst_amd/csrc/handle.cpp
+++ b/simulst_amd/csrc/handle.cpp
@@ -39,6 +39,14 @@
   if (const char* e = getenv("SIMULST_DEC_TALL_FFN")) h->dec_tall_ffn = atoi(e) != 0;
   h->dec_tall_min_rows = h->dec_chain_ffn_max_rows + 1;
   if (const char* e = getenv("SIMULST_DEC_TALL_MIN_ROWS")) h->dec_tall_min_rows = atoi(e);
+  h->dec_tall_k256 = true;
+  if (const char* e = getenv("SIMULST_DEC_TALL_K256")) h->dec_tall_k256 = atoi(e) != 0;
+  h->dec_tall_fc1_steps = 4;
+  if (const char* e = getenv("SIMULST_DEC_TALL_FC1_STEPS")) { const int v = atoi(e); if (v >= 1 && v <= 8) h->dec_tall_fc1_steps = v; }
+  h->dec_tall_qkv_steps = 2;
+  if (const char* e = getenv("SIMULST_DEC_TALL_QKV_STEPS")) { const int v = atoi(e); if (v >= 1 && v <= 8) h->dec_tall_qkv_steps = v; }
+  h->dec_tall_vocab_steps = 4;
+  if (const char* e = getenv("SIMULST_DEC_TALL_VOCAB_STEPS")) { const int v = atoi(e); if (v >= 1 && v <= 8) h->dec_tall_vocab_steps = v; }
   h->dec_chain_lds_attr_set = false;
   h->dec_chain_probe_attr_set = false;
   h->dec_chain_lds_bytes = 0;
@@ -228,6 +236,7 @@
     case SIMULST_OPT_DEC_EMBED_QKV_CHAIN: h->dec_embed_qkv_chain = value != 0; return SIMULST_OK;
     case SIMULST_OPT_WEIGHT_STATIONARY: h->wstat = value != 0; return SIMULST_OK;
     case SIMULST_OPT_DEC_TALL_FFN: h->dec_tall_ffn = value != 0; return SIMULST_OK;
+    case SIMULST_OPT_DEC_TALL_K256: h->dec_tall_k256 = value != 0; return SIMULST_OK;
     case SIMULST_OPT_CONV_TILE256:
       SL_REQUIRE(h, value >= 0 && value <= 2, SIMULST_E_ARG, "simulst_set_option(CONV_TILE256): 0 (128 x 128 tiles), 1 (256 x 256, register stage), 2 (256 x 256, LDS-DMA ring)");
       h->tile256 = value; return SIMULST_OK;
@@ -285,6 +294,7 @@
     case SIMULST_OPT_DEC_VOCAB_CHAIN_SPLIT: *value = h->dec_vocab_chain_split; return SIMULST_OK;
     case SIMULST_OPT_WEIGHT_STATIONARY: *value = h->wstat; return SIMULST_OK;
     case SIMULST_OPT_DEC_TALL_FFN: *value = h->dec_tall_ffn; return SIMULST_OK;
+    case SIMULST_OPT_DEC_TALL_K256: *value = h->dec_tall_k256; return SIMULST_OK;
     case SIMULST_OPT_CONV_TILE256: *value = h->tile256; return SIMULST_OK;
     case SIMULST_OPT_DEC_FUSE_FFN_QKV: *value = h->dec_fuse_ffn_qkv; return SIMULST_OK;
     case SIMULST_OPT_DEC_CHAIN_ROWS32: *value = h->dec_chain_rows32; return SIMULST_OK;
```

Result: no change. 1.906 million tokens/s (median of 2 runs) (+0.3%).
